# ielhelw/mcmc-ammsb-gpu

Hardware: AMD Instinct MI355X
Metric: mini-batch edges/s (SG-MCMC a-MMSB learner loop) (higher is better)
Workload: dtype f32

## Files before the change

### include/ammsb.h

```cpp
#ifndef AMMSB_H
#define AMMSB_H

#include <stddef.h>
#include <stdint.h>

#ifdef __cplusplus
extern "C" {
#endif

#define AMMSB_VERSION 200

enum {
  AMMSB_OK = 0,
  AMMSB_EINVAL = -1,
  AMMSB_EHIP = -2,
  AMMSB_ENOMEM = -3,
  AMMSB_ENODEV = -4,
  AMMSB_ERANGE = -5
};

#define AMMSB_MAX_GROUPS 65535u
#define AMMSB_RPM_MAX_BLOCKS 32

typedef struct { uint64_t x, y; } ammsb_seed;

typedef struct {
  uint64_t N, K, E;
  uint32_t num_node_sample;
  float alpha, a, b, c, epsilon, eta0, eta1;
} ammsb_params;

typedef struct {
  void* blocks[AMMSB_RPM_MAX_BLOCKS];
  uint64_t rows_in_block;
  uint64_t num_rows, num_cols;
  uint32_t num_blocks;
} ammsb_rpm;

typedef struct {
  const uint64_t* slots;
  uint64_t num_bins;
  uint32_t prime_idx;
} ammsb_set;

typedef struct {
  double link_ll, nonlink_ll;
  uint64_t link_cnt, nonlink_cnt;
} ammsb_ppx_sums;

typedef struct ammsb_ctx ammsb_ctx;

#define AMMSB_NOISE_OFF 1u
#define AMMSB_PHI_STREAMING 2u

int ammsb_version(void);
const char* ammsb_strerror(int code);
const char* ammsb_last_error(const ammsb_ctx* ctx);

int ammsb_params_quantize(ammsb_params* p);
float ammsb_eps_t(const ammsb_params* p, uint32_t step_count);

int ammsb_ctx_create(int device_id, const ammsb_params* params, ammsb_ctx** out);
int ammsb_ctx_destroy(ammsb_ctx* ctx);
int ammsb_ctx_params(const ammsb_ctx* ctx, ammsb_params* out);

int ammsb_rng_init(ammsb_ctx* ctx, ammsb_seed* seeds, uint64_t n, uint64_t sx, uint64_t sy, void* stream);
int ammsb_rng_init_mixed(ammsb_ctx* ctx, ammsb_seed* seeds, uint64_t n, uint64_t sx, uint64_t sy, void* stream);

int ammsb_set_has(ammsb_ctx* ctx, const ammsb_set* set, const uint64_t* keys, uint64_t n, uint8_t* out,
                  void* stream);

uint64_t ammsb_set_num_bins(uint64_t n);
int ammsb_set_build(ammsb_ctx* ctx, const uint64_t* keys, uint64_t n, uint64_t* slots, uint64_t num_bins,
                    uint32_t* prime_idx_out, uint32_t* scratch, void* stream);

int ammsb_pi_init_gamma(ammsb_ctx* ctx, const ammsb_rpm* pi, float* phi_sum, float eta0, float eta1,
                        ammsb_seed* seeds, void* stream);

int ammsb_sample_neighbors(ammsb_ctx* ctx, ammsb_seed* seeds, const uint32_t* nodes, uint32_t n_nodes,
                           uint32_t wg, uint32_t* table, uint32_t* packed, void* stream);

int ammsb_update_phi(ammsb_ctx* ctx, const float* beta, const ammsb_rpm* pi, const float* phi_sum,
                     const ammsb_set* training_set, const uint32_t* nodes, const uint32_t* neighbors,
                     uint32_t n_nodes, uint32_t step_count, ammsb_seed* seeds, uint32_t wg, uint32_t flags,
                     uint32_t group_begin, uint32_t group_end, float* phi_vec, void* stream);

int ammsb_update_phi_occupancy(ammsb_ctx* ctx, uint32_t wg, int* blocks_per_cu, int* waves_per_block);

int ammsb_update_pi(ammsb_ctx* ctx, const ammsb_rpm* pi, float* phi_sum, const float* phi_vec,
                    const uint32_t* nodes, uint32_t n_nodes, uint32_t wg, void* stream);

int ammsb_theta_sum(ammsb_ctx* ctx, float* out, void* stream);

int ammsb_beta_grads(ammsb_ctx* ctx, const float* theta, const float* beta, const ammsb_rpm* pi,
                     const ammsb_set* training_set, const uint64_t* edges, uint32_t n_edges,
                     uint32_t edge_begin, uint32_t edge_end, uint32_t wg, float* grads_out, void* stream);

int ammsb_can_fuse_pi_beta(ammsb_ctx* ctx, uint32_t phi_wg, uint32_t beta_wg);
int ammsb_update_pi_beta_grads(ammsb_ctx* ctx, const float* theta, const float* beta, const ammsb_rpm* pi,
                               float* phi_sum, const float* phi_vec, const uint32_t* nodes,
                               const ammsb_set* training_set, const uint64_t* edges, uint32_t n_edges, uint32_t wg,
                               float* grads_out, void* stream);

int ammsb_sum_rows_f32(ammsb_ctx* ctx, const float* in, uint32_t rows, uint32_t cols, float* out, void* stream);

int ammsb_update_theta(ammsb_ctx* ctx, float* theta, float* beta, const float* grads, uint32_t step_count,
                       float scale, ammsb_seed* seeds, uint32_t flags, void* stream);

int ammsb_beta_from_theta(ammsb_ctx* ctx, const float* theta, float* beta, void* stream);

int ammsb_perplexity(ammsb_ctx* ctx, const float* beta, const ammsb_rpm* pi, const ammsb_set* heldout_set,
                     const uint64_t* edges, uint32_t n_edges, uint32_t edge_begin, uint32_t edge_end,
                     uint32_t call_count, uint32_t wg, float* ppx_per_edge, ammsb_ppx_sums* out, void* stream);


int ammsb_minibatch_link(ammsb_ctx* ctx, const uint64_t* csr_offsets, const uint32_t* csr_targets, uint32_t u,
                         uint32_t n, uint64_t* edges_out, uint32_t* nodes_out, void* stream);

uint32_t ammsb_minibatch_candidates(uint64_t N, uint32_t m);
uint32_t ammsb_minibatch_candidates_for(uint64_t N, uint32_t m, uint64_t excluded);
uint64_t ammsb_minibatch_workspace_bytes(uint32_t capacity);

int ammsb_minibatch_nonlink(ammsb_ctx* ctx, ammsb_seed* seeds, uint32_t n_candidates, uint32_t capacity, uint32_t u,
                            uint32_t m, const ammsb_set* training_set, const ammsb_set* heldout_set, void* workspace,
                            uint64_t* edges_out, uint32_t* nodes_out, uint32_t* count_out, void* stream);

typedef struct ammsb_loop ammsb_loop;

#define AMMSB_LOOP_TIMESTAMPS 1u

typedef struct {
  float* theta;
  float* beta;
  const ammsb_rpm* pi;
  float* phi_sum;
  const ammsb_set* training_set;
  const ammsb_set* heldout_set;
  ammsb_seed* phi_seeds;
  float* phi_vec;
  uint32_t phi_wg, phi_flags;
  ammsb_seed* beta_seeds;
  float* grads;
  uint32_t beta_wg, beta_flags;
  uint64_t* edges[2];
  uint32_t* nodes[2];
  uint32_t* neighbors[2];
  uint32_t* nbr_table[2];
  ammsb_seed* nbr_seeds[2];
  uint32_t nbr_wg;
  const uint64_t* csr_offsets;
  const uint32_t* csr_targets;
  ammsb_seed* mb_seeds;
  uint32_t mb_candidates;
  void* mb_workspace;
  uint32_t* mb_count;
  uint32_t mini_batch;
  uint32_t max_fan_out;
  uint32_t max_nodes;
  uint32_t max_edges;
  uint32_t flags;
} ammsb_loop_config;

typedef struct {
  uint32_t link, u, n, n_candidates;
} ammsb_mb_choice;

int ammsb_loop_create(ammsb_ctx* ctx, const ammsb_loop_config* cfg, ammsb_loop** out);
int ammsb_loop_destroy(ammsb_loop* loop);
// ... 30 lines not shown
```

### mcmc-ammsb-gpu_amd/_capi.py

```python
import ctypes as C
import os

_HERE = os.path.dirname(os.path.abspath(__file__))
LIB_PATH = os.environ.get("AMMSB_HIP_LIB") or os.path.join(_HERE, "libammsb_hip.so")

RPM_MAX_BLOCKS = 32
MAX_GROUPS = 65535
NOISE_OFF = 1
PHI_STREAMING = 2


class AmmsbError(RuntimeError):
    pass


class Params(C.Structure):
    _fields_ = [("N", C.c_uint64), ("K", C.c_uint64), ("E", C.c_uint64),
                ("num_node_sample", C.c_uint32),
                ("alpha", C.c_float), ("a", C.c_float), ("b", C.c_float), ("c", C.c_float),
                ("epsilon", C.c_float), ("eta0", C.c_float), ("eta1", C.c_float)]


class Rpm(C.Structure):
    _fields_ = [("blocks", C.c_void_p * RPM_MAX_BLOCKS), ("rows_in_block", C.c_uint64),
                ("num_rows", C.c_uint64), ("num_cols", C.c_uint64), ("num_blocks", C.c_uint32)]


class SetDesc(C.Structure):
    _fields_ = [("slots", C.c_void_p), ("num_bins", C.c_uint64), ("prime_idx", C.c_uint32)]


class PpxSums(C.Structure):
    _fields_ = [("link_ll", C.c_double), ("nonlink_ll", C.c_double),
                ("link_cnt", C.c_uint64), ("nonlink_cnt", C.c_uint64)]


_vp, _u32, _u64, _f32 = C.c_void_p, C.c_uint32, C.c_uint64, C.c_float
_P = C.POINTER

LOOP_TIMESTAMPS = 1


class LoopConfig(C.Structure):
    _fields_ = [("theta", _vp), ("beta", _vp), ("pi", _P(Rpm)), ("phi_sum", _vp),
                ("training_set", _P(SetDesc)), ("heldout_set", _P(SetDesc)),
                ("phi_seeds", _vp), ("phi_vec", _vp), ("phi_wg", _u32), ("phi_flags", _u32),
                ("beta_seeds", _vp), ("grads", _vp), ("beta_wg", _u32), ("beta_flags", _u32),
                ("edges", _vp * 2), ("nodes", _vp * 2), ("neighbors", _vp * 2), ("nbr_table", _vp * 2),
                ("nbr_seeds", _vp * 2), ("nbr_wg", _u32),
                ("csr_offsets", _vp), ("csr_targets", _vp), ("mb_seeds", _vp), ("mb_candidates", _u32),
                ("mb_workspace", _vp), ("mb_count", _vp), ("mini_batch", _u32), ("max_fan_out", _u32),
                ("max_nodes", _u32), ("max_edges", _u32), ("flags", _u32)]


class MbChoice(C.Structure):
    _fields_ = [("link", _u32), ("u", _u32), ("n", _u32), ("n_candidates", _u32)]


SIGNATURES = {
    "ammsb_version": [],
    "ammsb_strerror": [C.c_int],
    "ammsb_last_error": [_vp],
    "ammsb_last_kernel_name": [_vp, C.c_int],
    "ammsb_params_quantize": [_P(Params)],
    "ammsb_eps_t": [_P(Params), _u32],
    "ammsb_ctx_create": [C.c_int, _P(Params), _P(_vp)],
    "ammsb_ctx_destroy": [_vp],
    "ammsb_theta_sum": [_vp, _vp, _vp],
    "ammsb_ctx_params": [_vp, _P(Params)],
    "ammsb_rng_init": [_vp, _vp, _u64, _u64, _u64, _vp],
    "ammsb_rng_init_mixed": [_vp, _vp, _u64, _u64, _u64, _vp],
    "ammsb_set_has": [_vp, _P(SetDesc), _vp, _u64, _vp, _vp],
    "ammsb_set_num_bins": [_u64],
    "ammsb_set_build": [_vp, _vp, _u64, _vp, _u64, _P(_u32), _vp, _vp],
    "ammsb_pi_init_gamma": [_vp, _P(Rpm), _vp, _f32, _f32, _vp, _vp],
    "ammsb_sample_neighbors": [_vp, _vp, _vp, _u32, _u32, _vp, _vp, _vp],
    "ammsb_update_phi": [_vp, _vp, _P(Rpm), _vp, _P(SetDesc), _vp, _vp, _u32, _u32, _vp, _u32, _u32,
                         _u32, _u32, _vp, _vp],
    "ammsb_update_phi_occupancy": [_vp, _u32, _P(C.c_int), _P(C.c_int)],
    "ammsb_update_pi": [_vp, _P(Rpm), _vp, _vp, _vp, _u32, _u32, _vp],
    "ammsb_beta_grads": [_vp, _vp, _vp, _P(Rpm), _P(SetDesc), _vp, _u32, _u32, _u32, _u32, _vp, _vp],
    "ammsb_can_fuse_pi_beta": [_vp, _u32, _u32],
    "ammsb_update_pi_beta_grads": [_vp, _vp, _vp, _P(Rpm), _vp, _vp, _vp, _P(SetDesc), _vp, _u32, _u32, _vp, _vp],
    "ammsb_sum_rows_f32": [_vp, _vp, _u32, _u32, _vp, _vp],
    "ammsb_update_theta": [_vp, _vp, _vp, _vp, _u32, _f32, _vp, _u32, _vp],
    "ammsb_beta_from_theta": [_vp, _vp, _vp, _vp],
    "ammsb_perplexity": [_vp, _vp, _P(Rpm), _P(SetDesc), _vp, _u32, _u32, _u32, _u32, _u32, _vp, _vp, _vp],
    "ammsb_minibatch_link": [_vp, _vp, _vp, _u32, _u32, _vp, _vp, _vp],
    "ammsb_minibatch_candidates": [_u64, _u32],
    "ammsb_minibatch_candidates_for": [_u64, _u32, _u64],
    "ammsb_minibatch_workspace_bytes": [_u32],
    "ammsb_minibatch_nonlink": [_vp, _vp, _u32, _u32, _u32, _u32, _P(SetDesc), _P(SetDesc), _vp, _vp, _vp, _vp, _vp],
    "ammsb_loop_create": [_vp, _P(LoopConfig), _P(_vp)],
    "ammsb_loop_destroy": [_vp],
    "ammsb_loop_run": [_vp, _P(MbChoice), _P(MbChoice), _u32, _u32, _u32, _vp],
    "ammsb_loop_check": [_vp, _P(_u32)],
    "ammsb_loop_status": [_vp, _P(_u32), _P(_u32)],
    "ammsb_loop_timestamps": [_vp, _u32, _u32, _P(C.c_double), _P(C.c_double)],
    "ammsb_loop_step_stamps": [_vp, _u32, _u32, _P(C.c_double)],
    "ammsb_wg_sum_f32": [_vp, _vp, _vp, _u32, _u32, _u32, _vp],
    "ammsb_wg_sum_u32": [_vp, _vp, _vp, _u32, _u32, _u32, _vp],
    "ammsb_wg_normalize_f32": [_vp, _vp, _vp, _u32, _u32, _u32, _vp],
    "ammsb_rpm_sum_f32": [_vp, _P(Rpm), _vp, _u32, _vp],
    "ammsb_rpm_normalize_f32": [_vp, _P(Rpm), _vp, _u32, _vp],
    "ammsb_wg_sort_u32": [_vp, _vp, _vp, _u32, _vp],
    "ammsb_wg_sort_f32": [_vp, _vp, _vp, _u32, _vp],
    "ammsb_randn_fill": [_vp, _vp, _u32, _u32, _vp, _vp],
    "ammsb_rpm_fetch": [_vp, _P(Rpm), _u64, _u64, _vp, _vp],
    "ammsb_clock_probe": [_vp, _vp, _u32, _u32, _vp],
}
_OTHER_RES = {"ammsb_strerror": C.c_char_p, "ammsb_last_error": C.c_char_p, "ammsb_last_kernel_name": C.c_char_p,
              "ammsb_eps_t": C.c_float,
              "ammsb_minibatch_candidates": C.c_uint32, "ammsb_minibatch_candidates_for": C.c_uint32,
              "ammsb_minibatch_workspace_bytes": C.c_uint64, "ammsb_set_num_bins": C.c_uint64}

_lib = None


def load(path=None):
    global _lib
    if _lib is not None and path is None:
        return _lib
    so = path or LIB_PATH
    if not os.path.exists(so):
        raise AmmsbError("%s not found: build it with `make -C mcmc-ammsb-gpu_amd/csrc` "
                         "(or __graft_entry__.build()); there is no CPU fallback" % so)
    import torch
    lib = C.CDLL(so)
    for name, args in SIGNATURES.items():
        fn = getattr(lib, name)
        fn.argtypes = args
        fn.restype = _OTHER_RES.get(name, C.c_int)
    if path is None:
        _lib = lib
    return lib


def check(rc, ctx=None):
    if rc != 0:
        lib = load()
        msg = lib.ammsb_strerror(rc).decode()
        if ctx:
            msg += " (" + lib.ammsb_last_error(ctx).decode() + ")"
        raise AmmsbError("ammsb call failed: %d %s" % (rc, msg))
```

### mcmc-ammsb-gpu_amd/csrc/ammsb_core.hip

```cpp
#include <math.h>
#include <stdlib.h>
#include <string.h>

#include "ammsb_ctx.h"
#include "ammsb_dev.h"
#include "ammsb_step.h"

using namespace ammsb;


extern "C" int ammsb_version(void) { return AMMSB_VERSION; }

extern "C" const char* ammsb_strerror(int code) {
  switch (code) {
    case AMMSB_OK: return "ok";
    case AMMSB_EINVAL: return "invalid argument";
    case AMMSB_EHIP: return "HIP runtime error";
    case AMMSB_ENOMEM: return "out of device memory";
    case AMMSB_ENODEV: return "no usable gfx950 device";
    case AMMSB_ERANGE: return "size out of range for the launch shape";
    default: return "unknown error";
  }
}

// ... 165 lines not shown
  AMMSB_CHECK_ARG(ctx, m, "null matrix");
  AMMSB_CHECK_ARG(ctx, m->num_blocks >= 1 && m->num_blocks <= AMMSB_RPM_MAX_BLOCKS, "bad block count");
  AMMSB_CHECK_ARG(ctx, m->rows_in_block > 0 && m->num_cols > 0, "bad block shape");
  AMMSB_CHECK_ARG(ctx, (uint64_t)m->num_blocks * m->rows_in_block >= m->num_rows, "blocks do not cover rows");
  for (uint32_t i = 0; i < m->num_blocks; ++i) AMMSB_CHECK_ARG(ctx, m->blocks[i], "null block");
  return AMMSB_OK;
}


__global__ __launch_bounds__(64) void pi_init_kernel(ammsb_rpm pi, float* phi_sum, float eta0, float eta1,
                                                      ammsb_seed* seeds, uint32_t G) {
  using Grp = Group<32>;
  __shared__ ZigTables zig;
  zig_load(&zig);
  __syncthreads();
  const uint32_t g = blockIdx.x * Grp::PER_BLOCK + Grp::slot();
  const uint32_t l = Grp::lane();
  const bool live = g < G;
  ammsb_seed s = {0, 0};
  if (live) s = seeds[(uint64_t)g * 32 + l];
  const uint64_t N = pi.num_rows, K = pi.num_cols;
  const uint64_t trips = (N + G - 1) / G;
  int phase = 0;
  for (uint64_t t = 0; t < trips; ++t) {
    const uint64_t row = g + t * G;
    const bool on = live && row < N;
    float* r = on ? rpm_row(pi, row) : nullptr;
    float lsum = 0;
    if (on)
      for (uint64_t j = l; j < K; j += 32) {
        const float v = rng_gamma(s, &zig, eta0, eta1);
        r[j] = v;
        lsum += v;
      }
    const float sum = Grp::sum(lsum, (float*)nullptr, phase);
    if (on) {
      for (uint64_t j = l; j < K; j += 32) r[j] = r[j] / sum;
      if (l == 0) phi_sum[row] = sum;
    }
  }
  if (live) seeds[(uint64_t)g * 32 + l] = s;
}

extern "C" int ammsb_pi_init_gamma(ammsb_ctx* ctx, const ammsb_rpm* pi, float* phi_sum, float eta0, float eta1,
                                   ammsb_seed* seeds, void* stream) {
  AMMSB_CHECK_ARG(ctx, ctx && phi_sum && seeds, "null argument");
  int rc = check_rpm(ctx, pi);
  if (rc) return rc;
  const uint32_t G = pi->num_rows < AMMSB_MAX_GROUPS ? (uint32_t)pi->num_rows : AMMSB_MAX_GROUPS;
  pi_init_kernel<<<div_up(G, 2), 64, 0, as_stream(stream)>>>(*pi, phi_sum, eta0, eta1, seeds, G);
  AMMSB_LAUNCH_CHECK(ctx);
  return AMMSB_OK;
}


__device__ __forceinline__ void ns_generate(ammsb_seed& seed, uint32_t* out, uint32_t capacity, uint32_t max_id,
                                            uint32_t node) {
  uint32_t r, val;
  do {
    do {
      r = (uint32_t)(rng_next(seed) % (uint64_t)(max_id + 1));
    } while (r == node);
    const uint32_t l1 = (r ^ 553105253u) % capacity;
    const uint32_t l2 = 1u + (capacity << 1);
    for (uint32_t i = 0;; ++i) {
      const uint32_t offset = (l1 + i * l2) % capacity;
      val = out[offset];
      if (val == r) break;
      if (val == max_id + 1) {
        out[offset] = r;
        break;
      }
    }
  } while (val == r);
}

__host__ __device__ __forceinline__ uint32_t ns_global_size(uint32_t n_nodes, uint32_t wg) {
  uint32_t groups = n_nodes / wg + (n_nodes % wg ? 1 : 0);
  const uint32_t maxg = AMMSB_MAX_GROUPS / wg;
  if (groups > maxg) groups = maxg;
  return groups * wg;
}

__global__ __launch_bounds__(64) void sample_neighbors_kernel(ammsb_seed* seeds, const uint32_t* nodes,
                                                               uint32_t n_nodes, uint32_t N, uint32_t n,
                                                               uint32_t gsize, uint32_t* table, uint32_t* packed,
                                                               const ammsb_step_desc* desc, uint32_t wg) {
  if (desc) {
    n_nodes = desc->n_nodes;
    gsize = ns_global_size(n_nodes, wg);
  }
  const uint32_t gid = blockIdx.x * blockDim.x + threadIdx.x;
  if (gid >= gsize || gid >= n_nodes) return;
  const uint32_t capacity = 2 * n;
  ammsb_seed seed = seeds[gid];
  for (uint32_t i = gid; i < n_nodes; i += gsize) {
    uint32_t* out = table + (uint64_t)i * capacity;
    uint32_t* pk = packed + (uint64_t)i * n;
    const uint32_t node = nodes[i];
    for (uint32_t j = 0; j < capacity; ++j) out[j] = N;
    for (uint32_t j = 0; j < n; ++j) ns_generate(seed, out, capacity, N - 1, node);
    uint32_t count = 0;
    for (uint32_t j = 0; j < capacity && count < n; ++j) {
      const uint32_t v = out[j];
      if (v != N) pk[count++] = v;
    }
  }
  seeds[gid] = seed;
}

__global__ __launch_bounds__(64) void sample_neighbors_lds_kernel(ammsb_seed* seeds, const uint32_t* nodes,
                                                                   uint32_t n_nodes, uint32_t N, uint32_t n,
                                                                   uint32_t gsize, uint32_t* table, uint32_t* packed,
                                                                   const ammsb_step_desc* desc, uint32_t wg) {
  if (desc) {
    n_nodes = desc->n_nodes;
    gsize = ns_global_size(n_nodes, wg);
    if (blockIdx.x * 64 >= gsize || blockIdx.x * 64 >= n_nodes) return;
  }
  extern __shared__ uint32_t lds[];
  constexpr uint32_t S = 65;
  const uint32_t lane = threadIdx.x;
  const uint32_t gid = blockIdx.x * 64 + lane;
  const uint32_t capacity = 2 * n;
  const bool owner = gid < gsize && gid < n_nodes;
  ammsb_seed seed = owner ? seeds[gid] : ammsb_seed{0, 0};
  const uint32_t max_id = N - 1;
  const FastMod mod_n = fast_mod_init((uint64_t)max_id + 1);
  const uint64_t cap_m = ~0ull / capacity + 1;
  auto advance = [](uint32_t& row, uint32_t& col, uint32_t width) {
    col += 64;
    while (col >= width) {
      col -= width;
      ++row;
    }
  };
  for (uint32_t base = blockIdx.x * 64; base < n_nodes; base += gsize) {
    const uint32_t i = base + lane;
    const bool on = owner && i < n_nodes;
    const uint32_t live = min(64u, min(n_nodes - base, gsize - blockIdx.x * 64));
    for (uint32_t j = 0; j < capacity; ++j) lds[j * S + lane] = N;
    if (on) {
      const uint32_t node = nodes[i];
      for (uint32_t j = 0; j < n; ++j) {
        uint32_t r, val;
        do {
          do {
            r = (uint32_t)fast_mod(rng_next(seed), mod_n);
          } while (r == node);
          uint32_t offset = (uint32_t)__umul64hi(cap_m * (uint64_t)(r ^ 553105253u), capacity);
          for (;;) {
            val = lds[offset * S + lane];
            if (val == r) break;
            if (val == max_id + 1) {
              lds[offset * S + lane] = r;
              break;
            }
            offset = offset + 1 == capacity ? 0 : offset + 1;
          }
        } while (val == r);
      }
    }
    __syncthreads();
    uint32_t* tout = table + (uint64_t)base * capacity;
    {
      uint32_t row = 0, col = lane;
      while (col >= capacity) {
        col -= capacity;
        ++row;
      }
      for (uint32_t x = lane; x < live * capacity; x += 64) {
        tout[x] = lds[col * S + row];
        advance(row, col, capacity);
      }
    }
    __syncthreads();
    if (on) {
      uint32_t count = 0;
      for (uint32_t j = 0; j < capacity && count < n; ++j) {
        const uint32_t v = lds[j * S + lane];
        if (v != N) lds[(count++) * S + lane] = v;
      }
    }
    __syncthreads();
    uint32_t* pout = packed + (uint64_t)base * n;
    {
      uint32_t row = 0, col = lane;
      while (col >= n) {
        col -= n;
        ++row;
      }
      for (uint32_t x = lane; x < live * n; x += 64) {
        pout[x] = lds[col * S + row];
        advance(row, col, n);
      }
    }
    __syncthreads();
  }
  if (owner) seeds[gid] = seed;
}

__global__ __launch_bounds__(256) void sample_neighbors_wave_kernel(ammsb_seed* seeds, const uint32_t* nodes,
                                                                     uint32_t n_nodes, uint32_t N, uint32_t gsize,
                                                                     uint32_t* table, uint32_t* packed,
                                                                     const ammsb_step_desc* desc, uint32_t wg) {
  constexpr uint32_t CAP = 64, NN = 32, B = 40;
  if (desc) {
    n_nodes = desc->n_nodes;
    gsize = ns_global_size(n_nodes, wg);
  }
  const uint32_t lane = threadIdx.x & 63;
  const uint32_t gid = __builtin_amdgcn_readfirstlane(blockIdx.x * 4 + (threadIdx.x >> 6));
  if (gid >= gsize || gid >= n_nodes) return;
  ammsb_seed st = seeds[gid];
  const FastMod mod_n = fast_mod_init((uint64_t)N);
  for (uint32_t i = gid; i < n_nodes; i += gsize) {
    const uint32_t node = nodes[i];
    uint32_t slot = N;
    uint32_t count = 0;
    while (count < NN) {
      ammsb_seed run = st, mine = st;
      uint64_t raw = 0;
#pragma unroll 8
      for (uint32_t j = 0; j < B; ++j) {
        const uint64_t x = rng_next(run);
        if (lane == j) {
          raw = x;
          mine = run;
        }
      }
      const uint32_t r = (uint32_t)fast_mod(raw, mod_n);
      const uint32_t h = (r ^ 553105253u) & (CAP - 1);
      uint32_t used = 0;
      for (uint32_t j = 0; j < B && count < NN; ++j) {
        used = j + 1;
        const uint32_t rj = (uint32_t)__builtin_amdgcn_readlane((int)r, (int)j);
        if (rj == node) continue;
        if (__ballot(slot == rj) != 0ull) continue;
        const uint32_t hj = (uint32_t)__builtin_amdgcn_readlane((int)h, (int)j);
        const unsigned long long freeb = ~__ballot(slot != N);
        const unsigned long long rot = hj ? ((freeb >> hj) | (freeb << (64 - hj))) : freeb;
        const uint32_t pos = (hj + (uint32_t)__builtin_ctzll(rot)) & (CAP - 1);
        if (lane == pos) slot = rj;
        ++count;
      }
      auto lane64 = [&](uint64_t v) -> uint64_t {
        const uint32_t hi = (uint32_t)__builtin_amdgcn_readlane((int)(uint32_t)(v >> 32), (int)(used - 1));
        const uint32_t lo = (uint32_t)__builtin_amdgcn_readlane((int)(uint32_t)v, (int)(used - 1));
        return ((uint64_t)hi << 32) | lo;
      };
      st.x = lane64(mine.x);
      st.y = lane64(mine.y);
    }
    table[(uint64_t)i * CAP + lane] = slot;
    const unsigned long long occ = __ballot(slot != N);
    if (slot != N) packed[(uint64_t)i * NN + __popcll(occ & ((1ull << lane) - 1ull))] = slot;
  }
  if (lane == 0) seeds[gid] = st;
}

static int sample_neighbors_common(ammsb_ctx* ctx, ammsb_seed* seeds, const uint32_t* nodes, uint32_t n_nodes,
                                   uint32_t wg, uint32_t* table, uint32_t* packed, const ammsb_step_desc* desc,
                                   void* stream) {
  AMMSB_CHECK_ARG(ctx, ctx && seeds && nodes && table && packed, "null argument");
  AMMSB_CHECK_ARG(ctx, wg >= 1 && wg <= 1024, "sampler wg out of range");
  if (n_nodes == 0) return AMMSB_OK;
  const uint32_t n = ctx->params.num_node_sample;
  AMMSB_CHECK_ARG(ctx, ctx->params.N > (uint64_t)n + 1, "N must exceed num_node_sample + 1");
  const uint32_t gsize = ns_global_size(n_nodes, wg);
  const size_t lds_bytes = (size_t)2 * n * 65 * sizeof(uint32_t);
  static const bool per_thread = [] {
    const char* f = getenv("AMMSB_NBR_FORM");
    return f && f[0] == 't';
  }();
  if (n == 32 && !per_thread && n_nodes <= 20000) {
    const uint32_t waves = gsize < n_nodes ? gsize : n_nodes;
    ctx->kernel_name[AMMSB_KN_NBR] = "sample_neighbors_wave_kernel";
    sample_neighbors_wave_kernel<<<div_up(waves, 4), 256, 0, as_stream(stream)>>>(
        seeds, nodes, n_nodes, (uint32_t)ctx->params.N, gsize, table, packed, desc, wg);
  } else if (lds_bytes <= 64 * 1024) {
    ctx->kernel_name[AMMSB_KN_NBR] = "sample_neighbors_lds_kernel";
    sample_neighbors_lds_kernel<<<div_up(gsize, 64), 64, lds_bytes, as_stream(stream)>>>(
        seeds, nodes, n_nodes, (uint32_t)ctx->params.N, n, gsize, table, packed, desc, wg);
  } else {
    ctx->kernel_name[AMMSB_KN_NBR] = "sample_neighbors_kernel";
    sample_neighbors_kernel<<<div_up(gsize, 64), 64, 0, as_stream(stream)>>>(
        seeds, nodes, n_nodes, (uint32_t)ctx->params.N, n, gsize, table, packed, desc, wg);
  }
  AMMSB_LAUNCH_CHECK(ctx);
  return AMMSB_OK;
}

extern "C" int ammsb_sample_neighbors(ammsb_ctx* ctx, ammsb_seed* seeds, const uint32_t* nodes, uint32_t n_nodes,
                                      uint32_t wg, uint32_t* table, uint32_t* packed, void* stream) {
  return sample_neighbors_common(ctx, seeds, nodes, n_nodes, wg, table, packed, nullptr, stream);
}

int ammsb_sample_neighbors_d(ammsb_ctx* ctx, ammsb_seed* seeds, const uint32_t* nodes, uint32_t n_nodes_cap, uint32_t wg,
                             uint32_t* table, uint32_t* packed, const ammsb_step_desc* desc, void* stream) {
  AMMSB_CHECK_ARG(ctx, ctx && desc, "null descriptor");
  return sample_neighbors_common(ctx, seeds, nodes, n_nodes_cap, wg, table, packed, desc, stream);
}


__device__ __forceinline__ uint32_t power_of_2(uint32_t v) {
  v |= v >> 1;
  v |= v >> 2;
  v |= v >> 4;
  v |= v >> 8;
  v |= v >> 16;
  return v + 1;
}

template <typename T>
__device__ __forceinline__ T wg_sum_lds(const T* in, T* aux, uint32_t len) {
  const uint32_t lid = threadIdx.x, lsize = blockDim.x;
  T lsum = 0;
  for (uint32_t i = lid; i < len; i += lsize) lsum += in[i];
  aux[lid] = lsum;
  __syncthreads();
  for (uint32_t p2 = power_of_2(lsize) >> 1; p2 > 0; p2 >>= 1) {
    if (lid < p2 && lid + p2 < lsize) aux[lid] += aux[lid + p2];
    __syncthreads();
  }
  const T r = aux[0];
  __syncthreads();
  return r;
}

template <typename T>
__global__ void wg_sum_kernel(const T* in, T* out, uint32_t rows, uint32_t len) {
  __shared__ T aux[1024];
  for (uint32_t gid = blockIdx.x; gid < rows; gid += gridDim.x) {
    const T s = wg_sum_lds(in + (uint64_t)gid * len, aux, len);
    if (threadIdx.x == 0) out[gid] = s;
  }
}

__global__ void wg_normalize_kernel(float* in, float* sums, uint32_t rows, uint32_t len) {
  __shared__ float aux[1024];
  for (uint32_t gid = blockIdx.x; gid < rows; gid += gridDim.x) {
    float* row = in + (uint64_t)gid * len;
    const float sum = wg_sum_lds(row, aux, len);
    for (uint32_t i = threadIdx.x; i < len; i += blockDim.x) row[i] = row[i] / sum;
    if (sums && threadIdx.x == 0) sums[gid] = sum;
    __syncthreads();
  }
}

__global__ void rpm_sum_kernel(ammsb_rpm m, float* out, int normalize) {
  __shared__ float aux[1024];
  for (uint64_t gid = blockIdx.x; gid < m.num_rows; gid += gridDim.x) {
    float* row = rpm_row(m, gid);
    const float sum = wg_sum_lds(row, aux, (uint32_t)m.num_cols);
    if (normalize)
      for (uint64_t i = threadIdx.x; i < m.num_cols; i += blockDim.x) row[i] = row[i] / sum;
    if (threadIdx.x == 0) out[gid] = sum;
    __syncthreads();
  }
}

template <typename T>
__global__ void wg_sort_kernel(const T* in, T* out) {
  __shared__ T aux[1024];
  const size_t i = threadIdx.x, wg = blockDim.x;
  aux[i] = in[i];
  __syncthreads();
  for (size_t length = 1; length < wg; length <<= 1) {
    const bool direction = ((i & (length << 1)) != 0);
    for (size_t inc = length; inc > 0; inc >>= 1) {
      const size_t j = i ^ inc;
      const T idata = aux[i], jdata = aux[j];
      const bool smaller = (jdata < idata) || (jdata == idata && j < i);
      const bool swap = smaller ^ (j < i) ^ direction;
      __syncthreads();
      aux[i] = swap ? jdata : idata;
      __syncthreads();
    }
  }
  out[i] = aux[i];
}

static inline uint32_t cap_groups(uint64_t rows) { return rows < AMMSB_MAX_GROUPS ? (uint32_t)rows : AMMSB_MAX_GROUPS; }

// ... 107 lines not shown
```

### mcmc-ammsb-gpu_amd/csrc/ammsb_loop.hip

```cpp
#include "ammsb_ctx.h"
#include "ammsb_step.h"

#include <stdlib.h>
#include <string.h>

#include <atomic>
#include <chrono>
#include <mutex>
#include <new>
#include <thread>
#include <vector>

namespace {

constexpr uint32_t CHUNK = 1024;
constexpr uint32_t STAMP_CAP = AMMSB_STAMP_CAP;
constexpr int NBUF = 3;

__global__ void loop_prime_kernel(const ammsb_step_desc* ring, uint32_t* cursor, ammsb_step_desc* cur,
                                  ammsb_step_desc* nxt, const uint32_t* timeouts) {
  *cur = ring[0];
  *nxt = ring[2];
  *cursor = 0;
  if (timeouts && *timeouts != 0u) {
    cur->n_nodes = 0;
    cur->n_edges = 0;
  }
}

constexpr int HS_MAIN = 0, HS_AVAIL = 1, HS_TIMEOUTS = 2;

__global__ void loop_wait_kernel(const uint32_t* a, const uint32_t* b, int min_diff, uint32_t* timeouts,
                                 unsigned long long max_ticks, const ammsb_step_desc* src, ammsb_step_desc* dst,
                                 uint32_t fail_at) {
  const uint32_t have = *b;
  const unsigned long long t0 = wall_clock64();
  bool ok = false;
  for (;;) {
    if (__hip_atomic_load(timeouts, __ATOMIC_ACQUIRE, __HIP_MEMORY_SCOPE_AGENT) != 0u) break;
    if (fail_at != 0u && have + 1u == fail_at) {
      atomicAdd(timeouts, 1u);
      break;
    }
    const uint32_t v = __hip_atomic_load(a, __ATOMIC_ACQUIRE, __HIP_MEMORY_SCOPE_AGENT);
    if ((int)(v - have) >= min_diff) {
      ok = true;
      break;
    }
    if (wall_clock64() - t0 > max_ticks) {
      atomicAdd(timeouts, 1u);
      break;
    }
    __builtin_amdgcn_s_sleep(8);
  }
  if (dst) {
    if (ok) {
      *dst = *src;
    } else {
      ammsb_step_desc skip = *src;
      skip.n_nodes = 0;
      skip.n_edges = 0;
      skip.n_cand = 0;
      *dst = skip;
    }
  }
}

__global__ void loop_bump_kernel(uint32_t* counter, const ammsb_step_desc* desc) {
  if (ammsb_desc_skip(desc)) return;
  __hip_atomic_store(counter, *counter + 1u, __ATOMIC_RELEASE, __HIP_MEMORY_SCOPE_AGENT);
}

__global__ void loop_copy_kernel(uint4* dst, const uint4* src, size_t bytes, const uint32_t* timeouts) {
  if (timeouts && *timeouts != 0u) return;
  const size_t n16 = bytes / 16;
  for (size_t i = (size_t)blockIdx.x * blockDim.x + threadIdx.x; i < n16; i += (size_t)gridDim.x * blockDim.x)
    dst[i] = src[i];
  if (blockIdx.x == 0 && threadIdx.x < (bytes % 16) / 4)
    reinterpret_cast<uint32_t*>(dst + n16)[threadIdx.x] = reinterpret_cast<const uint32_t*>(src + n16)[threadIdx.x];
}

__global__ void loop_probe_wait_kernel(const uint32_t* flag, uint32_t* saw, unsigned long long max_ticks) {
  const unsigned long long t0 = wall_clock64();
  while (wall_clock64() - t0 <= max_ticks) {
    if (__hip_atomic_load(flag, __ATOMIC_ACQUIRE, __HIP_MEMORY_SCOPE_AGENT) != 0u) {
      *saw = 1u;
      return;
    }
    __builtin_amdgcn_s_sleep(8);
  }
  *saw = 0u;
}
__global__ void loop_probe_set_kernel(uint32_t* flag) { __hip_atomic_store(flag, 1u, __ATOMIC_RELEASE, __HIP_MEMORY_SCOPE_AGENT); }

struct Stage {
  ammsb_step_desc* ring;
  hipEvent_t done;
  bool used;
};

struct SampleBuf {
  uint64_t* edges;
  uint32_t* nodes;
  uint32_t* neighbors;
  uint32_t* nbr_table;
};

}

struct ammsb_loop {
  ammsb_ctx* ctx;
  ammsb_loop_config c;
  ammsb_rpm pi;
  ammsb_set training, heldout;
  bool has_heldout;
  hipStream_t main, side;
  hipEvent_t ev_in, ev_out, ev_prime, ev_first;
  hipEvent_t ev_main[NBUF], ev_samp[NBUF];
  SampleBuf buf[NBUF];
  void* own_mem;
  ammsb_step_desc* d_ring;
  uint32_t* d_cursor;
  ammsb_step_desc* d_cur[2];
  ammsb_step_desc* d_nxt[NBUF];
  uint32_t* d_hs;
  ammsb_step_desc* d_samp[NBUF];
  bool use_events;
  bool direct_only;
  uint32_t fallbacks;
  uint32_t test_fail_at;
  struct Run {
    ammsb_mb_choice pending;
    std::vector<ammsb_mb_choice> next;
    uint32_t n_steps, first_step_count, parity;
    hipStream_t stream;
    uint64_t main_start;
  };
  std::vector<Run>* runs;
  uint64_t main_total;
  unsigned long long wait_ticks;
  unsigned long long* d_stamps;
  Stage stage[2];
  int next_stage;
  hipGraphExec_t exec_main[2][NBUF][2];
  hipGraphExec_t exec_samp[2][NBUF][2];
  uint32_t link_nodes_cap, link_edges_cap, n_nbr;
  float w_link, w_nonlink;
  int wall_khz;
  uint64_t graphs_launched;
  bool serial_launch;
  bool eager_launch;
  bool host_prof;
  double t_side_us, t_main_us, t_run_us, t_pro_us, t_epi_us;
  uint64_t runs_done;
};

namespace {

#define LOOP_HIP(lp, call)                                                                              \
  do {                                                                                                  \
    hipError_t e_ = (call);                                                                             \
    if (e_ != hipSuccess) {                                                                             \
      snprintf((lp)->ctx->err, sizeof((lp)->ctx->err), "%s: %s -> %s", __func__, #call, hipGetErrorString(e_)); \
      return AMMSB_EHIP;                                                                                \
    }                                                                                                   \
  } while (0)

#define LOOP_RC(call)         \
  do {                        \
    const int rc_ = (call);   \
    if (rc_ != AMMSB_OK) return rc_; \
  } while (0)

int record_sampler(ammsb_loop* lp, int nl, int b, int sp, const ammsb_step_desc* desc, hipStream_t st) {
  const ammsb_loop_config& c = lp->c;
  ammsb_ctx* ctx = lp->ctx;
  const SampleBuf& o = lp->buf[b];
  const uint32_t m = c.mini_batch;
  if (!lp->use_events) {
    loop_wait_kernel<<<1, 1, 0, st>>>(lp->d_hs + HS_MAIN, lp->d_hs + HS_AVAIL, -2, lp->d_hs + HS_TIMEOUTS, lp->wait_ticks,
                                      desc, lp->d_samp[b], lp->test_fail_at);
    LOOP_HIP(lp, hipGetLastError());
    desc = lp->d_samp[b];
  }
  if (nl)
    LOOP_RC(ammsb_minibatch_link_d(ctx, c.csr_offsets, c.csr_targets, lp->link_edges_cap, o.edges, o.nodes, desc, st));
  else
    LOOP_RC(ammsb_minibatch_nonlink_d(ctx, c.mb_seeds, c.mb_candidates, m, &lp->training,
                                      lp->has_heldout ? &lp->heldout : nullptr, c.mb_workspace, o.edges, o.nodes,
                                      c.mb_count, desc, st));
  LOOP_RC(ammsb_sample_neighbors_d(ctx, c.nbr_seeds[sp], o.nodes, nl ? lp->link_nodes_cap : m + 1, c.nbr_wg, o.nbr_table,
                                   o.neighbors, desc, st));
  if (!lp->use_events) {
    loop_bump_kernel<<<1, 1, 0, st>>>(lp->d_hs + HS_AVAIL, desc);
    LOOP_HIP(lp, hipGetLastError());
  }
  return AMMSB_OK;
}

int record_main(ammsb_loop* lp, int cl, int b, int dp, hipStream_t st) {
  const ammsb_loop_config& c = lp->c;
  ammsb_ctx* ctx = lp->ctx;
  const SampleBuf& in = lp->buf[b];
  const ammsb_step_desc* cur = lp->d_cur[dp];
  const uint32_t m = c.mini_batch;
  const uint32_t cap_nodes = cl ? lp->link_nodes_cap : m + 1;
  const uint32_t cap_edges = cl ? lp->link_edges_cap : m;
  LOOP_RC(ammsb_update_phi_d(ctx, c.beta, &lp->pi, c.phi_sum, &lp->training, in.nodes, in.neighbors, cap_nodes,
                             c.phi_seeds, c.phi_wg, c.phi_flags, c.phi_vec, cur, lp->d_stamps, st));
  const bool fuse_pi = ammsb_beta_can_fuse_pi(ctx, c.phi_wg, c.beta_wg) && lp->pi.num_cols % 4 == 0;
  const ammsb_pi_fusion fuse = {c.phi_vec, c.phi_sum, in.nodes, lp->d_stamps};
  if (!fuse_pi)
    LOOP_RC(ammsb_update_pi_d(ctx, &lp->pi, c.phi_sum, c.phi_vec, in.nodes, cap_nodes, c.phi_wg, cur, lp->d_stamps, st));
  const bool hs = !lp->use_events;
  const ammsb_step_advance adv = {lp->d_ring, lp->d_cursor, lp->d_cur[1 - dp], lp->d_nxt[b], 3u,
                                  hs ? lp->d_hs + HS_MAIN : nullptr, hs ? lp->d_hs + HS_AVAIL : nullptr,
                                  hs ? lp->d_hs + HS_TIMEOUTS : nullptr, lp->wait_ticks, lp->d_stamps};
  LOOP_RC(ammsb_beta_step_d(ctx, c.theta, c.beta, &lp->pi, &lp->training, in.edges, cap_edges, c.beta_wg, c.grads,
                            c.beta_seeds, c.beta_flags, cur, &adv, fuse_pi ? &fuse : nullptr, lp->d_stamps, st));
  return AMMSB_OK;
}

int capture(ammsb_loop* lp, int kind, int link, int b, int dp, hipGraphExec_t* out) {
  hipStream_t st = kind == 2 ? lp->side : lp->main;
  LOOP_HIP(lp, hipStreamBeginCapture(st, hipStreamCaptureModeThreadLocal));
  const int rc = kind == 2 ? record_sampler(lp, link, b, dp, lp->d_nxt[b], st) : record_main(lp, link, b, dp, st);
  hipGraph_t g = nullptr;
  const hipError_t e = hipStreamEndCapture(st, &g);
  if (rc != AMMSB_OK) {
    if (g) (void)hipGraphDestroy(g);
    return rc;
  }
  if (e != hipSuccess || !g) {
    snprintf(lp->ctx->err, sizeof lp->ctx->err, "ammsb_loop: hipStreamEndCapture -> %s", hipGetErrorString(e));
    return AMMSB_EHIP;
  }
  const hipError_t e2 = hipGraphInstantiate(out, g, nullptr, nullptr, 0);
  (void)hipGraphDestroy(g);
  if (e2 != hipSuccess) {
    snprintf(lp->ctx->err, sizeof lp->ctx->err, "ammsb_loop: hipGraphInstantiate -> %s", hipGetErrorString(e2));
    return AMMSB_EHIP;
  }
  return AMMSB_OK;
}

void destroy(ammsb_loop* lp) {
  if (!lp) return;
  if (lp->host_prof && lp->graphs_launched)
    fprintf(stderr,
            "ammsb_loop host profile: %llu steps, hipGraphLaunch sampler %.2f us, main %.2f us per step; %llu runs: %.1f us "
            "each (prologue %.1f, epilogue %.1f)\n",
            (unsigned long long)lp->graphs_launched, lp->t_side_us / lp->graphs_launched, lp->t_main_us / lp->graphs_launched,
            (unsigned long long)lp->runs_done, lp->t_run_us / lp->runs_done, lp->t_pro_us / lp->runs_done, lp->t_epi_us / lp->runs_done);
  if (lp->main) (void)hipStreamSynchronize(lp->main);
  if (lp->side) (void)hipStreamSynchronize(lp->side);
  for (int a = 0; a < 2; ++a)
    for (int b = 0; b < NBUF; ++b)
      for (int p = 0; p < 2; ++p) {
        if (lp->exec_main[a][b][p]) (void)hipGraphExecDestroy(lp->exec_main[a][b][p]);
        if (lp->exec_samp[a][b][p]) (void)hipGraphExecDestroy(lp->exec_samp[a][b][p]);
      }
  for (Stage& st : lp->stage) {
    if (st.ring) (void)hipHostFree(st.ring);
    if (st.done) (void)hipEventDestroy(st.done);
  }
  for (hipEvent_t ev : {lp->ev_in, lp->ev_out, lp->ev_prime, lp->ev_first, lp->ev_main[0], lp->ev_main[1], lp->ev_main[2],
                        lp->ev_samp[0], lp->ev_samp[1], lp->ev_samp[2]})
    if (ev) (void)hipEventDestroy(ev);
  if (lp->d_ring) (void)hipFree(lp->d_ring);
  if (lp->d_stamps) (void)hipFree(lp->d_stamps);
  if (lp->d_hs) (void)hipFree(lp->d_hs);
  if (lp->own_mem) (void)hipFree(lp->own_mem);
  if (lp->side) (void)hipStreamDestroy(lp->side);
  if (lp->main) (void)hipStreamDestroy(lp->main);
  delete lp->runs;
  delete lp;
}

ammsb_step_desc make_desc(const ammsb_loop* lp, const ammsb_mb_choice& ch, uint32_t step) {
  ammsb_step_desc d;
  memset(&d, 0, sizeof d);
  if (ch.link) {
    d.n_nodes = ch.n + 1;
    d.n_edges = ch.n;
    d.scale = lp->w_link;
  } else {
    d.n_nodes = lp->c.mini_batch + 1;
    d.n_edges = lp->c.mini_batch;
    d.scale = lp->w_nonlink;
  }
  d.eps_t = ammsb_eps_t(&lp->ctx->params, step);
  d.u = ch.u;
  d.link = ch.link ? 1u : 0u;
  d.n_cand = ch.n_candidates;
  d.step = step;
  return d;
}

int check_choice(ammsb_loop* lp, const ammsb_mb_choice& ch) {
  ammsb_ctx* ctx = lp->ctx;
  AMMSB_CHECK_ARG(ctx, ch.u < ctx->params.N, "mini-batch vertex out of range");
  if (ch.link) {
    AMMSB_CHECK_ARG(ctx, ch.n > 0 && ch.n <= lp->link_edges_cap, "link batch: degree 0 or above max_fan_out");
  } else {
    AMMSB_CHECK_ARG(ctx, ch.n_candidates >= lp->c.mini_batch && ch.n_candidates <= lp->c.mb_candidates &&
                             ch.n_candidates % 256 == 0,
                    "non-link batch: bad candidate count");
  }
  return AMMSB_OK;
}

size_t align256(size_t x) { return (x + 255) & ~(size_t)255; }

}

extern "C" int ammsb_loop_create(ammsb_ctx* ctx, const ammsb_loop_config* cfg, ammsb_loop** out) {
  AMMSB_CHECK_ARG(ctx, ctx && cfg && out, "null argument");
  const ammsb_loop_config& c = *cfg;
  AMMSB_CHECK_ARG(ctx, c.theta && c.beta && c.pi && c.phi_sum && c.training_set && c.phi_seeds && c.phi_vec &&
                           c.beta_seeds && c.grads,
                  "null model / operator buffer");
  for (int i = 0; i < 2; ++i)
    AMMSB_CHECK_ARG(ctx, c.edges[i] && c.nodes[i] && c.neighbors[i] && c.nbr_table[i] && c.nbr_seeds[i],
                    "null sample buffer");
  for (int i = 0; i < 2; ++i)
    AMMSB_CHECK_ARG(ctx, ((reinterpret_cast<uintptr_t>(c.edges[i]) | reinterpret_cast<uintptr_t>(c.nodes[i]) |
                           reinterpret_cast<uintptr_t>(c.neighbors[i]) | reinterpret_cast<uintptr_t>(c.nbr_table[i])) & 15u) == 0,
                    "edges / nodes / neighbors / nbr_table must be 16-byte aligned");
  AMMSB_CHECK_ARG(ctx, c.csr_offsets && c.csr_targets && c.mb_seeds && c.mb_workspace && c.mb_count,
                  "null mini-batch sampler buffer");
  AMMSB_CHECK_ARG(ctx, c.mini_batch > 0 && c.max_fan_out > 0, "mini_batch / max_fan_out must be positive");
  AMMSB_CHECK_ARG(ctx, c.mb_candidates >= c.mini_batch && c.mb_candidates % 256 == 0, "bad candidate capacity");
  AMMSB_CHECK_ARG(ctx, c.max_nodes >= c.mini_batch + 1 && c.max_nodes >= c.max_fan_out + 1 && c.max_edges >= c.mini_batch &&
                           c.max_edges >= c.max_fan_out,
                  "max_nodes / max_edges smaller than the largest mini-batch (sample.cc:129-131)");
  AMMSB_HIP(ctx, hipSetDevice(ctx->device));
  ammsb_loop* lp = new (std::nothrow) ammsb_loop();
  if (!lp) return AMMSB_ENOMEM;
  memset(static_cast<void*>(lp), 0, sizeof *lp);
  lp->ctx = ctx;
  lp->c = c;
  lp->pi = *c.pi;
  lp->training = *c.training_set;
  lp->has_heldout = c.heldout_set != nullptr;
  if (lp->has_heldout) lp->heldout = *c.heldout_set;
  lp->c.pi = &lp->pi;
  lp->c.training_set = &lp->training;
  lp->c.heldout_set = lp->has_heldout ? &lp->heldout : nullptr;
  lp->link_edges_cap = c.max_fan_out;
  lp->link_nodes_cap = c.max_fan_out + 1;
  lp->n_nbr = ctx->params.num_node_sample;
  lp->w_link = static_cast<float>(ctx->params.N);
  lp->w_nonlink = static_cast<float>(2 * ctx->params.E) / static_cast<float>(c.mini_batch);
#define CREATE_HIP(call)                                                                           \
  do {                                                                                             \
    hipError_t e_ = (call);                                                                        \
    if (e_ != hipSuccess) {                                                                        \
      snprintf(ctx->err, sizeof ctx->err, "ammsb_loop_create: %s -> %s", #call, hipGetErrorString(e_)); \
      destroy(lp);                                                                                 \
      return AMMSB_EHIP;                                                                           \
    }                                                                                              \
  } while (0)
  {
    static const int prio = [] {
      const char* f = getenv("AMMSB_LOOP_PRIO");
      return f ? atoi(f) : 0;
    }();
    int least = 0, greatest = 0;
    if (prio) CREATE_HIP(hipDeviceGetStreamPriorityRange(&least, &greatest));
    static const int side_cus = [] {
      const char* f = getenv("AMMSB_LOOP_SIDE_CUS");
      return f ? atoi(f) : 0;
    }();
    if (side_cus > 0 && side_cus < ctx->num_cus) {
      uint32_t mask[16] = {0};
      for (int i = 0; i < side_cus && i < 512; ++i) mask[i / 32] |= 1u << (i % 32);
      CREATE_HIP(hipStreamCreateWithFlags(&lp->main, hipStreamNonBlocking));
      CREATE_HIP(hipExtStreamCreateWithCUMask(&lp->side, (uint32_t)((ctx->num_cus + 31) / 32), mask));
    } else if (prio && least != greatest) {
      CREATE_HIP(hipStreamCreateWithPriority(&lp->main, hipStreamNonBlocking, greatest));
      CREATE_HIP(hipStreamCreateWithPriority(&lp->side, hipStreamNonBlocking, least));
    } else {
      CREATE_HIP(hipStreamCreateWithFlags(&lp->main, hipStreamNonBlocking));
      CREATE_HIP(hipStreamCreateWithFlags(&lp->side, hipStreamNonBlocking));
    }
  }
  for (hipEvent_t* ev : {&lp->ev_in, &lp->ev_out, &lp->ev_prime, &lp->ev_first, &lp->ev_main[0], &lp->ev_main[1],
                         &lp->ev_main[2], &lp->ev_samp[0], &lp->ev_samp[1], &lp->ev_samp[2]})
    CREATE_HIP(hipEventCreateWithFlags(ev, hipEventDisableTiming));
  for (int i = 0; i < 2; ++i) lp->buf[i] = SampleBuf{c.edges[i], c.nodes[i], c.neighbors[i], c.nbr_table[i]};
  {
    const size_t e_b = align256(sizeof(uint64_t) * c.max_edges), n_b = align256(sizeof(uint32_t) * c.max_nodes);
    const size_t p_b = align256(sizeof(uint32_t) * (size_t)c.max_nodes * lp->n_nbr);
    const size_t t_b = align256(sizeof(uint32_t) * (size_t)c.max_nodes * 2 * lp->n_nbr);
    CREATE_HIP(hipMalloc(&lp->own_mem, e_b + n_b + p_b + t_b));
    CREATE_HIP(hipMemset(lp->own_mem, 0, e_b + n_b + p_b + t_b));
    char* p = static_cast<char*>(lp->own_mem);
    lp->buf[2].edges = reinterpret_cast<uint64_t*>(p);
    lp->buf[2].nodes = reinterpret_cast<uint32_t*>(p + e_b);
    lp->buf[2].neighbors = reinterpret_cast<uint32_t*>(p + e_b + n_b);
    lp->buf[2].nbr_table = reinterpret_cast<uint32_t*>(p + e_b + n_b + p_b);
  }
  lp->runs = new (std::nothrow) std::vector<ammsb_loop::Run>();
  if (!lp->runs) {
    destroy(lp);
    return AMMSB_ENOMEM;
  }
  const size_t n_desc = CHUNK + 4 + 8;
  CREATE_HIP(hipMalloc(&lp->d_ring, sizeof(ammsb_step_desc) * n_desc + 64));
  CREATE_HIP(hipMemset(lp->d_ring, 0, sizeof(ammsb_step_desc) * n_desc + 64));
  lp->d_cur[0] = lp->d_ring + CHUNK + 4;
  lp->d_cur[1] = lp->d_ring + CHUNK + 5;
  lp->d_nxt[0] = lp->d_ring + CHUNK + 6;
  lp->d_nxt[1] = lp->d_ring + CHUNK + 7;
  lp->d_nxt[2] = lp->d_ring + CHUNK + 8;
  for (int b = 0; b < NBUF; ++b) lp->d_samp[b] = lp->d_ring + CHUNK + 9 + b;
  lp->d_cursor = reinterpret_cast<uint32_t*>(lp->d_ring + n_desc);
  {
    CREATE_HIP(hipMalloc(&lp->d_hs, 64));
    const uint32_t hs0[4] = {0u, 1u, 0u, 0u};
    CREATE_HIP(hipMemcpy(lp->d_hs, hs0, sizeof hs0, hipMemcpyHostToDevice));
    const char* mode = getenv("AMMSB_LOOP_HANDSHAKE");
    const char* pmc = getenv("ROCPROF_COUNTER_COLLECTION");
    auto truthy = [](const char* v) { return v && v[0] && strcmp(v, "0") != 0 && strcmp(v, "False") != 0 && strcmp(v, "false") != 0; };
    const bool serialising_tool = truthy(pmc) || truthy(getenv("AMD_SERIALIZE_KERNEL")) || truthy(getenv("HIP_LAUNCH_BLOCKING")) ||
                                  truthy(getenv("CUDA_LAUNCH_BLOCKING"));
    lp->use_events = mode ? strcmp(mode, "event") == 0 : serialising_tool;
    int khz0 = 100000;
    CREATE_HIP(hipDeviceGetAttribute(&khz0, hipDeviceAttributeWallClockRate, ctx->device));
    if (!lp->use_events && !(mode && strcmp(mode, "flag") == 0)) {
      uint32_t* probe = lp->d_hs + 8;
      CREATE_HIP(hipMemset(probe, 0, 2 * sizeof(uint32_t)));
      loop_probe_wait_kernel<<<1, 1, 0, lp->main>>>(probe, probe + 1, 20ull * (unsigned long long)(khz0 > 0 ? khz0 : 100000));
      CREATE_HIP(hipGetLastError());
      loop_probe_set_kernel<<<1, 1, 0, lp->side>>>(probe);
      CREATE_HIP(hipGetLastError());
      CREATE_HIP(hipStreamSynchronize(lp->main));
      CREATE_HIP(hipStreamSynchronize(lp->side));
      uint32_t saw = 0;
      CREATE_HIP(hipMemcpy(&saw, probe + 1, sizeof saw, hipMemcpyDeviceToHost));
      if (!saw) lp->use_events = true;
    }
    if (const char* f = getenv("AMMSB_LOOP_TEST_FAIL_AT")) {
      const long v = strtol(f, nullptr, 10);
      if (v > 0) {
        lp->test_fail_at = (uint32_t)v;
        fprintf(stderr, "ammsb_loop: AMMSB_LOOP_TEST_FAIL_AT=%ld -- the sampler chain of mini-batch %ld will be made to give up (fault injection)\n", v, v);
      }
    }
    lp->host_prof = getenv("AMMSB_LOOP_HOSTPROF") != nullptr;
    const char* lm = getenv("AMMSB_LOOP_LAUNCH");
    lp->serial_launch = lm && strcmp(lm, "serial") == 0;
    lp->eager_launch = !(lm && strcmp(lm, "graph") == 0) && !lp->serial_launch && !lp->use_events;
    int khz = 100000;
    CREATE_HIP(hipDeviceGetAttribute(&khz, hipDeviceAttributeWallClockRate, ctx->device));
    lp->wait_ticks = 5000ull * (unsigned long long)(khz > 0 ? khz : 100000);
    if (const char* w = getenv("AMMSB_LOOP_WAIT_MS")) {
      char* end = nullptr;
      const long ms = strtol(w, &end, 10);
      if (end == w || *end != '\0' || ms < 1 || ms > 600000) {
        fprintf(stderr, "ammsb_loop: AMMSB_LOOP_WAIT_MS='%s' ignored (want 1 .. 600000); waits give up after 5 s\n", w);
      } else {
        lp->wait_ticks = (unsigned long long)ms * (unsigned long long)(khz > 0 ? khz : 100000);
        fprintf(stderr, "ammsb_loop: AMMSB_LOOP_WAIT_MS=%ld -- device-side waits give up after %ld ms\n", ms, ms);
      }
    }
  }
  for (Stage& st : lp->stage) {
    CREATE_HIP(hipHostMalloc(&st.ring, sizeof(ammsb_step_desc) * (CHUNK + 4), hipHostMallocDefault));
    CREATE_HIP(hipEventCreateWithFlags(&st.done, hipEventDisableTiming));
    st.used = false;
  }
  if (c.flags & AMMSB_LOOP_TIMESTAMPS) {
    CREATE_HIP(hipMalloc(&lp->d_stamps, sizeof(unsigned long long) * AMMSB_STAMP_SLOTS * STAMP_CAP));
    CREATE_HIP(hipMemset(lp->d_stamps, 0, sizeof(unsigned long long) * AMMSB_STAMP_SLOTS * STAMP_CAP));
    CREATE_HIP(hipDeviceGetAttribute(&lp->wall_khz, hipDeviceAttributeWallClockRate, ctx->device));
  }
#undef CREATE_HIP
  for (int link = 0; link < 2; ++link)
    for (int b = 0; b < NBUF; ++b)
      for (int dp = 0; dp < 2; ++dp) {
        int rc = capture(lp, 1, link, b, dp, &lp->exec_main[link][b][dp]);
        if (rc == AMMSB_OK) rc = capture(lp, 2, link, b, dp, &lp->exec_samp[link][b][dp]);
        if (rc != AMMSB_OK) {
          destroy(lp);
          return rc;
        }
      }
  *out = lp;
  return AMMSB_OK;
}

extern "C" int ammsb_loop_destroy(ammsb_loop* lp) {
  destroy(lp);
  return AMMSB_OK;
}

static std::mutex g_submit_mutex;

namespace {

int submit(ammsb_loop* lp, const ammsb_mb_choice* pending, const ammsb_mb_choice* next, uint32_t n_steps,
           uint32_t first_step_count, uint32_t parity, hipStream_t s, uint32_t done0, uint32_t avail0) {
  ammsb_ctx* ctx = lp->ctx;
  const uint32_t p0 = parity;
  const bool ev = lp->use_events;
  using clk = std::chrono::steady_clock;
  auto us_since = [](clk::time_point t) { return std::chrono::duration<double, std::micro>(clk::now() - t).count(); };
  const clk::time_point t_run = clk::now();
  auto choice = [&](uint32_t j) -> const ammsb_mb_choice& { return j == 0 ? *pending : next[j - 1]; };
  LOOP_HIP(lp, hipEventRecord(lp->ev_in, s));
  LOOP_HIP(lp, hipStreamWaitEvent(lp->main, lp->ev_in, 0));
  uint32_t done = done0;
  if (done0 == n_steps && avail0 <= n_steps) {
    Stage& st = lp->stage[lp->next_stage];
    lp->next_stage ^= 1;
    if (st.used) LOOP_HIP(lp, hipEventSynchronize(st.done));
    st.ring[0] = make_desc(lp, choice(n_steps), first_step_count + n_steps);
    LOOP_HIP(lp, hipMemcpyAsync(lp->d_ring, st.ring, sizeof(ammsb_step_desc), hipMemcpyHostToDevice, lp->main));
    LOOP_HIP(lp, hipEventRecord(st.done, lp->main));
    st.used = true;
    LOOP_HIP(lp, hipEventRecord(lp->ev_prime, lp->main));
    LOOP_HIP(lp, hipStreamWaitEvent(lp->side, lp->ev_prime, 0));
    LOOP_RC(record_sampler(lp, choice(n_steps).link ? 1 : 0, (int)((p0 + n_steps) % NBUF), (int)((p0 + n_steps) & 1u),
                           lp->d_ring, lp->side));
    if (ev) LOOP_HIP(lp, hipEventRecord(n_steps == 1 ? lp->ev_first : lp->ev_samp[(n_steps - 2) % NBUF], lp->side));
  }
  while (done < n_steps) {
    const uint32_t cnt = n_steps - done < CHUNK ? n_steps - done : CHUNK;
    const clk::time_point t_pro = clk::now();
    Stage& st = lp->stage[lp->next_stage];
    lp->next_stage ^= 1;
    if (st.used) LOOP_HIP(lp, hipEventSynchronize(st.done));
    for (uint32_t i = 0; i < cnt + 4; ++i) {
      const uint32_t j = done + i <= n_steps ? done + i : n_steps;
      st.ring[i] = make_desc(lp, choice(j), first_step_count + done + i);
    }
    LOOP_HIP(lp, hipMemcpyAsync(lp->d_ring, st.ring, sizeof(ammsb_step_desc) * (cnt + 4), hipMemcpyHostToDevice, lp->main));
    LOOP_HIP(lp, hipEventRecord(st.done, lp->main));
    st.used = true;
    const int dp0 = (int)((p0 + done) & 1u);
    loop_prime_kernel<<<1, 1, 0, lp->main>>>(lp->d_ring, lp->d_cursor, lp->d_cur[dp0], lp->d_nxt[(p0 + done + 2) % NBUF],
                                             ev ? nullptr : lp->d_hs + HS_TIMEOUTS);
    LOOP_HIP(lp, hipGetLastError());
    LOOP_RC(ammsb_theta_coef_d(ctx, lp->c.theta, lp->c.beta, lp->main));
    LOOP_HIP(lp, hipEventRecord(lp->ev_prime, lp->main));
    if (done == done0) {
      const uint32_t hi = done0 + 2 < n_steps + 1 ? done0 + 2 : n_steps + 1;
      for (uint32_t j = avail0 > done0 ? avail0 : done0; j < hi; ++j) {
        if (j == 0) continue;
        LOOP_HIP(lp, hipStreamWaitEvent(lp->side, lp->ev_prime, 0));
        LOOP_RC(record_sampler(lp, choice(j).link ? 1 : 0, (int)((p0 + j) % NBUF), (int)((p0 + j) & 1u),
                               lp->d_ring + (j - done0), lp->side));
        if (ev) LOOP_HIP(lp, hipEventRecord(j == 1 ? lp->ev_first : lp->ev_samp[(j - 2) % NBUF], lp->side));
      }
    }
    lp->t_pro_us += us_since(t_pro);
    bool threaded = !ev && cnt >= 32 && !lp->serial_launch && avail0 <= 1;
    if (threaded) {
      hipError_t side_err = hipSuccess;
      int side_rc = AMMSB_OK, main_rc = AMMSB_OK;
      std::atomic<uint32_t> main_sub(0), side_sub(0);
      std::atomic<bool> stop(false);
      const clk::time_point ts = clk::now();
      auto side_body = [&]() {
        side_err = hipSetDevice(ctx->device);
        if (side_err == hipSuccess) side_err = hipStreamWaitEvent(lp->side, lp->ev_prime, 0);
        for (uint32_t i = 0; i < cnt && side_err == hipSuccess && side_rc == AMMSB_OK && !stop.load(); ++i) {
          const uint32_t gi = done + i;
          if (gi + 2 > n_steps) break;
          while (main_sub.load(std::memory_order_acquire) < i) std::this_thread::yield();
          const int b = (int)((p0 + gi + 2) % NBUF), dp = (int)((p0 + gi) & 1u), nl = choice(gi + 2).link ? 1 : 0;
          if (lp->eager_launch) side_rc = record_sampler(lp, nl, b, dp, lp->d_nxt[b], lp->side);
          else side_err = hipGraphLaunch(lp->exec_samp[nl][b][dp], lp->side);
          side_sub.store(i + 1, std::memory_order_release);
        }
        if (side_err != hipSuccess || side_rc != AMMSB_OK) stop.store(true);
        side_sub.store(cnt + 2, std::memory_order_release);
      };
      std::thread helper;
      try {
        helper = std::thread(side_body);
      } catch (...) {
        threaded = false;
      }
      if (threaded) {
        hipError_t main_err = hipSuccess;
        for (uint32_t i = 0; i < cnt && main_err == hipSuccess && main_rc == AMMSB_OK && !stop.load(); ++i) {
          const uint32_t gi = done + i;
          while (i >= 1 && side_sub.load(std::memory_order_acquire) < i) std::this_thread::yield();
          const int b = (int)((p0 + gi) % NBUF), dp = (int)((p0 + gi) & 1u), cl = choice(gi).link ? 1 : 0;
          if (lp->eager_launch) main_rc = record_main(lp, cl, b, dp, lp->main);
          else main_err = hipGraphLaunch(lp->exec_main[cl][b][dp], lp->main);
          main_sub.store(i + 1, std::memory_order_release);
        }
        if (main_err != hipSuccess || main_rc != AMMSB_OK) stop.store(true);
        main_sub.store(cnt + 2, std::memory_order_release);
        if (lp->host_prof) lp->t_main_us += us_since(ts);
        helper.join();
        if (lp->host_prof) lp->t_side_us += us_since(ts);
        LOOP_HIP(lp, side_err);
        LOOP_HIP(lp, main_err);
        LOOP_RC(side_rc);
        LOOP_RC(main_rc);
      }
    }
    if (!threaded)
    for (uint32_t i = 0; i < cnt; ++i) {
      const uint32_t gi = done + i;
      const int dp = (int)((p0 + gi) & 1u);
      const bool sample = gi + 2 <= n_steps && gi + 2 >= avail0;
      if (sample) {
        if (i == 0) LOOP_HIP(lp, hipStreamWaitEvent(lp->side, lp->ev_prime, 0));
        else if (ev) LOOP_HIP(lp, hipStreamWaitEvent(lp->side, lp->ev_main[(gi - 1) % NBUF], 0));
        const auto t0 = lp->host_prof ? std::chrono::steady_clock::now() : std::chrono::steady_clock::time_point();
        const int nl = choice(gi + 2).link ? 1 : 0, b = (int)((p0 + gi + 2) % NBUF);
        if (lp->direct_only) LOOP_RC(record_sampler(lp, nl, b, dp, lp->d_nxt[b], lp->side));
        else LOOP_HIP(lp, hipGraphLaunch(lp->exec_samp[nl][b][dp], lp->side));
        if (lp->host_prof) lp->t_side_us += std::chrono::duration<double, std::micro>(std::chrono::steady_clock::now() - t0).count();
        if (ev) LOOP_HIP(lp, hipEventRecord(lp->ev_samp[gi % NBUF], lp->side));
      }
      if (ev && gi >= avail0) {
        if (gi == 1) LOOP_HIP(lp, hipStreamWaitEvent(lp->main, lp->ev_first, 0));
        else LOOP_HIP(lp, hipStreamWaitEvent(lp->main, lp->ev_samp[(gi - 2) % NBUF], 0));
      }
      const auto t1 = lp->host_prof ? std::chrono::steady_clock::now() : std::chrono::steady_clock::time_point();
      const int cl = choice(gi).link ? 1 : 0, bm = (int)((p0 + gi) % NBUF);
      if (lp->direct_only) LOOP_RC(record_main(lp, cl, bm, dp, lp->main));
      else LOOP_HIP(lp, hipGraphLaunch(lp->exec_main[cl][bm][dp], lp->main));
      if (lp->host_prof) lp->t_main_us += std::chrono::duration<double, std::micro>(std::chrono::steady_clock::now() - t1).count();
      if (ev) LOOP_HIP(lp, hipEventRecord(lp->ev_main[gi % NBUF], lp->main));
    }
    lp->graphs_launched += cnt;
    done += cnt;
  }
  const clk::time_point t_epi = clk::now();
  if (ev && n_steps >= avail0) LOOP_HIP(lp, hipStreamWaitEvent(lp->main, n_steps == 1 ? lp->ev_first : lp->ev_samp[(n_steps - 2) % NBUF], 0));
  if (!ev) {
    loop_wait_kernel<<<1, 1, 0, lp->main>>>(lp->d_hs + HS_AVAIL, lp->d_hs + HS_MAIN, 1, lp->d_hs + HS_TIMEOUTS, lp->wait_ticks,
                                            nullptr, nullptr, 0u);
    LOOP_HIP(lp, hipGetLastError());
  }
  const uint32_t from = (p0 + n_steps) % NBUF, to = (p0 + n_steps) & 1u;
  if (from != to) {
    const ammsb_mb_choice& ch = choice(n_steps);
    const size_t ne = ch.link ? ch.n : lp->c.mini_batch, nv = ne + 1;
    const SampleBuf &a = lp->buf[from], &b = lp->buf[to];
    const uint32_t* poison = ev ? nullptr : lp->d_hs + HS_TIMEOUTS;
    auto copy = [&](void* dst, const void* src, size_t bytes) {
      const size_t n16 = bytes / 16;
      const unsigned blocks = (unsigned)(n16 / 256 + 1 < 1024 ? n16 / 256 + 1 : 1024);
      loop_copy_kernel<<<blocks, 256, 0, lp->main>>>(static_cast<uint4*>(dst), static_cast<const uint4*>(src), bytes, poison);
    };
    copy(b.edges, a.edges, sizeof(uint64_t) * ne);
    copy(b.nodes, a.nodes, sizeof(uint32_t) * nv);
    copy(b.neighbors, a.neighbors, sizeof(uint32_t) * nv * lp->n_nbr);
    copy(b.nbr_table, a.nbr_table, sizeof(uint32_t) * nv * 2 * lp->n_nbr);
    LOOP_HIP(lp, hipGetLastError());
  }
  LOOP_HIP(lp, hipEventRecord(lp->ev_out, lp->main));
  LOOP_HIP(lp, hipStreamWaitEvent(s, lp->ev_out, 0));
  lp->t_epi_us += us_since(t_epi);
  lp->t_run_us += us_since(t_run);
  lp->runs_done += 1;
  return AMMSB_OK;
}

}

extern "C" int ammsb_loop_run(ammsb_loop* lp, const ammsb_mb_choice* pending, const ammsb_mb_choice* next,
                              uint32_t n_steps, uint32_t first_step_count, uint32_t parity, void* stream) {
  if (!lp) return AMMSB_EINVAL;
  ammsb_ctx* ctx = lp->ctx;
  AMMSB_CHECK_ARG(ctx, pending && (next || n_steps == 0), "null argument");
  AMMSB_CHECK_ARG(ctx, parity < 2 && first_step_count >= 1, "bad parity / step count");
  if (n_steps == 0) return AMMSB_OK;
  LOOP_RC(check_choice(lp, *pending));
  for (uint32_t i = 0; i < n_steps; ++i) LOOP_RC(check_choice(lp, next[i]));
  std::lock_guard<std::mutex> guard(g_submit_mutex);
  if (!lp->use_events) {
    try {
      ammsb_loop::Run r;
      r.pending = *pending;
      r.next.assign(next, next + n_steps);
      r.n_steps = n_steps;
      r.first_step_count = first_step_count;
      r.parity = parity;
      r.stream = as_stream(stream);
      r.main_start = lp->main_total;
      lp->runs->push_back(std::move(r));
    } catch (...) {
      return AMMSB_ENOMEM;
    }
  }
  lp->main_total += n_steps;
  return submit(lp, pending, next, n_steps, first_step_count, parity, as_stream(stream), 0u, 1u);
}

extern "C" int ammsb_loop_check(ammsb_loop* lp, uint32_t* wait_timeouts) {
  if (!lp) return AMMSB_EINVAL;
  ammsb_ctx* ctx = lp->ctx;
  AMMSB_CHECK_ARG(ctx, wait_timeouts, "null argument");
  std::lock_guard<std::mutex> guard(g_submit_mutex);
  LOOP_HIP(lp, hipStreamSynchronize(lp->side));
  LOOP_HIP(lp, hipStreamSynchronize(lp->main));
  uint32_t hs[3] = {0, 0, 0};
  LOOP_HIP(lp, hipMemcpy(hs, lp->d_hs, sizeof hs, hipMemcpyDeviceToHost));
  *wait_timeouts = 0;
  if (!hs[HS_TIMEOUTS]) {
    lp->runs->clear();
    return AMMSB_OK;
  }
  const uint64_t done_total = lp->main_total - (uint64_t)(uint32_t)((uint32_t)lp->main_total - hs[HS_MAIN]);
  const uint32_t avail_ahead = hs[HS_AVAIL] - hs[HS_MAIN];
  lp->use_events = true;
  lp->direct_only = true;
  lp->eager_launch = false;
  lp->fallbacks += 1;
  const uint32_t clear = 0;
  LOOP_HIP(lp, hipMemcpy(lp->d_hs + HS_TIMEOUTS, &clear, sizeof clear, hipMemcpyHostToDevice));
  std::vector<ammsb_loop::Run> runs;
  runs.swap(*lp->runs);
  const uint64_t avail_total = done_total + (avail_ahead <= 3 ? avail_ahead : 0);
  bool resumed = false;
  for (const ammsb_loop::Run& r : runs) {
    if (!resumed && r.main_start + r.n_steps <= done_total && r.main_start + r.n_steps < avail_total) continue;
    uint32_t done0 = 0, avail0 = 1;
    if (!resumed) {
      done0 = (uint32_t)(done_total > r.main_start ? done_total - r.main_start : 0);
      if (done0 > r.n_steps) done0 = r.n_steps;
      avail0 = (uint32_t)(avail_total > r.main_start ? avail_total - r.main_start : 0);
      if (avail0 == 0) avail0 = 1;
      resumed = true;
    }
    const int rc = submit(lp, &r.pending, r.next.data(), r.n_steps, r.first_step_count, r.parity, r.stream, done0, avail0);
    if (rc != AMMSB_OK) {
      *wait_timeouts = hs[HS_TIMEOUTS];
      return rc;
    }
  }
  LOOP_HIP(lp, hipStreamSynchronize(lp->side));
// ... 54 lines not shown
```

### mcmc-ammsb-gpu_amd/csrc/ammsb_phi.hip

```cpp
#pragma clang fp contract(off)

#include <stdlib.h>

#include "ammsb_ctx.h"
#include "ammsb_dev.h"
#include "ammsb_step.h"

#include <type_traits>

using namespace ammsb;

#ifdef AMMSB_PHI_TRACE
__device__ unsigned long long g_phi_trace[256];
#define PHI_TRACE(slot) do { if (blockIdx.x == 0 && threadIdx.x == 0 && (slot) < 256) g_phi_trace[(slot)] = __builtin_readcyclecounter(); } while (0)
extern "C" int ammsb_debug_trace(unsigned long long* out, int n) {
  return hipMemcpyFromSymbol(out, HIP_SYMBOL(g_phi_trace), sizeof(unsigned long long) * (n < 256 ? n : 256)) == hipSuccess ? 0 : -2;
}
#define AMMSB_PHI_BLK_CAP 65536
__device__ unsigned long long g_phi_blk[AMMSB_PHI_BLK_CAP * 5];
#define PHI_BLK(end) do { if (threadIdx.x == 0 && blockIdx.x < AMMSB_PHI_BLK_CAP) { \
    g_phi_blk[blockIdx.x * 5 + (end)] = __builtin_readcyclecounter(); \
    g_phi_blk[blockIdx.x * 5 + 2 + (end)] = __builtin_amdgcn_s_memrealtime(); \
    if (!(end)) g_phi_blk[blockIdx.x * 5 + 4] = (unsigned long long)__builtin_amdgcn_s_getreg((31 << 11) | 4) | \
                                               ((unsigned long long)__builtin_amdgcn_s_getreg((31 << 11) | 20) << 32); } } while (0)
extern "C" int ammsb_debug_blocks(unsigned long long* out, int n_blocks) {
  return hipMemcpyFromSymbol(out, HIP_SYMBOL(g_phi_blk), sizeof(unsigned long long) * 5 * (n_blocks < AMMSB_PHI_BLK_CAP ? n_blocks : AMMSB_PHI_BLK_CAP)) == hipSuccess ? 0 : -2;
}
#else
#define PHI_TRACE(slot) do { } while (0)
#define PHI_BLK(end) do { } while (0)
#endif

#ifndef AMMSB_PHI_LDS3_DEFAULT
#define AMMSB_PHI_LDS3_DEFAULT false
#endif

namespace {

struct PhiArgs {
  const float* beta;
  ammsb_rpm pi;
  const float* phi_sum;
  DevSet set;
  const uint32_t* nodes;
  const uint32_t* neighbors;
  ammsb_seed* seeds;
  float* phi_vec;
  uint32_t n_nodes, G, group_begin, group_end;
  uint32_t K, n;
  float eps_t, alpha, epsilon, Nn;
  uint32_t noise_on;
  uint32_t rows_nt;
  const ammsb_step_desc* desc;
  unsigned long long* stamps;
};


struct PhiStep {
  uint32_t n_nodes, G, group_end;
  float eps_t;
};
__device__ __forceinline__ PhiStep phi_step(const PhiArgs& a) {
  PhiStep st = {a.n_nodes, a.G, a.group_end, a.eps_t};
  if (a.desc) {
    st.n_nodes = a.desc->n_nodes;
    st.G = st.n_nodes < AMMSB_MAX_GROUPS ? st.n_nodes : AMMSB_MAX_GROUPS;
    st.group_end = st.G;
    st.eps_t = a.desc->eps_t;
  }
  return st;
}

template <int L, int KPT, int DEPTH, bool FULL, bool ONE = false>
__global__ __launch_bounds__(Group<L>::BLOCK) void update_phi_kernel(const PhiArgs a) {
  if constexpr (ONE) __builtin_assume(a.pi.num_blocks == 1);
  using Grp = Group<L>;
  extern __shared__ uint32_t s_nb_all[];
  __shared__ ZigTables zig;
  __shared__ float aux[Grp::AUX];

  const int l = Grp::lane();
  const int slot = Grp::slot();
  uint32_t* s_nb = s_nb_all + slot * a.n;
  const PhiStep st = phi_step(a);
  if (st.n_nodes == 0) return;
  note_stamp(a.stamps, a.desc, AMMSB_STAMP_PHI);
  const uint32_t g = a.group_begin + blockIdx.x * Grp::PER_BLOCK + slot;
  const bool live = g < st.group_end;
  const uint32_t K = a.K, n = a.n;
  const float EPS = a.epsilon;

  if (a.noise_on) zig_load(&zig);

  auto col = [&](int j) -> uint32_t { return l + j * L; };
  auto ccol = [&](int j) -> uint32_t {
    const uint32_t k = l + j * L;
    return FULL ? k : (k < K ? k : K - 1);
  };
  auto has = [&](int j) -> bool { return FULL || (uint32_t)(l + j * L) < K; };

  float bf[KPT];
  bool beta_safe = true;
#pragma unroll
  for (int j = 0; j < KPT; ++j) {
    const float b = a.beta[2 * ccol(j) + 1];
    bf[j] = b - EPS;
    beta_safe = beta_safe && in_range(b, EPS, kBetaHi);
  }

  ammsb_seed rs = {0, 0};
  if (live && a.noise_on) rs = a.seeds[(uint64_t)g * L + l];

  const uint32_t trips = (st.n_nodes + st.G - 1) / st.G;
  int phase = 0;
  for (uint32_t t = 0; t < trips; ++t) {
    const uint64_t i_raw = (uint64_t)g + (uint64_t)t * st.G;
    const bool on = live && i_raw < st.n_nodes;
    if constexpr (Grp::PER_BLOCK == 1) {
      if (!on) continue;
    }
    const uint64_t i = on ? i_raw : 0;
    const uint32_t node = a.nodes[i];

    __syncthreads();
    for (uint32_t q = l; q < n; q += L) {
      const uint32_t nb = a.neighbors[i * n + q];
      const bool y = set_has(a.set, make_edge(node, nb));
      s_nb[q] = nb | (y ? 0x80000000u : 0u);
    }
    __syncthreads();

    const float phi_sum = a.phi_sum[node];
    const float inv_phi_sum = 1.0f / phi_sum;
    const float* row_a = rpm_row(a.pi, node);
    float pi_a[KPT], grads[KPT], rden[KPT];
    bool node_safe = beta_safe && in_range(phi_sum, kPhiSumLo, kPhiSumHi);
#pragma unroll
    for (int j = 0; j < KPT; ++j) {
      const float x = row_a[ccol(j)];
      pi_a[j] = has(j) ? x : 0.0f;
      grads[j] = 0.0f;
      const float den = pi_a[j] * phi_sum;
      rden[j] = refined_rcp(den);
      node_safe = node_safe && (in_range(den, kDenLo, kDenHi) || !has(j));
    }

    float buf[DEPTH][KPT];
    auto load_row = [&](float (&dst)[KPT], uint32_t q) {
      uint32_t w = s_nb[q] & 0x7fffffffu;
      if constexpr (L >= 64) w = __builtin_amdgcn_readfirstlane(w);
      const float* row = rpm_row(a.pi, w);
#pragma unroll
      for (int j = 0; j < KPT; ++j) dst[j] = row[ccol(j)];
    };
    auto consume = [&](float (&pin)[KPT], uint32_t q) {
      bool y = (s_nb[q] >> 31) != 0;
      if constexpr (L >= 64) y = __builtin_amdgcn_readfirstlane((int)y) != 0;
      const float e = y ? EPS : 1.0f - EPS;
      float partial = 0.0f;
      float lo = 1.0f;
      if (y) {
#pragma unroll
        for (int j = 0; j < KPT; ++j) {
          float tt = pin[j] * bf[j];
          tt = tt + e;
          pin[j] = pi_a[j] * tt;
        }
      } else {
#pragma unroll
        for (int j = 0; j < KPT; ++j) {
          const float tt0 = pin[j] * bf[j];
          const float tt = e - tt0;
          pin[j] = pi_a[j] * tt;
        }
      }
#pragma unroll
      for (int j = 0; j < KPT; ++j) {
        partial += pin[j];
        lo = fminf(lo, has(j) ? fabsf(pin[j]) : 1.0f);
      }
      const float probs_sum = Grp::sum(partial, aux, phase);
      if (node_safe && lo >= kProbsLo && in_range(probs_sum, kPsumLo, kPsumHi)) {
        const float rps = refined_rcp(probs_sum);
#pragma unroll
        for (int j = 0; j < KPT; ++j) {
          float qv = div_with_rcp(pin[j], probs_sum, rps);
          qv = div_with_rcp(qv, pi_a[j] * phi_sum, rden[j]);
          grads[j] += qv - inv_phi_sum;
        }
      } else {
#pragma unroll
        for (int j = 0; j < KPT; ++j) {
          float qv = pin[j] / probs_sum;
          qv = qv / (pi_a[j] * phi_sum);
          grads[j] += qv - inv_phi_sum;
        }
      }
    };

    bool batched = false;
    if constexpr (KPT <= 2 && DEPTH == 4) {
      if (n % 4 == 0) {
        batched = true;
        float nxt[4][KPT];
        auto consume4 = [&](float (&pin)[4][KPT], uint32_t q0) {
          float ee[4], sg[4], part[4], lo[4], psum[4];
          bool fast[4], all_fast = true;
#pragma unroll
          for (int r = 0; r < 4; ++r) {
            const bool y = (s_nb[q0 + r] >> 31) != 0;
// ... 169 lines not shown
  auto group_sync = [&]() {
    if constexpr (NB == 1) {
      __syncthreads();
    } else {
      asm volatile("s_waitcnt lgkmcnt(0)" ::: "memory");
      __builtin_amdgcn_wave_barrier();
    }
  };

  const PhiStep st = phi_step(a);
  note_stamp(a.stamps, a.desc, AMMSB_STAMP_PHI);
  if constexpr (NB > 1) {
    if (a.noise_on) zig_load(&zig);
    __syncthreads();
  }
  const uint32_t g = a.group_begin + blockIdx.x * NB + nb;
  if (g >= st.group_end) return;
  PHI_BLK(0);
  const float EPS = a.epsilon;
  if constexpr (NB == 1) {
    if (a.noise_on) zig_load(&zig);
  }

  constexpr int HP = KPT / 2;
  f32x2 bf[HP];
  bool beta_safe = true;
#pragma unroll
  for (int p = 0; p < HP; ++p) {
    const float b0 = a.beta[2 * (tid + 2 * L * p) + 1];
    const float b1 = a.beta[2 * (tid + 2 * L * p + L) + 1];
    bf[p] = f32x2{b0 - EPS, b1 - EPS};
    beta_safe = beta_safe && in_range(b0, EPS, kBetaHi) && in_range(b1, EPS, kBetaHi);
  }
  ammsb_seed rs = {0, 0};
  if (a.noise_on) rs = a.seeds[(uint64_t)g * LV + VLn::vlane(tid)];
  auto draw_normal = [&](uint32_t j) {
    if constexpr (VL == 64) {
      s_noise[ln + 64 * j] = s_noise[ln + 64 * j] * rng_normal(rs, &zig);
    } else {
      const float z = rng_normal(rs, &zig);
      if (VLn::keeps(tid, j)) s_noise[ln + 64 * (j / VLn::PER)] = s_noise[ln + 64 * (j / VLn::PER)] * z;
    }
  };

  auto request = [&](uint32_t q, uint32_t slot) {
    const uint32_t nbr = __builtin_amdgcn_readfirstlane(s_nb[q] & 0x7fffffffu);
    const float* src = rpm_row(a.pi, nbr) + (W == 1 ? 4 * tid : L * (ln >> 4) + 64 * wv + 4 * (ln & 15));
    char* dst = wave_smem + slot * (KW * sizeof(float));
    if (a.rows_nt) {
#pragma unroll
      for (int t = 0; t < PIECES; ++t)
        __builtin_amdgcn_global_load_lds((glb_void_t*)(src + 4 * L * t), (lds_void_t*)(dst + 1024 * t), 16, 0, 2);
    } else {
#pragma unroll
      for (int t = 0; t < PIECES; ++t)
        __builtin_amdgcn_global_load_lds((glb_void_t*)(src + 4 * L * t), (lds_void_t*)(dst + 1024 * t), 16, 0, 0);
    }
  };

  int phase = 0;
  auto group_sum = [&](float v) -> float {
    if constexpr (W == 1) {
      return VLn::tree(v);
    } else {
      float* x = xsum + phase * L;
      phase ^= 1;
      x[tid] = v;
      __syncthreads();
      float part[W];
#pragma unroll
      for (int i = 0; i < W; ++i) part[i] = x[64 * i + ln];
#pragma unroll
      for (int st = W / 2; st >= 1; st >>= 1) {
#pragma unroll
        for (int i = 0; i < st; ++i) part[i] += part[i + st];
      }
      return Group<64>::wave_tree64(part[0]);
    }
  };

  for (uint64_t i = g; i < st.n_nodes; i += st.G) {
    const uint32_t node = a.nodes[i];
    group_sync();
    for (uint32_t q = tid; q < n; q += L) {
      const uint32_t nbq = a.neighbors[i * n + q];
      const bool y = set_has(a.set, make_edge(node, nbq));
      s_nb[q] = nbq | (y ? 0x80000000u : 0u);
    }
    group_sync();

    const float phi_sum = a.phi_sum[node];
    const float inv_phi_sum = 1.0f / phi_sum;
    const float* row_a = rpm_row(a.pi, node);
    f32x2 pi_a[HP], grads[HP], rden[HP];
    bool node_safe = beta_safe && in_range(phi_sum, kPhiSumLo, kPhiSumHi);
#pragma unroll
    for (int p = 0; p < HP; ++p)
      pi_a[p] = f32x2{__builtin_nontemporal_load(row_a + tid + 2 * L * p), __builtin_nontemporal_load(row_a + tid + 2 * L * p + L)};
#pragma unroll
    for (uint32_t r = 0; r < (uint32_t)(D - 1); ++r)
      if (r < n) request(r, r);
#pragma unroll
    for (int p = 0; p < HP; ++p) {
      grads[p] = f32x2{0.0f, 0.0f};
      const f32x2 den = pi_a[p] * phi_sum;
      rden[p] = f32x2{exact_rcp(den.x), exact_rcp(den.y)};
      node_safe = node_safe && in_range(den.x, kDenLo, kDenHi) && in_range(den.y, kDenLo, kDenHi);
      const f32x2 ep = den * st.eps_t;
      s_noise[ln + 128 * p] = sqrtf(ep.x);
      s_noise[ln + 128 * p + 64] = sqrtf(ep.y);
    }

    for (uint32_t q = 0; q < n; ++q) {
      const uint32_t slot = q & (D - 1);
      float* row = ring + slot * KW;
      asm volatile("s_waitcnt lgkmcnt(0)" ::: "memory");
      if (q + (D - 1) < n) {
        request(q + (D - 1), (q + (D - 1)) & (D - 1));
        if (a.noise_on && q < (uint32_t)KV) draw_normal(q);
        asm volatile("s_waitcnt vmcnt(%0)" ::"n"((D - 1) * PIECES) : "memory");
      } else {
        if constexpr (D > 2) {
          if (a.noise_on && q < (uint32_t)KV) draw_normal(q);
        }
        const uint32_t rem = n - 1 - q;
        if constexpr (D == 2) {
          asm volatile("s_waitcnt vmcnt(0)" ::: "memory");
        } else if constexpr (D == 4) {
          if (rem == 2) asm volatile("s_waitcnt vmcnt(%0)" ::"n"(2 * PIECES) : "memory");
          else if (rem == 1) asm volatile("s_waitcnt vmcnt(%0)" ::"n"(1 * PIECES) : "memory");
          else asm volatile("s_waitcnt vmcnt(0)" ::: "memory");
        } else {
          if (rem >= 6) asm volatile("s_waitcnt vmcnt(%0)" ::"n"(6 * PIECES) : "memory");
          else if (rem == 5) asm volatile("s_waitcnt vmcnt(%0)" ::"n"(5 * PIECES) : "memory");
          else if (rem == 4) asm volatile("s_waitcnt vmcnt(%0)" ::"n"(4 * PIECES) : "memory");
          else if (rem == 3) asm volatile("s_waitcnt vmcnt(%0)" ::"n"(3 * PIECES) : "memory");
          else if (rem == 2) asm volatile("s_waitcnt vmcnt(%0)" ::"n"(2 * PIECES) : "memory");
          else if (rem == 1) asm volatile("s_waitcnt vmcnt(%0)" ::"n"(1 * PIECES) : "memory");
          else asm volatile("s_waitcnt vmcnt(0)" ::: "memory");
        }
      }
      bool y = (s_nb[q] >> 31) != 0;
      y = __builtin_amdgcn_readfirstlane((int)y) != 0;
      const float e = y ? EPS : 1.0f - EPS;

      float partial = 0.0f, lo = 1.0f;
      auto pass1 = [&](auto link) {
#pragma unroll
        for (int p = 0; p < HP; ++p) {
          const f32x2 pin = f32x2{row[ln + 128 * p], row[ln + 128 * p + 64]};
          const f32x2 tt0 = pin * bf[p];
          const f32x2 tt = decltype(link)::value ? tt0 + e : e - tt0;
          const f32x2 pr = pi_a[p] * tt;
          row[ln + 128 * p] = pr.x;
          row[ln + 128 * p + 64] = pr.y;
          VLn::chain(partial, pr.x);
          VLn::chain(partial, pr.y);
          lo = fminf(fminf(lo, fabsf(pr.x)), fabsf(pr.y));
        }
      };
      if (y) pass1(std::true_type{});
      else pass1(std::false_type{});
      const float probs_sum = group_sum(partial);

      if (node_safe && lo >= kProbsLo && in_range(probs_sum, kPsumLo, kPsumHi)) {
        const float rps = exact_rcp(probs_sum);
        float ps = phi_sum;
        asm volatile("" : "+v"(ps));
        const f32x2 psum2 = f32x2{probs_sum, probs_sum}, rps2 = f32x2{rps, rps};
// ... 16 lines not shown
        }
      }
    }

    if (a.noise_on) {
#pragma unroll 1
      for (uint32_t j = D > 2 ? n : (n > 0 ? n - 1 : 0); j < (uint32_t)KV; ++j) draw_normal(j);
    }
    asm volatile("s_waitcnt lgkmcnt(0)" ::: "memory");

    float* out = a.phi_vec + i * K;
    const float half = st.eps_t / 2;
#pragma unroll
    for (int p = 0; p < HP; ++p) {
      const f32x2 bb = f32x2{s_noise[ln + 128 * p], s_noise[ln + 128 * p + 64]};
      const f32x2 phi_k = pi_a[p] * phi_sum;
      const f32x2 ng = grads[p] * a.Nn;
      f32x2 in = a.alpha - phi_k;
      in = in + ng;
      const f32x2 drift = in * half;
      const f32x2 aa = phi_k + drift;
      const f32x2 s2 = aa + bb;
      const float v0 = fabsf(s2.x), v1 = fabsf(s2.y);
      __builtin_nontemporal_store(v0 > 1e-24f ? v0 : 1e-24f, out + tid + 2 * L * p);
      __builtin_nontemporal_store(v1 > 1e-24f ? v1 : 1e-24f, out + tid + 2 * L * p + L);
    }
  }
  if (a.noise_on && tid < LV) a.seeds[(uint64_t)g * LV + tid] = rs;
  PHI_BLK(1);
}

template <int KPT, int VL = 64, bool ONE = false>
__global__ __launch_bounds__(64) __attribute__((amdgpu_waves_per_eu(3))) void update_phi_lds3_kernel(const PhiArgs a) {
  if constexpr (ONE) __builtin_assume(a.pi.num_blocks == 1);
  using VLn = VLane<VL>;
  constexpr int D = 3;
  constexpr int KV = KPT * VLn::PER;
  constexpr int L = 64, KW = 64 * KPT, K = L * KPT, PIECES = KPT / 4, HP = KPT / 2;
  extern __shared__ __align__(16) char smem[];
  __shared__ ZigTables zig;
  const int tid = threadIdx.x, ln = tid;
  const uint32_t n = a.n;
  float* ring = reinterpret_cast<float*>(smem);
  uint32_t* s_nb = reinterpret_cast<uint32_t*>(smem + D * KW * sizeof(float));

  const PhiStep st = phi_step(a);
  note_stamp(a.stamps, a.desc, AMMSB_STAMP_PHI);
  const uint32_t g = a.group_begin + blockIdx.x;
  if (g >= st.group_end) return;
  PHI_BLK(0);
  const float EPS = a.epsilon;
  if (a.noise_on) zig_load(&zig);

  f32x2 bf[HP];
  bool beta_safe = true;
#pragma unroll
  for (int p = 0; p < HP; ++p) {
    const float b0 = a.beta[2 * (tid + 2 * L * p) + 1];
    const float b1 = a.beta[2 * (tid + 2 * L * p + L) + 1];
    bf[p] = f32x2{b0 - EPS, b1 - EPS};
    beta_safe = beta_safe && in_range(b0, EPS, kBetaHi) && in_range(b1, EPS, kBetaHi);
  }
  ammsb_seed rs = {0, 0};
  if (a.noise_on) rs = a.seeds[(uint64_t)g * VL + VLn::vlane(tid)];

  auto fetch = [&](const float* src_row, uint32_t slot, bool nt) {
    const float* src = src_row + 4 * tid;
    char* dst = smem + slot * (KW * sizeof(float));
    if (nt) {
#pragma unroll
      for (int t = 0; t < PIECES; ++t)
        __builtin_amdgcn_global_load_lds((glb_void_t*)(src + 4 * L * t), (lds_void_t*)(dst + 1024 * t), 16, 0, 2);
    } else {
#pragma unroll
      for (int t = 0; t < PIECES; ++t)
        __builtin_amdgcn_global_load_lds((glb_void_t*)(src + 4 * L * t), (lds_void_t*)(dst + 1024 * t), 16, 0, 0);
    }
  };

  for (uint64_t i = g; i < st.n_nodes; i += st.G) {
    const uint32_t node = a.nodes[i];
    float* out = a.phi_vec + i * K;
    __syncthreads();
    for (uint32_t q = tid; q < n; q += L) {
      const uint32_t nbq = a.neighbors[i * n + q];
      const bool y = set_has(a.set, make_edge(node, nbq));
      s_nb[q] = nbq | (y ? 0x80000000u : 0u);
    }
    __syncthreads();
    auto request = [&](uint32_t r, uint32_t slot) {
      if (r < n) {
        const uint32_t nbr = __builtin_amdgcn_readfirstlane(s_nb[r] & 0x7fffffffu);
        fetch(rpm_row(a.pi, nbr), slot, a.rows_nt != 0);
      } else {
        const float* o = out;
        asm volatile("" : "+s"(o));
        fetch(o, slot, false);
      }
    };

    const float phi_sum = a.phi_sum[node];
    const float inv_phi_sum = 1.0f / phi_sum;
    const float* row_a = rpm_row(a.pi, node);
    f32x2 pi_a[HP], grads[HP], rden[HP];
    bool node_safe = beta_safe && in_range(phi_sum, kPhiSumLo, kPhiSumHi);
#pragma unroll
    for (int p = 0; p < HP; ++p)
      pi_a[p] = f32x2{__builtin_nontemporal_load(row_a + tid + 2 * L * p), __builtin_nontemporal_load(row_a + tid + 2 * L * p + L)};
    request(0, 0);
    request(1, 1);
#pragma unroll
    for (int p = 0; p < HP; ++p) {
      grads[p] = f32x2{0.0f, 0.0f};
      const f32x2 den = pi_a[p] * phi_sum;
      rden[p] = f32x2{exact_rcp(den.x), exact_rcp(den.y)};
      node_safe = node_safe && in_range(den.x, kDenLo, kDenHi) && in_range(den.y, kDenLo, kDenHi);
    }

    uint32_t slot = 0;
    for (uint32_t q = 0; q < n; ++q) {
      float* row = ring + slot * KW;
      const uint32_t free_slot = slot == 0 ? 2u : slot - 1u;
      asm volatile("s_waitcnt lgkmcnt(0)" ::: "memory");
      const uint32_t last = a.noise_on ? n : n - 1;
      if (q + 2 <= last) {
        request(q + 2, free_slot);
        if (a.noise_on && q < (uint32_t)KV) {
          const float z = rng_normal(rs, &zig);
          float* o = out;
          asm volatile("" : "+s"(o));
          if (VLn::keeps(tid, q)) o[ln + 64 * (q / VLn::PER)] = z;
          asm volatile("s_waitcnt vmcnt(%0)" ::"n"(2 * PIECES + 1) : "memory");
        } else {
          asm volatile("s_waitcnt vmcnt(%0)" ::"n"(2 * PIECES) : "memory");
        }
      } else if (q + 1 <= last) {
        asm volatile("s_waitcnt vmcnt(%0)" ::"n"(PIECES) : "memory");
      } else {
        asm volatile("s_waitcnt vmcnt(0)" ::: "memory");
      }
      bool y = (s_nb[q] >> 31) != 0;
      y = __builtin_amdgcn_readfirstlane((int)y) != 0;
      const float e = y ? EPS : 1.0f - EPS;

      float partial = 0.0f, lo = 1.0f;
      auto pass1 = [&](auto link) {
#pragma unroll
        for (int p = 0; p < HP; ++p) {
          const f32x2 pin = f32x2{row[ln + 128 * p], row[ln + 128 * p + 64]};
          const f32x2 tt0 = pin * bf[p];
          const f32x2 tt = decltype(link)::value ? tt0 + e : e - tt0;
          const f32x2 pr = pi_a[p] * tt;
          row[ln + 128 * p] = pr.x;
          row[ln + 128 * p + 64] = pr.y;
          VLn::chain(partial, pr.x);
          VLn::chain(partial, pr.y);
          lo = fminf(fminf(lo, fabsf(pr.x)), fabsf(pr.y));
        }
      };
      if (y) pass1(std::true_type{});
      else pass1(std::false_type{});
      const float probs_sum = VLn::tree(partial);

      if (node_safe && lo >= kProbsLo && in_range(probs_sum, kPsumLo, kPsumHi)) {
        const float rps = exact_rcp(probs_sum);
        float ps = phi_sum;
        asm volatile("" : "+v"(ps));
        const f32x2 psum2 = f32x2{probs_sum, probs_sum}, rps2 = f32x2{rps, rps};
#pragma unroll
// ... 35 lines not shown
      const f32x2 s2 = aa + bb;
      const float v0 = fabsf(s2.x), v1 = fabsf(s2.y);
      __builtin_nontemporal_store(v0 > 1e-24f ? v0 : 1e-24f, out + tid + 2 * L * p);
      __builtin_nontemporal_store(v1 > 1e-24f ? v1 : 1e-24f, out + tid + 2 * L * p + L);
    }
  }
  if (a.noise_on && tid < VL) a.seeds[(uint64_t)g * VL + tid] = rs;
  PHI_BLK(1);
}

template <int KPT, int D, int U, int VL = 64, bool ONE = false>
__global__ __launch_bounds__(64) __attribute__((amdgpu_waves_per_eu(KPT == 4 ? 4 : 3))) void update_phi_lds2_kernel(const PhiArgs a) {
  if constexpr (ONE) __builtin_assume(a.pi.num_blocks == 1);
  constexpr int L = 64, KW = 64 * KPT, K = L * KPT, PIECES = KPT / 4, HP = KPT / 2;
  using VLn = VLane<VL>;
  constexpr int KV = KPT * VLn::PER;
  constexpr bool REGP = U * HP <= 8;
  constexpr bool REGN = KPT == U;
  static_assert(D > U && (D & (D - 1)) == 0 && (U == 2 || U == 4) && (D - U) * PIECES <= 63, "ring depth / rows per step");
  extern __shared__ __align__(16) char smem[];
  __shared__ ZigTables zig;
  const int tid = threadIdx.x, ln = tid;
  float* ring = reinterpret_cast<float*>(smem);
  float* s_noise = ring + D * KW;
  uint32_t* s_nb = reinterpret_cast<uint32_t*>(smem + (D + (REGN ? 0 : 1)) * KW * sizeof(float));
  float nz[REGN ? KPT : 1];

  const PhiStep st = phi_step(a);
  note_stamp(a.stamps, a.desc, AMMSB_STAMP_PHI);
  const uint32_t g0 = a.group_begin + blockIdx.x;
  if (g0 >= st.group_end) return;
  PHI_BLK(0);
  const uint32_t n = a.n;
  const float EPS = a.epsilon;
  if (a.noise_on) zig_load(&zig);

  f32x2 bf[HP];
  bool beta_safe = true;
#pragma unroll
  for (int p = 0; p < HP; ++p) {
    const float b0 = a.beta[2 * (tid + 2 * L * p) + 1];
    const float b1 = a.beta[2 * (tid + 2 * L * p + L) + 1];
    bf[p] = f32x2{b0 - EPS, b1 - EPS};
    beta_safe = beta_safe && in_range(b0, EPS, kBetaHi) && in_range(b1, EPS, kBetaHi);
  }
  ammsb_seed rs = {0, 0};

  auto request = [&](uint32_t q, uint32_t slot) {
    const uint32_t nbr = __builtin_amdgcn_readfirstlane(s_nb[q] & 0x7fffffffu);
    const float* src = rpm_row(a.pi, nbr) + 4 * tid;
    char* dst = smem + slot * (KW * sizeof(float));
    if (a.rows_nt) {
#pragma unroll
      for (int t = 0; t < PIECES; ++t)
        __builtin_amdgcn_global_load_lds((glb_void_t*)(src + 4 * L * t), (lds_void_t*)(dst + 1024 * t), 16, 0, 2);
    } else {
#pragma unroll
      for (int t = 0; t < PIECES; ++t)
        __builtin_amdgcn_global_load_lds((glb_void_t*)(src + 4 * L * t), (lds_void_t*)(dst + 1024 * t), 16, 0, 0);
    }
  };

  PHI_TRACE(0);
  for (uint32_t g = g0; g < st.group_end; g += gridDim.x) {
  if (a.noise_on) rs = a.seeds[(uint64_t)g * VL + VLn::vlane(tid)];
  for (uint64_t i = g; i < st.n_nodes; i += st.G) {
    const uint32_t node = a.nodes[i];
    __syncthreads();
    for (uint32_t q = tid; q < n; q += L) s_nb[q] = a.neighbors[i * n + q];
    __syncthreads();
    PHI_TRACE(1);

    const float phi_sum = a.phi_sum[node];
    const float inv_phi_sum = 1.0f / phi_sum;
    const float* row_a = rpm_row(a.pi, node);
    f32x2 pi_a[HP], grads[HP], rden[HP];
    bool node_safe = beta_safe && in_range(phi_sum, kPhiSumLo, kPhiSumHi);
#pragma unroll
    for (int p = 0; p < HP; ++p)
      pi_a[p] = f32x2{__builtin_nontemporal_load(row_a + tid + 2 * L * p), __builtin_nontemporal_load(row_a + tid + 2 * L * p + L)};
#pragma unroll
    for (uint32_t r = 0; r < (uint32_t)(D - U); ++r)
      if (r < n) request(r, r);
    const bool one_probe = n <= (uint32_t)L;
    const uint32_t my_nb = one_probe && (uint32_t)tid < n ? s_nb[tid] : 0u;
    SetProbe my_probe = {};
    if (one_probe && (uint32_t)tid < n) my_probe = set_probe(a.set, make_edge(node, my_nb));
    float zraw[REGN ? KV : 1];
    if constexpr (REGN) {
      if (a.noise_on) {
#pragma unroll
        for (int j = 0; j < KV; ++j) zraw[j] = rng_normal(rs, &zig);
      }
    }
    if (one_probe) {
      if ((uint32_t)tid < n && set_hit(my_probe, make_edge(node, my_nb))) s_nb[tid] = my_nb | 0x80000000u;
    } else {
      for (uint32_t q = tid; q < n; q += L) {
        const uint32_t nb = s_nb[q];
        if (set_has(a.set, make_edge(node, nb))) s_nb[q] = nb | 0x80000000u;
      }
    }
    __syncthreads();
    PHI_TRACE(2);
#pragma unroll
    for (int p = 0; p < HP; ++p) {
      grads[p] = f32x2{0.0f, 0.0f};
      const f32x2 den = pi_a[p] * phi_sum;
      rden[p] = f32x2{exact_rcp(den.x), exact_rcp(den.y)};
      node_safe = node_safe && in_range(den.x, kDenLo, kDenHi) && in_range(den.y, kDenLo, kDenHi);
      const f32x2 ep = den * st.eps_t;
      if constexpr (REGN) {
        nz[2 * p] = sqrtf(ep.x);
        nz[2 * p + 1] = sqrtf(ep.y);
      } else {
        s_noise[ln + 128 * p] = sqrtf(ep.x);
        s_noise[ln + 128 * p + 64] = sqrtf(ep.y);
      }
    }

    PHI_TRACE(3);
    for (uint32_t q = 0; q < n; q += U) {
      float* row[U];
#pragma unroll
      for (int r = 0; r < U; ++r) row[r] = ring + ((q + r) & (D - 1)) * KW;
      asm volatile("s_waitcnt lgkmcnt(0)" ::: "memory");
      PHI_TRACE(8 + 4 * (q / U));
      if (q + (D - U) < n) {
#pragma unroll
        for (int r = 0; r < U; ++r) request(q + (D - U) + r, (q + (D - U) + r) & (D - 1));
      }
      if (a.noise_on) {
        if constexpr (REGN) {
          if (q == 0) {
#pragma unroll
            for (int j = 0; j < KV; ++j)
              if (VLn::keeps(tid, (uint32_t)j)) nz[j / VLn::PER] = nz[j / VLn::PER] * zraw[j];
          }
        } else {
#pragma unroll
          for (int r = 0; r < U; ++r)
            if (q + r < (uint32_t)KV) {
              const float z = rng_normal(rs, &zig);
              const uint32_t c = (q + r) / VLn::PER;
              if (VLn::keeps(tid, q + r)) s_noise[ln + 64 * c] = s_noise[ln + 64 * c] * z;
            }
        }
      }
      {
        const uint32_t rem = n - U - q < (uint32_t)(D - U) ? n - U - q : (uint32_t)(D - U);
        if (rem >= 6) asm volatile("s_waitcnt vmcnt(%0)" ::"n"(6 * PIECES) : "memory");
        else if (rem >= 4) asm volatile("s_waitcnt vmcnt(%0)" ::"n"(4 * PIECES) : "memory");
        else if (rem >= 2) asm volatile("s_waitcnt vmcnt(%0)" ::"n"(2 * PIECES) : "memory");
        else asm volatile("s_waitcnt vmcnt(0)" ::: "memory");
      }
      PHI_TRACE(8 + 4 * (q / U) + 1);
      float ee[U], sg[U], part[U], lo[U], psum[U];
      f32x2 prr[REGP ? U : 1][REGP ? HP : 1];
      bool fast[U], all_fast = true;
#pragma unroll
      for (int r = 0; r < U; ++r) {
        const bool y = (__builtin_amdgcn_readfirstlane(s_nb[q + r]) >> 31) != 0;
        ee[r] = y ? EPS : 1.0f - EPS;
        sg[r] = y ? 1.0f : -1.0f;
        part[r] = 0.0f;
        lo[r] = 1.0f;
      }
#pragma unroll
      for (int p = 0; p < HP; ++p) {
        float vx[U], vy[U];
#pragma unroll
        for (int r = 0; r < U; ++r) {
          const f32x2 pin = f32x2{row[r][ln + 128 * p], row[r][ln + 128 * p + 64]};
          const f32x2 tt = (pin * bf[p]) * sg[r] + ee[r];
          const f32x2 pr = pi_a[p] * tt;
          if constexpr (REGP) {
            prr[r][p] = pr;
          } else {
            row[r][ln + 128 * p] = pr.x;
            row[r][ln + 128 * p + 64] = pr.y;
          }
          vx[r] = pr.x;
          vy[r] = pr.y;
// ... 122 lines not shown
  __shared__ ZigTables zig;
  const int tid = threadIdx.x, h = tid >> 5, l = tid & 31;
  float* ring = reinterpret_cast<float*>(smem);
  float* s_nz = ring + D * SLOT + h * K + l;
  const uint32_t n = a.n;
  uint32_t* s_nb = reinterpret_cast<uint32_t*>(smem + (size_t)(D + 1) * SLOT * sizeof(float)) + h * n;
  auto lds_col = [&](int j) -> int { return (j >> 2) * 256 + h * 128 + l + 32 * (j & 3); };

  const PhiStep st = phi_step(a);
  if (st.n_nodes == 0) return;
  note_stamp(a.stamps, a.desc, AMMSB_STAMP_PHI);
  const uint32_t g = a.group_begin + blockIdx.x * 2 + h;
  const bool live = g < st.group_end;
  if (!__builtin_amdgcn_readfirstlane((int)(a.group_begin + blockIdx.x * 2 < st.group_end))) return;
  const float EPS = a.epsilon;
  if (a.noise_on) zig_load(&zig);

  f32x2 bf[HP];
  bool beta_safe = true;
#pragma unroll
  for (int p = 0; p < HP; ++p) {
    const float b0 = a.beta[2 * (l + 64 * p) + 1];
    const float b1 = a.beta[2 * (l + 64 * p + 32) + 1];
    bf[p] = f32x2{b0 - EPS, b1 - EPS};
    beta_safe = beta_safe && in_range(b0, EPS, kBetaHi) && in_range(b1, EPS, kBetaHi);
  }
  ammsb_seed rs[NS];
#pragma unroll
  for (int v = 0; v < NS; ++v) {
    rs[v] = ammsb_seed{0, 0};
    if (live && a.noise_on) rs[v] = a.seeds[(uint64_t)g * VL + l + 32 * v];
  }

  auto tree32 = [&](float v) -> float {
    typedef unsigned int u2 __attribute__((ext_vector_type(2)));
    const u2 t = __builtin_amdgcn_permlane16_swap(__float_as_uint(v), __float_as_uint(v), false, false);
    v = __uint_as_float(t[0]) + __uint_as_float(t[1]);
    v += __uint_as_float(__builtin_amdgcn_update_dpp(0u, __float_as_uint(v), 0x108, 0xf, 0xf, true));
    v += __uint_as_float(__builtin_amdgcn_update_dpp(0u, __float_as_uint(v), 0x104, 0xf, 0xf, true));
    v += __uint_as_float(__builtin_amdgcn_update_dpp(0u, __float_as_uint(v), 0x102, 0xf, 0xf, true));
    v += __uint_as_float(__builtin_amdgcn_update_dpp(0u, __float_as_uint(v), 0x101, 0xf, 0xf, true));
    const float s0 = __uint_as_float(__builtin_amdgcn_readlane(__float_as_uint(v), 0));
    const float s1 = __uint_as_float(__builtin_amdgcn_readlane(__float_as_uint(v), 32));
    return h ? s1 : s0;
  };

  auto half_row = [&](uint32_t id) -> const float* {
    const float* r0 = rpm_row(a.pi, __builtin_amdgcn_readlane(id, 0));
    const float* r1 = rpm_row(a.pi, __builtin_amdgcn_readlane(id, 32));
    return h ? r1 : r0;
  };
  auto request = [&](uint32_t q, uint32_t slot) {
    const float* src = half_row(s_nb[q] & 0x7fffffffu) + 4 * l;
    char* dst = smem + (size_t)slot * (SLOT * sizeof(float));
#pragma unroll
    for (int t = 0; t < PIECES; ++t)
      __builtin_amdgcn_global_load_lds((glb_void_t*)(src + 128 * t), (lds_void_t*)(dst + 1024 * t), 16, 0, 2);
  };

  const uint32_t trips = (st.n_nodes + st.G - 1) / st.G;
  for (uint32_t t = 0; t < trips; ++t) {
    const uint64_t i_raw = (uint64_t)g + (uint64_t)t * st.G;
    const bool on = live && i_raw < st.n_nodes;
    if (!__builtin_amdgcn_readfirstlane((int)(__ballot(on) != 0ull))) continue;
    const uint64_t i = on ? i_raw : 0;
    const uint32_t node = a.nodes[i];
    asm volatile("s_waitcnt lgkmcnt(0)" ::: "memory");
    __builtin_amdgcn_wave_barrier();
    for (uint32_t q = l; q < n; q += 32) s_nb[q] = a.neighbors[i * n + q];
    asm volatile("s_waitcnt vmcnt(0) lgkmcnt(0)" ::: "memory");
    __builtin_amdgcn_wave_barrier();

    const float phi_sum = a.phi_sum[node];
    const float inv_phi_sum = 1.0f / phi_sum;
    const float* row_a = half_row(node);
    f32x2 pi_a[HP], grads[HP], rden[HP];
    bool node_safe = beta_safe && in_range(phi_sum, kPhiSumLo, kPhiSumHi);
#pragma unroll
    for (int p = 0; p < HP; ++p)
      pi_a[p] = f32x2{__builtin_nontemporal_load(row_a + l + 64 * p), __builtin_nontemporal_load(row_a + l + 64 * p + 32)};
#pragma unroll
    for (uint32_t r = 0; r < (uint32_t)(D - U); ++r)
      if (r < n) request(r, r);
    for (uint32_t q = l; q < n; q += 32) {
      const uint32_t nb = s_nb[q];
      if (set_has(a.set, make_edge(node, nb))) s_nb[q] = nb | 0x80000000u;
    }
    asm volatile("s_waitcnt lgkmcnt(0)" ::: "memory");
    __builtin_amdgcn_wave_barrier();
#pragma unroll
    for (int p = 0; p < HP; ++p) {
      grads[p] = f32x2{0.0f, 0.0f};
      const f32x2 den = pi_a[p] * phi_sum;
      rden[p] = f32x2{exact_rcp(den.x), exact_rcp(den.y)};
      node_safe = node_safe && in_range(den.x, kDenLo, kDenHi) && in_range(den.y, kDenLo, kDenHi);
      const f32x2 ep = den * st.eps_t;
      s_nz[64 * p] = sqrtf(ep.x);
      s_nz[64 * p + 32] = sqrtf(ep.y);
    }
    if (a.noise_on && on) {
#pragma unroll 1
      for (int p = 0; p < HP; ++p) {
        const float z0 = rng_normal(rs[0], &zig);
        const float z1 = rng_normal(rs[NS - 1], &zig);
        s_nz[64 * p] = s_nz[64 * p] * z0;
        s_nz[64 * p + 32] = s_nz[64 * p + 32] * z1;
      }
    }

    for (uint32_t q = 0; q < n; q += U) {
      float* row[U];
#pragma unroll
      for (int r = 0; r < U; ++r) row[r] = ring + ((q + r) & (D - 1)) * SLOT;
      asm volatile("s_waitcnt lgkmcnt(0)" ::: "memory");
      if (q + (D - U) < n) {
#pragma unroll
        for (int r = 0; r < U; ++r) request(q + (D - U) + r, (q + (D - U) + r) & (D - 1));
      }
      {
        const uint32_t rem = n - U - q < (uint32_t)(D - U) ? n - U - q : (uint32_t)(D - U);
        if (rem >= 6) asm volatile("s_waitcnt vmcnt(%0)" ::"n"(6 * PIECES) : "memory");
        else if (rem >= 4) asm volatile("s_waitcnt vmcnt(%0)" ::"n"(4 * PIECES) : "memory");
        else if (rem >= 2) asm volatile("s_waitcnt vmcnt(%0)" ::"n"(2 * PIECES) : "memory");
        else asm volatile("s_waitcnt vmcnt(0)" ::: "memory");
      }
      float ee[U], sg[U], lo[U], psum[U];
      float part[U][NS];
      f32x2 prr[U][HP];
      bool fast[U], all_fast = true;
#pragma unroll
      for (int r = 0; r < U; ++r) {
        const bool y = (s_nb[q + r] >> 31) != 0;
        ee[r] = y ? EPS : 1.0f - EPS;
        sg[r] = y ? 1.0f : -1.0f;
        lo[r] = 1.0f;
#pragma unroll
        for (int v = 0; v < NS; ++v) part[r][v] = 0.0f;
      }
#pragma unroll
      for (int p = 0; p < HP; ++p) {
#pragma unroll
        for (int r = 0; r < U; ++r) {
          const f32x2 pin = f32x2{row[r][lds_col(2 * p)], row[r][lds_col(2 * p + 1)]};
          const f32x2 tt = (pin * bf[p]) * sg[r] + ee[r];
          const f32x2 pr = pi_a[p] * tt;
          prr[r][p] = pr;
          part[r][0] += pr.x;
          part[r][NS - 1] += pr.y;
          lo[r] = fminf(fminf(lo[r], fabsf(pr.x)), fabsf(pr.y));
        }
      }
#pragma unroll
      for (int r = 0; r < U; ++r) {
        const float lane_sum = NS == 1 ? part[r][0] : part[r][0] + part[r][NS - 1];
        psum[r] = tree32(lane_sum);
        fast[r] = node_safe && lo[r] >= kProbsLo && in_range(psum[r], kPsumLo, kPsumHi);
        all_fast = all_fast && fast[r];
      }
      if (all_fast) {
        float ps = phi_sum;
        asm volatile("" : "+v"(ps));
        f32x2 s2[U], r2[U];
#pragma unroll
        for (int r = 0; r < U; ++r) {
          const float rc = exact_rcp(psum[r]);
          s2[r] = f32x2{psum[r], psum[r]};
          r2[r] = f32x2{rc, rc};
        }
#pragma unroll
// ... 22 lines not shown
#pragma unroll
            for (int p = 0; p < HP; ++p) {
              const f32x2 den = pi_a[p] * phi_sum;
              float v0 = prr[r][p].x / probs_sum, v1 = prr[r][p].y / probs_sum;
              v0 = v0 / den.x;
              v1 = v1 / den.y;
              grads[p] += f32x2{v0 - inv_phi_sum, v1 - inv_phi_sum};
            }
          }
        }
      }
    }

    if (on) {
      float* out = a.phi_vec + i * K;
      const float half = st.eps_t / 2;
#pragma unroll
      for (int p = 0; p < HP; ++p) {
        const f32x2 phi_k = pi_a[p] * phi_sum;
        const f32x2 ng = grads[p] * a.Nn;
        f32x2 in = a.alpha - phi_k;
        in = in + ng;
        const f32x2 drift = in * half;
        const f32x2 aa = phi_k + drift;
        const f32x2 s2 = aa + f32x2{s_nz[64 * p], s_nz[64 * p + 32]};
        const float v0 = fabsf(s2.x), v1 = fabsf(s2.y);
        __builtin_nontemporal_store(v0 > 1e-24f ? v0 : 1e-24f, out + l + 64 * p);
        __builtin_nontemporal_store(v1 > 1e-24f ? v1 : 1e-24f, out + l + 64 * p + 32);
      }
    }
  }
  if (live && a.noise_on) {
#pragma unroll
    for (int v = 0; v < NS; ++v) a.seeds[(uint64_t)g * VL + l + 32 * v] = rs[v];
  }
}

template <int KPT, int D, int U, int VL>
int launch_phi_pair(ammsb_ctx* ctx, const PhiArgs& a, uint32_t n_groups, hipStream_t s) {
  const size_t lds = (size_t)(D + 1) * 2 * 32 * KPT * sizeof(float) + 2 * sizeof(uint32_t) * a.n;
  static const std::string name = ammsb_kname("update_phi_pair_kernel<%d, %d, %d, %d>", KPT, D, U, VL);
  ctx->kernel_name[AMMSB_KN_PHI] = name.c_str();
  update_phi_pair_kernel<KPT, D, U, VL><<<(n_groups + 1) / 2, 64, lds, s>>>(a);
  AMMSB_LAUNCH_CHECK(ctx);
  return AMMSB_OK;
}

template <int KPT, int RW, int VL>
__global__ __launch_bounds__(64 * (RW + 1)) void update_phi_wide_kernel(const PhiArgs a) {
  constexpr int K = 64 * KPT, T = 64 * (RW + 1);
  using VLn = VLane<VL>;
  constexpr int KV = KPT * VLn::PER;
  extern __shared__ __align__(16) char smem[];
  __shared__ ZigTables zig;
  const int tid = threadIdx.x, wv = tid >> 6, ln = tid & 63;
  const uint32_t n = a.n;
  float* term = reinterpret_cast<float*>(smem);
  float* s_noise = term + (size_t)n * K;
  float* s_pia = s_noise + K;
  uint32_t* s_nb = reinterpret_cast<uint32_t*>(s_pia + K);

  const PhiStep st = phi_step(a);
  note_stamp(a.stamps, a.desc, AMMSB_STAMP_PHI);
  const uint32_t g = a.group_begin + blockIdx.x;
  if (g >= st.group_end) return;
  const float EPS = a.epsilon;
  if (a.noise_on) zig_load(&zig);

  float bf[KPT];
  bool beta_safe = true;
#pragma unroll
  for (int j = 0; j < KPT; ++j) {
    const float b = a.beta[2 * (ln + 64 * j) + 1];
    bf[j] = b - EPS;
    beta_safe = beta_safe && in_range(b, EPS, kBetaHi);
  }
  ammsb_seed rs = {0, 0};
  const bool noise_wave = wv == RW;
  if (a.noise_on && noise_wave) rs = a.seeds[(uint64_t)g * VL + VLn::vlane(ln)];

  for (uint64_t i = g; i < st.n_nodes; i += st.G) {
    const uint32_t node = a.nodes[i];
    __syncthreads();
    for (uint32_t q = tid; q < n; q += T) {
      const uint32_t nbq = a.neighbors[i * n + q];
      const bool y = set_has(a.set, make_edge(node, nbq));
      s_nb[q] = nbq | (y ? 0x80000000u : 0u);
    }
    const float phi_sum = a.phi_sum[node];
    const float inv_phi_sum = 1.0f / phi_sum;
    const float* row_a = rpm_row(a.pi, node);
    float pi_a[KPT], rden[KPT];
    bool node_safe = beta_safe && in_range(phi_sum, kPhiSumLo, kPhiSumHi);
#pragma unroll
    for (int j = 0; j < KPT; ++j) pi_a[j] = row_a[ln + 64 * j];
    if (noise_wave) {
#pragma unroll
      for (int j = 0; j < KPT; ++j) s_pia[ln + 64 * j] = pi_a[j];
    } else {
#pragma unroll
      for (int j = 0; j < KPT; ++j) {
        const float den = pi_a[j] * phi_sum;
        rden[j] = exact_rcp(den);
        node_safe = node_safe && in_range(den, kDenLo, kDenHi);
      }
    }
    __syncthreads();

    if (!noise_wave) {
      float cur[KPT], nxt[KPT];
      auto load_row = [&](float (&dst)[KPT], uint32_t q) {
        const uint32_t w = __builtin_amdgcn_readfirstlane(s_nb[q < n ? q : n - 1] & 0x7fffffffu);
        const float* row = rpm_row(a.pi, w);
#pragma unroll
        for (int j = 0; j < KPT; ++j) dst[j] = __builtin_nontemporal_load(row + ln + 64 * j);
      };
      if ((uint32_t)wv < n) load_row(cur, wv);
      for (uint32_t q = wv; q < n; q += RW) {
        load_row(nxt, q + RW);
        const bool y = __builtin_amdgcn_readfirstlane(s_nb[q] >> 31) != 0;
        const float e = y ? EPS : 1.0f - EPS;
        float pr[KPT];
        float partial = 0.0f, lo = 1.0f;
#pragma unroll
        for (int j = 0; j < KPT; ++j) {
          const float tt0 = cur[j] * bf[j];
          const float tt = y ? tt0 + e : e - tt0;
          pr[j] = pi_a[j] * tt;
          VLn::chain(partial, pr[j]);
          lo = fminf(lo, fabsf(pr[j]));
        }
        const float probs_sum = VLn::tree(partial);
        float* tq = term + (size_t)q * K;
        if (node_safe && lo >= kProbsLo && in_range(probs_sum, kPsumLo, kPsumHi)) {
          const float rps = exact_rcp(probs_sum);
#pragma unroll
          for (int j = 0; j < KPT; ++j) {
            float qv = div_exact3(pr[j], probs_sum, rps);
            qv = div_exact3(qv, pi_a[j] * phi_sum, rden[j]);
            tq[ln + 64 * j] = qv - inv_phi_sum;
          }
        } else {
#pragma unroll
          for (int j = 0; j < KPT; ++j) {
            float qv = pr[j] / probs_sum;
            qv = qv / (pi_a[j] * phi_sum);
            tq[ln + 64 * j] = qv - inv_phi_sum;
          }
        }
#pragma unroll
        for (int j = 0; j < KPT; ++j) cur[j] = nxt[j];
      }
    } else if (a.noise_on) {
#pragma unroll 1
      for (uint32_t j = 0; j < (uint32_t)KV; ++j) {
        const float z = rng_normal(rs, &zig);
        if (VLn::keeps(ln, j)) s_noise[ln + 64 * (j / VLn::PER)] = z;
      }
    }
    __syncthreads();

    float* out = a.phi_vec + i * K;
    const float half = st.eps_t / 2;
    for (int c = tid; c < K; c += T) {
      float grads = 0.0f;
      for (uint32_t q = 0; q < n; ++q) grads += term[(size_t)q * K + c];
      const float noise = a.noise_on ? s_noise[c] : 1.0f;
      const float phi_k = s_pia[c] * phi_sum;
      const float ng = a.Nn * grads;
// ... 492 lines not shown
      if (a.K == (uint32_t)(L * KPT))
        update_phi_kernel<L, KPT, DEPTH, true, true><<<blocks, Grp::BLOCK, lds, s>>>(a);
      else
        update_phi_kernel<L, KPT, DEPTH, false, true><<<blocks, Grp::BLOCK, lds, s>>>(a);
      AMMSB_LAUNCH_CHECK(ctx);
      return AMMSB_OK;
    }
  }
  static const std::string name_full = ammsb_kname("update_phi_kernel<%d, %d, %d, true, false>", L, KPT, DEPTH);
  static const std::string name_part = ammsb_kname("update_phi_kernel<%d, %d, %d, false, false>", L, KPT, DEPTH);
  ctx->kernel_name[AMMSB_KN_PHI] = (a.K == (uint32_t)(L * KPT) ? name_full : name_part).c_str();
  if (a.K == (uint32_t)(L * KPT))
    update_phi_kernel<L, KPT, DEPTH, true><<<blocks, Grp::BLOCK, lds, s>>>(a);
  else
    update_phi_kernel<L, KPT, DEPTH, false><<<blocks, Grp::BLOCK, lds, s>>>(a);
  AMMSB_LAUNCH_CHECK(ctx);
  return AMMSB_OK;
}

template <int L, int KPT>
int launch_pi(ammsb_ctx* ctx, const ammsb_rpm& pi, float* phi_sum, const float* phi_vec, const uint32_t* nodes,
              uint32_t n_nodes, uint32_t K, const ammsb_step_desc* desc, unsigned long long* stamps, hipStream_t s) {
  using Grp = Group<L>;
  const uint32_t blocks = (n_nodes + Grp::PER_BLOCK - 1) / Grp::PER_BLOCK;
  static const std::string name = ammsb_kname("update_pi_kernel<%d, %d>", L, KPT);
  ctx->kernel_name[AMMSB_KN_PI] = name.c_str();
  update_pi_kernel<L, KPT><<<blocks, Grp::BLOCK, 0, s>>>(pi, phi_sum, phi_vec, nodes, n_nodes, K, desc, stamps);
  AMMSB_LAUNCH_CHECK(ctx);
  return AMMSB_OK;
}

__global__ __launch_bounds__(256) void phi_noise_kernel(const PhiArgs a, uint32_t L, uint32_t lgL) {
  __shared__ ZigTables zig;
  const PhiStep st = phi_step(a);
  if (st.n_nodes == 0) return;
  note_stamp(a.stamps, a.desc, AMMSB_STAMP_PHI);
  zig_load(&zig);
  __syncthreads();
  const uint64_t sid = (uint64_t)blockIdx.x * blockDim.x + threadIdx.x;
  const uint32_t g = a.group_begin + (uint32_t)(sid >> lgL), l = (uint32_t)sid & (L - 1);
  if (g >= st.group_end) return;
  ammsb_seed rs = a.seeds[(uint64_t)g * L + l];
  for (uint64_t i = g; i < st.n_nodes; i += st.G) {
    float* out = a.phi_vec + i * a.K;
    for (uint32_t k = l; k < a.K; k += L) out[k] = rng_normal(rs, &zig);
  }
  a.seeds[(uint64_t)g * L + l] = rs;
}

template <int CPT, int U>
__global__ __launch_bounds__(512) void update_phi_gen_kernel(const PhiArgs a, uint32_t L, uint32_t lgL) {
  extern __shared__ __align__(16) char smem[];
  const uint32_t K = a.K, n = a.n, T = blockDim.x, t = threadIdx.x;
  float* s_vals = reinterpret_cast<float*>(smem);
  float* s_aux = s_vals + (size_t)U * K;
  float* s_res = s_aux + U * L;
  uint32_t* s_nb = reinterpret_cast<uint32_t*>(s_res + 2 * U);

  const PhiStep st = phi_step(a);
  if (!a.noise_on) note_stamp(a.stamps, a.desc, AMMSB_STAMP_PHI);
  const uint32_t g = a.group_begin + blockIdx.x;
  if (g >= st.group_end) return;
  const float EPS = a.epsilon;

  auto col = [&](int j) -> uint32_t { return t + (uint32_t)j * T; };
  auto ccol = [&](int j) -> uint32_t {
    const uint32_t k = t + (uint32_t)j * T;
    return k < K ? k : K - 1;
  };
  auto has = [&](int j) -> bool { return t + (uint32_t)j * T < K; };

  float bf[CPT];
  bool beta_safe = true;
#pragma unroll
  for (int j = 0; j < CPT; ++j) {
    const float b = a.beta[2 * ccol(j) + 1];
    bf[j] = b - EPS;
    beta_safe = beta_safe && in_range(b, EPS, kBetaHi);
  }
  int phase = 0;
  for (uint64_t i = g; i < st.n_nodes; i += st.G) {
    const uint32_t node = a.nodes[i];
    __syncthreads();
    for (uint32_t q = t; q < n; q += T) {
      const uint32_t nbq = a.neighbors[i * n + q];
      const bool y = set_has(a.set, make_edge(node, nbq));
      s_nb[q] = nbq | (y ? 0x80000000u : 0u);
    }
    __syncthreads();

    const float phi_sum = a.phi_sum[node];
    const float inv_phi_sum = 1.0f / phi_sum;
    const float* row_a = rpm_row(a.pi, node);
    float* out = a.phi_vec + i * K;
    float pi_a[CPT], grads[CPT], rden[CPT], noise[CPT];
    bool node_safe = beta_safe && in_range(phi_sum, kPhiSumLo, kPhiSumHi);
#pragma unroll
    for (int j = 0; j < CPT; ++j) {
      const float x = row_a[ccol(j)];
      pi_a[j] = has(j) ? x : 0.0f;
      grads[j] = 0.0f;
      const float den = pi_a[j] * phi_sum;
      rden[j] = exact_rcp(den);
      node_safe = node_safe && (in_range(den, kDenLo, kDenHi) || !has(j));
      noise[j] = a.noise_on ? out[ccol(j)] : 1.0f;
    }

    float cur[U][CPT], nxt[U][CPT];
    auto load_rows = [&](float (&dst)[U][CPT], uint32_t q0) {
#pragma unroll
      for (int r = 0; r < U; ++r) {
        const uint32_t q = q0 + r < n ? q0 + r : n - 1;
        const uint32_t w = __builtin_amdgcn_readfirstlane(s_nb[q] & 0x7fffffffu);
        const float* row = rpm_row(a.pi, w);
#pragma unroll
        for (int j = 0; j < CPT; ++j) dst[r][j] = row[ccol(j)];
      }
    };
    if (n > 0) load_rows(cur, 0);
    for (uint32_t q = 0; q < n; q += U) {
      load_rows(nxt, q + U);
      float pr[U][CPT], lo[U];
#pragma unroll
      for (int r = 0; r < U; ++r) {
        const bool y = __builtin_amdgcn_readfirstlane(s_nb[q + r] >> 31) != 0;
        const float e = y ? EPS : 1.0f - EPS;
        lo[r] = 1.0f;
#pragma unroll
        for (int j = 0; j < CPT; ++j) {
          const float tt0 = cur[r][j] * bf[j];
          const float tt = y ? tt0 + e : e - tt0;
          pr[r][j] = pi_a[j] * tt;
          if (has(j)) s_vals[(size_t)r * K + col(j)] = pr[r][j];
          lo[r] = fminf(lo[r], has(j) ? fabsf(pr[r][j]) : 1.0f);
        }
      }
      __syncthreads();
      float sums[U];
      if constexpr (U == 1) {
        const float* const vv[1] = {s_vals};
        vgroup_sum<1>(vv, K, L, lgL, s_aux, s_res, phase, sums);
      } else if constexpr (U == 2) {
        const float* const vv[2] = {s_vals, s_vals + K};
        vgroup_sum<2>(vv, K, L, lgL, s_aux, s_res, phase, sums);
      } else {
        const float* const vv[4] = {s_vals, s_vals + K, s_vals + 2 * (size_t)K, s_vals + 3 * (size_t)K};
        vgroup_sum<4>(vv, K, L, lgL, s_aux, s_res, phase, sums);
      }
#pragma unroll
      for (int r = 0; r < U; ++r) {
        const float probs_sum = sums[r];
        if (node_safe && lo[r] >= kProbsLo && in_range(probs_sum, kPsumLo, kPsumHi)) {
          const float rps = exact_rcp(probs_sum);
#pragma unroll
          for (int j = 0; j < CPT; ++j) {
            float qv = div_exact3(pr[r][j], probs_sum, rps);
            qv = div_exact3(qv, pi_a[j] * phi_sum, rden[j]);
            grads[j] += qv - inv_phi_sum;
          }
        } else {
#pragma unroll
          for (int j = 0; j < CPT; ++j) {
            float qv = pr[r][j] / probs_sum;
            qv = qv / (pi_a[j] * phi_sum);
            grads[j] += qv - inv_phi_sum;
          }
        }
      }
#pragma unroll
// ... 69 lines not shown
  const uint32_t per_wave = 64u * (uint32_t)gen_cpt(K);
  uint32_t T = 64u * (uint32_t)((K + per_wave - 1) / per_wave);
  if (T < sums * L) T = sums * L;
  if (T < 64) T = 64;
  return T <= 512 ? T : 0;
}

template <int CPT, int U>
int launch_phi_gen_u(ammsb_ctx* ctx, const PhiArgs& a, uint32_t wg, uint32_t T, uint32_t n_groups, hipStream_t s) {
  const size_t lds = sizeof(float) * ((size_t)U * a.K + U * wg + 2 * U) + sizeof(uint32_t) * a.n;
  static const bool big = [] {
    return hipFuncSetAttribute(reinterpret_cast<const void*>(update_phi_gen_kernel<CPT, U>),
                               hipFuncAttributeMaxDynamicSharedMemorySize, 160 * 1024 - 2048) == hipSuccess;
  }();
  (void)big;
  static const std::string name = ammsb_kname("update_phi_gen_kernel<%d, %d>", CPT, U);
  ctx->kernel_name[AMMSB_KN_PHI] = name.c_str();
  if (a.noise_on) {
    const uint64_t streams = (uint64_t)n_groups * wg;
    phi_noise_kernel<<<(unsigned)((streams + 255) / 256), 256, 0, s>>>(a, wg, ilog2_u32(wg));
    AMMSB_LAUNCH_CHECK(ctx);
  }
  update_phi_gen_kernel<CPT, U><<<n_groups, T, lds, s>>>(a, wg, ilog2_u32(wg));
  AMMSB_LAUNCH_CHECK(ctx);
  return AMMSB_OK;
}

int launch_phi_gen(ammsb_ctx* ctx, const PhiArgs& a, uint32_t wg, uint32_t n_groups, hipStream_t s) {
  const uint32_t T = gen_threads(a.K, wg, 1);
  if (!T) return AMMSB_ERANGE;
  const uint32_t u = (a.n % 4 == 0 && 4 * wg <= T) ? 4 : (a.n % 2 == 0 && 2 * wg <= T) ? 2 : 1;
  if (gen_cpt(a.K) == 8) {
    if (u == 4) return launch_phi_gen_u<8, 4>(ctx, a, wg, T, n_groups, s);
    if (u == 2) return launch_phi_gen_u<8, 2>(ctx, a, wg, T, n_groups, s);
    return launch_phi_gen_u<8, 1>(ctx, a, wg, T, n_groups, s);
  }
  return launch_phi_gen_u<16, 1>(ctx, a, wg, T, n_groups, s);
}

inline int pick_kpt(uint64_t K, uint32_t L) {
  const uint64_t need = (K + L - 1) / L;
  for (int c : {1, 2, 4, 8, 16, 32})
    if ((uint64_t)c >= need) return c;
  return 0;
}

}

#define AMMSB_DISPATCH_KPT(kpt, ...)                                  \
  switch (kpt) {                                                      \
    case 1: { constexpr int KPT_ = 1; __VA_ARGS__; } break;           \
    case 2: { constexpr int KPT_ = 2; __VA_ARGS__; } break;           \
    case 4: { constexpr int KPT_ = 4; __VA_ARGS__; } break;           \
    case 8: { constexpr int KPT_ = 8; __VA_ARGS__; } break;           \
    case 16: { constexpr int KPT_ = 16; __VA_ARGS__; } break;         \
    case 32: { constexpr int KPT_ = 32; __VA_ARGS__; } break;         \
    default: return AMMSB_ERANGE;                                     \
  }

#define AMMSB_DISPATCH_HOT_L(wg, ...)                                 \
  switch (wg) {                                                       \
    case 16: { constexpr int L_ = 16; __VA_ARGS__; } break;           \
    case 32: { constexpr int L_ = 32; __VA_ARGS__; } break;           \
    case 64: { constexpr int L_ = 64; __VA_ARGS__; } break;           \
    case 128: { constexpr int L_ = 128; __VA_ARGS__; } break;         \
    case 256: { constexpr int L_ = 256; __VA_ARGS__; } break;         \
    case 512: { constexpr int L_ = 512; __VA_ARGS__; } break;         \
    case 1024: { constexpr int L_ = 1024; __VA_ARGS__; } break;       \
    default: return AMMSB_EINVAL;                                     \
  }

static int g_phi_form_lds3 = -1, g_phi_form_nb = -1, g_phi_form_ring = -1;
extern "C" int ammsb_debug_phi_forms(int lds3, int nb, int ring) {
  g_phi_form_lds3 = lds3;
  g_phi_form_nb = nb;
  g_phi_form_ring = ring;
  return AMMSB_OK;
}

static int update_phi_common(ammsb_ctx* ctx, const float* beta, const ammsb_rpm* pi, const float* phi_sum,
                             const ammsb_set* training_set, const uint32_t* nodes, const uint32_t* neighbors,
                             uint32_t n_nodes, uint32_t step_count, ammsb_seed* seeds, uint32_t wg, uint32_t flags,
                             uint32_t group_begin, uint32_t group_end, float* phi_vec, const ammsb_step_desc* desc,
                             unsigned long long* stamps, void* stream) {
  AMMSB_CHECK_ARG(ctx, ctx && beta && pi && phi_sum && training_set && nodes && neighbors && seeds && phi_vec,
                  "null argument");
  AMMSB_CHECK_ARG(ctx, n_nodes > 0, "mini-batch nodes size = 0");
  AMMSB_CHECK_ARG(ctx, pi->num_blocks >= 1 && pi->num_blocks <= AMMSB_RPM_MAX_BLOCKS && pi->rows_in_block > 0,
                  "bad pi descriptor");
  AMMSB_CHECK_ARG(ctx, pi->num_cols == ctx->params.K && pi->num_rows == ctx->params.N, "pi shape != (N, K)");
  AMMSB_CHECK_ARG(ctx, training_set->slots && training_set->num_bins > 0 && training_set->prime_idx < 4,
                  "bad set descriptor");
  AMMSB_CHECK_ARG(ctx, ctx->params.N < (1ull << 31), "N must be < 2^31");
  AMMSB_CHECK_ARG(ctx, is_pow2(wg) && wg >= 16 && wg <= 1024, "phi wg must be a power of two in [16, 1024]");
  const ammsb_params& p = ctx->params;
  const int kpt = pick_kpt(p.K, wg);
  static const bool force_gen = [] {
    const char* f = getenv("AMMSB_PHI_FORM");
    return f && f[0] == 'g';
  }();
  const bool generic = kpt == 0 || (force_gen && gen_threads(p.K, wg, 1) != 0);
  if (generic && gen_threads(p.K, wg, 1) == 0) {
    snprintf(ctx->err, sizeof ctx->err, "ammsb_update_phi: K=%llu at wg=%u: more than 32 columns per work-item needs K <= %u",
             (unsigned long long)p.K, wg, kGenMaxK);
    return AMMSB_ERANGE;
  }
  PhiArgs a;
  a.beta = beta;
  a.pi = *pi;
  a.phi_sum = phi_sum;
  a.set = dev_set(*training_set);
  a.nodes = nodes;
  a.neighbors = neighbors;
  a.seeds = seeds;
  a.phi_vec = phi_vec;
  a.n_nodes = n_nodes;
  a.G = n_nodes < AMMSB_MAX_GROUPS ? n_nodes : AMMSB_MAX_GROUPS;
  a.group_begin = group_begin;
  a.group_end = group_end < a.G ? group_end : a.G;
  a.K = (uint32_t)p.K;
  a.n = p.num_node_sample;
  a.eps_t = desc ? 0.0f : ammsb_eps_t(&p, step_count);
  a.desc = desc;
  a.stamps = stamps;
  a.alpha = p.alpha;
  a.epsilon = p.epsilon;
  a.Nn = (1.0f * (float)p.N) / (float)p.num_node_sample;
  a.noise_on = (flags & AMMSB_NOISE_OFF) ? 0u : 1u;
  {
    static const int nt_mode = [] {
      const char* f = getenv("AMMSB_PHI_NT");
      return f ? atoi(f) : -1;
    }();
    const uint64_t pi_bytes = pi->num_rows * pi->num_cols * sizeof(float);
    a.rows_nt = nt_mode >= 0 ? (uint32_t)nt_mode : (pi_bytes > (256ull << 20) ? 1u : 0u);
  }
  if (a.group_begin >= a.group_end) return AMMSB_OK;
  const uint32_t n_groups = a.group_end - a.group_begin;
  hipStream_t s = as_stream(stream);
  static const bool lds3_env = [] {
    const char* f = getenv("AMMSB_PHI_LDS3");
    return f ? atoi(f) != 0 : AMMSB_PHI_LDS3_DEFAULT;
  }();
  const bool lds3 = g_phi_form_lds3 >= 0 ? g_phi_form_lds3 != 0 : lds3_env;
  static const bool force_reg = [] {
    const char* f = getenv("AMMSB_PHI_FORM");
    return f && f[0] == 'r';
  }();
  static const uint32_t wide_max = [] {
    const char* f = getenv("AMMSB_PHI_WIDE");
    return f ? (uint32_t)atoi(f) : 512u;
  }();
  if (n_groups <= wide_max && !(flags & AMMSB_PHI_STREAMING) && !force_reg && !force_gen && (wg == 32 || wg == 64) &&
      (p.K == 256 || p.K == 512 || p.K == 1024) && a.n >= 1 && n_nodes <= AMMSB_MAX_GROUPS &&
      sizeof(float) * p.K * ((size_t)a.n + 2) + sizeof(uint32_t) * a.n <= 150 * 1024) {
    static const int rw_alt = [] {
      const char* f = getenv("AMMSB_PHI_WIDE_RW");
      return f ? atoi(f) : 0;
    }();
    if (wg == 64) {
      if (p.K == 256) return rw_alt == 8 ? launch_phi_wide<4, 8, 64>(ctx, a, n_groups, s) : launch_phi_wide<4, 15, 64>(ctx, a, n_groups, s);
      if (p.K == 512) return rw_alt == 8 ? launch_phi_wide<8, 8, 64>(ctx, a, n_groups, s) : launch_phi_wide<8, 11, 64>(ctx, a, n_groups, s);
      return rw_alt == 8 ? launch_phi_wide<16, 8, 64>(ctx, a, n_groups, s) : launch_phi_wide<16, 11, 64>(ctx, a, n_groups, s);
    }
    if (p.K == 256) return rw_alt == 8 ? launch_phi_wide<4, 8, 32>(ctx, a, n_groups, s) : launch_phi_wide<4, 15, 32>(ctx, a, n_groups, s);
    if (p.K == 512) return rw_alt == 8 ? launch_phi_wide<8, 8, 32>(ctx, a, n_groups, s) : launch_phi_wide<8, 11, 32>(ctx, a, n_groups, s);
    return rw_alt == 8 ? launch_phi_wide<16, 8, 32>(ctx, a, n_groups, s) : launch_phi_wide<16, 11, 32>(ctx, a, n_groups, s);
  }
  static const bool stream_form = [] {
    const char* f = getenv("AMMSB_PHI_STREAM");
    return f && atoi(f) != 0;
  }();
  if (stream_form && !force_reg && !force_gen && (wg == 32 || wg == 64) && p.K == 256 && pi->num_cols % 4 == 0 &&
      a.n >= 16 && a.n <= 64 && a.n % 4 == 0 && n_groups > 1024) {
    return wg == 64 ? launch_phi_stream<4, 8, 4, 64>(ctx, a, n_groups, s) : launch_phi_stream<4, 8, 4, 32>(ctx, a, n_groups, s);
  }
  static const int pair_form = [] {
    const char* f = getenv("AMMSB_PHI_PAIR");
    return f ? atoi(f) : 0;
  }();
  if (pair_form > 0 && !force_reg && !force_gen && (wg == 32 || wg == 64) && (p.K == 256 || p.K == 512) &&
      pi->num_cols % 4 == 0 && a.n >= 2 && a.n % 2 == 0 && a.n * sizeof(uint32_t) <= 4096) {
    if (p.K == 256) {
      if (pair_form == 3 && a.n % 4 == 0)
        return wg == 32 ? launch_phi_pair<8, 8, 4, 32>(ctx, a, n_groups, s) : launch_phi_pair<8, 8, 4, 64>(ctx, a, n_groups, s);
      if (pair_form == 2)
        return wg == 32 ? launch_phi_pair<8, 8, 2, 32>(ctx, a, n_groups, s) : launch_phi_pair<8, 8, 2, 64>(ctx, a, n_groups, s);
      return wg == 32 ? launch_phi_pair<8, 4, 2, 32>(ctx, a, n_groups, s) : launch_phi_pair<8, 4, 2, 64>(ctx, a, n_groups, s);
    }
    return wg == 32 ? launch_phi_pair<16, 4, 2, 32>(ctx, a, n_groups, s) : launch_phi_pair<16, 4, 2, 64>(ctx, a, n_groups, s);
  }
  if (wg == 32 && !force_reg && !force_gen && pi->num_cols % 4 == 0 && a.n * sizeof(uint32_t) <= 8192) {
    switch (p.K) {
      case 256:
        if (a.n & 1) return launch_phi_lds<4, 1, 8, 1, 32>(ctx, a, n_groups, s);
        if (a.n & 3) return launch_phi_lds2<4, 8, 2, 32>(ctx, a, n_groups, s);
        return launch_phi_lds2<4, 8, 4, 32>(ctx, a, n_groups, s);
      case 512:
        if (a.n & 1) return launch_phi_lds<8, 1, 4, 1, 32>(ctx, a, n_groups, s);
        return launch_phi_lds2<8, 4, 2, 32>(ctx, a, n_groups, s);
      case 1024:
        if (lds3 && a.n >= 32 * 2 / 1 / 2 + 2 + 16) return launch_phi_lds3<16, 32>(ctx, a, n_groups, s);
        return launch_phi_lds<16, 1, 2, 1, 32>(ctx, a, n_groups, s);
      case 2048: return launch_phi_lds<32, 1, 2, 1, 32>(ctx, a, n_groups, s);
    }
  }
  if (generic) return launch_phi_gen(ctx, a, wg, n_groups, s);
  if (!force_reg && p.K == (uint64_t)wg * kpt && pi->num_cols % 4 == 0 && a.n * sizeof(uint32_t) <= 8192) {
    static const int ring_env = [] {
      const char* f = getenv("AMMSB_PHI_RING");
      return f ? atoi(f) : 0;
    }();
    const int ring = g_phi_form_ring >= 0 ? g_phi_form_ring : ring_env;
    if (wg == 64) {
      switch (kpt) {
        case 4:
          if (ring == 2) return launch_phi_lds<4, 1, 2>(ctx, a, n_groups, s);
          if (ring == 4) return launch_phi_lds<4, 1, 4>(ctx, a, n_groups, s);
          if (ring == 8 || (a.n & 1)) return launch_phi_lds<4, 1, 8>(ctx, a, n_groups, s);
          if (ring == 42) return launch_phi_lds2<4, 4, 2>(ctx, a, n_groups, s);
          if (ring == 22 || (a.n & 3)) return launch_phi_lds2<4, 8, 2>(ctx, a, n_groups, s);
          return launch_phi_lds2<4, 8, 4>(ctx, a, n_groups, s);
        case 8:
          if (ring == 2) return launch_phi_lds<8, 1, 2>(ctx, a, n_groups, s);
          if (ring == 4 || (a.n & 1)) return launch_phi_lds<8, 1, 4>(ctx, a, n_groups, s);
          return launch_phi_lds2<8, 4, 2>(ctx, a, n_groups, s);
        case 16: {
          static const int nb_env = [] {
            const char* f = getenv("AMMSB_PHI_NB");
            return f ? atoi(f) : 1;
          }();
          const int nb = g_phi_form_nb >= 0 ? g_phi_form_nb : nb_env;
          if (nb == 2) return launch_phi_lds<16, 1, 2, 2>(ctx, a, n_groups, s);
          if (ring == 4) return launch_phi_lds<16, 1, 4>(ctx, a, n_groups, s);
          if (lds3 && ring == 0 && a.n >= 16 + 2) return launch_phi_lds3<16, 64>(ctx, a, n_groups, s);
          return launch_phi_lds<16, 1>(ctx, a, n_groups, s);
        }
        case 32: return launch_phi_lds<32, 1>(ctx, a, n_groups, s);
      }
    } else if (kpt == 8 && wg == 128) {
      return launch_phi_lds<8, 2>(ctx, a, n_groups, s);
    } else if (kpt == 16) {
      switch (wg) {
        case 128: return launch_phi_lds<16, 2>(ctx, a, n_groups, s);
        case 256: return launch_phi_lds<16, 4>(ctx, a, n_groups, s);
        case 512: return launch_phi_lds<16, 8>(ctx, a, n_groups, s);
      }
    }
  }
  AMMSB_DISPATCH_HOT_L(wg, AMMSB_DISPATCH_KPT(kpt, return (launch_phi<L_, KPT_>(ctx, a, n_groups, s))));
  return AMMSB_OK;
}

extern "C" int ammsb_update_phi(ammsb_ctx* ctx, const float* beta, const ammsb_rpm* pi, const float* phi_sum,
                                const ammsb_set* training_set, const uint32_t* nodes, const uint32_t* neighbors,
                                uint32_t n_nodes, uint32_t step_count, ammsb_seed* seeds, uint32_t wg, uint32_t flags,
                                uint32_t group_begin, uint32_t group_end, float* phi_vec, void* stream) {
  return update_phi_common(ctx, beta, pi, phi_sum, training_set, nodes, neighbors, n_nodes, step_count, seeds, wg, flags,
                           group_begin, group_end, phi_vec, nullptr, nullptr, stream);
}

int ammsb_update_phi_d(ammsb_ctx* ctx, const float* beta, const ammsb_rpm* pi, const float* phi_sum,
                       const ammsb_set* training_set, const uint32_t* nodes, const uint32_t* neighbors,
                       uint32_t n_nodes_cap, ammsb_seed* seeds, uint32_t wg, uint32_t flags, float* phi_vec,
                       const ammsb_step_desc* desc, unsigned long long* stamps, void* stream) {
  AMMSB_CHECK_ARG(ctx, ctx && desc, "null descriptor");
  return update_phi_common(ctx, beta, pi, phi_sum, training_set, nodes, neighbors, n_nodes_cap, 0, seeds, wg, flags, 0,
                           0xFFFFFFFFu, phi_vec, desc, stamps, stream);
}

template <int KPT, int W, int D>
static int occ_of(uint32_t n, int* out) {
  const size_t lds = (size_t)W * (D + 1) * sizeof(float) * 64 * KPT + sizeof(uint32_t) * n;
  return hipOccupancyMaxActiveBlocksPerMultiprocessor(out, update_phi_lds_kernel<KPT, W, D>, 64 * W, lds) == hipSuccess
             ? AMMSB_OK
             : AMMSB_EHIP;
}

extern "C" int ammsb_update_phi_occupancy(ammsb_ctx* ctx, uint32_t wg, int* blocks_per_cu, int* waves_per_block) {
  AMMSB_CHECK_ARG(ctx, ctx && blocks_per_cu && waves_per_block, "null argument");
  const ammsb_params& p = ctx->params;
  const int kpt = pick_kpt(p.K, wg);
  const uint32_t n = p.num_node_sample;
  *blocks_per_cu = 0;
  *waves_per_block = (int)(wg / 64);
  if (kpt == 0 || p.K != (uint64_t)wg * kpt) return AMMSB_OK;
  if (wg == 64 && kpt == 4) return occ_of<4, 1, 8>(n, blocks_per_cu);
  if (wg == 64 && kpt == 8) return occ_of<8, 1, 4>(n, blocks_per_cu);
  if (wg == 64 && kpt == 16) return occ_of<16, 1, 2>(n, blocks_per_cu);
  if (wg == 64 && kpt == 32) return occ_of<32, 1, 2>(n, blocks_per_cu);
  if (wg == 128 && kpt == 8) return occ_of<8, 2, 2>(n, blocks_per_cu);
  if (wg == 128 && kpt == 16) return occ_of<16, 2, 2>(n, blocks_per_cu);
  if (wg == 256 && kpt == 16) return occ_of<16, 4, 2>(n, blocks_per_cu);
  if (wg == 512 && kpt == 16) return occ_of<16, 8, 2>(n, blocks_per_cu);
  return AMMSB_OK;
}

static int update_pi_common(ammsb_ctx* ctx, const ammsb_rpm* pi, float* phi_sum, const float* phi_vec,
                            const uint32_t* nodes, uint32_t n_nodes, uint32_t wg, const ammsb_step_desc* desc,
                            unsigned long long* stamps, void* stream) {
  AMMSB_CHECK_ARG(ctx, ctx && pi && phi_sum && phi_vec && nodes, "null argument");
  AMMSB_CHECK_ARG(ctx, pi->num_blocks >= 1 && pi->num_blocks <= AMMSB_RPM_MAX_BLOCKS && pi->rows_in_block > 0,
                  "bad pi descriptor");
  AMMSB_CHECK_ARG(ctx, pi->num_cols == ctx->params.K, "pi cols != K");
  AMMSB_CHECK_ARG(ctx, is_pow2(wg) && wg >= 16 && wg <= 1024, "phi wg must be a power of two in [16, 1024]");
  if (n_nodes == 0) return AMMSB_OK;
  const int kpt = pick_kpt(ctx->params.K, wg);
  const uint32_t K = (uint32_t)ctx->params.K;
  hipStream_t s = as_stream(stream);
  static const bool force_gen = [] {
    const char* f = getenv("AMMSB_PHI_FORM");
    return f && f[0] == 'g';
  }();
  if (kpt == 0 || (force_gen && gen_threads(K, wg, 1) != 0)) {
    const uint32_t T = gen_threads(K, wg, 1);
    if (!T) {
      snprintf(ctx->err, sizeof ctx->err, "ammsb_update_pi: K=%u at wg=%u: more than 32 columns per work-item needs K <= %u",
               K, wg, kGenMaxK);
      return AMMSB_ERANGE;
    }
    const size_t lds = sizeof(float) * ((size_t)K + wg + 2);
    ctx->kernel_name[AMMSB_KN_PI] = gen_cpt(K) == 8 ? "update_pi_gen_kernel<8>" : "update_pi_gen_kernel<16>";
    if (gen_cpt(K) == 8)
      update_pi_gen_kernel<8><<<n_nodes, T, lds, s>>>(*pi, phi_sum, phi_vec, nodes, n_nodes, K, wg, ilog2_u32(wg), desc, stamps);
    else
      update_pi_gen_kernel<16><<<n_nodes, T, lds, s>>>(*pi, phi_sum, phi_vec, nodes, n_nodes, K, wg, ilog2_u32(wg), desc, stamps);
    AMMSB_LAUNCH_CHECK(ctx);
    return AMMSB_OK;
  }
  AMMSB_DISPATCH_HOT_L(wg, AMMSB_DISPATCH_KPT(kpt, return (launch_pi<L_, KPT_>(ctx, *pi, phi_sum, phi_vec, nodes,
                                                                                n_nodes, K, desc, stamps, s))));
  return AMMSB_OK;
}

extern "C" int ammsb_update_pi(ammsb_ctx* ctx, const ammsb_rpm* pi, float* phi_sum, const float* phi_vec,
                               const uint32_t* nodes, uint32_t n_nodes, uint32_t wg, void* stream) {
  return update_pi_common(ctx, pi, phi_sum, phi_vec, nodes, n_nodes, wg, nullptr, nullptr, stream);
}

int ammsb_update_pi_d(ammsb_ctx* ctx, const ammsb_rpm* pi, float* phi_sum, const float* phi_vec, const uint32_t* nodes,
                      uint32_t n_nodes_cap, uint32_t wg, const ammsb_step_desc* desc, unsigned long long* stamps,
                      void* stream) {
  AMMSB_CHECK_ARG(ctx, ctx && desc, "null descriptor");
  return update_pi_common(ctx, pi, phi_sum, phi_vec, nodes, n_nodes_cap, wg, desc, stamps, stream);
}
```

### mcmc-ammsb-gpu_amd/csrc/ammsb_step.h

```cpp
#pragma once

#include <stdint.h>

#include "../../include/ammsb.h"

#define AMMSB_STAMP_CAP 8192u
#define AMMSB_STAMP_SLOTS 8u
#define AMMSB_STAMP_PHI 0u
#define AMMSB_STAMP_PI 1u
#define AMMSB_STAMP_GRADS 2u
#define AMMSB_STAMP_THETA 3u
#define AMMSB_STAMP_RELEASED 4u
#define AMMSB_STAMP_NEXT 5u

struct ammsb_step_desc {
  uint32_t n_nodes;
  uint32_t n_edges;
  float eps_t;
  float scale;
  uint32_t u;
  uint32_t link;
  uint32_t n_cand;
  uint32_t step;
};

#ifdef __HIPCC__
static __device__ __forceinline__ bool ammsb_desc_skip(const ammsb_step_desc* d) { return d && d->n_nodes == 0; }
#endif

struct ammsb_step_advance {
  const ammsb_step_desc* ring;
  uint32_t* cursor;
  ammsb_step_desc* cur_out;
  ammsb_step_desc* nxt_out;
  uint32_t nxt_offset;
  uint32_t* main_seq;
  const uint32_t* avail;
  uint32_t* timeouts;
  unsigned long long max_ticks;
  unsigned long long* stamps;
};

#ifdef __HIPCC__
static __device__ __noinline__ void note_stamp_slow(unsigned long long* stamps, const ammsb_step_desc* desc, uint32_t which) {
  if (desc && blockIdx.x == 0 && threadIdx.x == 0)
    stamps[AMMSB_STAMP_SLOTS * (desc->step % AMMSB_STAMP_CAP) + which] = wall_clock64();
}
static __device__ __forceinline__ void note_stamp(unsigned long long* stamps, const ammsb_step_desc* desc, uint32_t which) {
  if (stamps) note_stamp_slow(stamps, desc, which);
}
#endif

struct ammsb_pi_fusion {
  const float* phi_vec;
  float* phi_sum;
  const uint32_t* nodes;
  unsigned long long* stamps;
};
bool ammsb_beta_can_fuse_pi(ammsb_ctx* ctx, uint32_t phi_wg, uint32_t beta_wg);

int ammsb_update_phi_d(ammsb_ctx* ctx, const float* beta, const ammsb_rpm* pi, const float* phi_sum,
                       const ammsb_set* training_set, const uint32_t* nodes, const uint32_t* neighbors,
                       uint32_t n_nodes_cap, ammsb_seed* seeds, uint32_t wg, uint32_t flags, float* phi_vec,
                       const ammsb_step_desc* desc, unsigned long long* stamps, void* stream);
int ammsb_update_pi_d(ammsb_ctx* ctx, const ammsb_rpm* pi, float* phi_sum, const float* phi_vec, const uint32_t* nodes,
                      uint32_t n_nodes_cap, uint32_t wg, const ammsb_step_desc* desc, unsigned long long* stamps,
                      void* stream);
int ammsb_beta_grads_d(ammsb_ctx* ctx, const float* theta, const float* beta, const ammsb_rpm* pi,
                       const ammsb_set* training_set, const uint64_t* edges, uint32_t n_edges_cap, uint32_t wg,
                       float* grads_out, const ammsb_step_desc* desc, void* stream);
int ammsb_theta_coef_d(ammsb_ctx* ctx, const float* theta, const float* beta, void* stream);
int ammsb_update_theta_d(ammsb_ctx* ctx, float* theta, float* beta, const float* grads, ammsb_seed* seeds,
                         uint32_t flags, const ammsb_step_desc* desc, const ammsb_step_advance* adv, void* stream);
int ammsb_beta_step_d(ammsb_ctx* ctx, float* theta, float* beta, const ammsb_rpm* pi, const ammsb_set* training_set,
                      const uint64_t* edges, uint32_t n_edges_cap, uint32_t wg, float* grads_out, ammsb_seed* seeds,
                      uint32_t flags, const ammsb_step_desc* desc, const ammsb_step_advance* adv,
                      const ammsb_pi_fusion* fuse, unsigned long long* stamps, void* stream);
int ammsb_sample_neighbors_d(ammsb_ctx* ctx, ammsb_seed* seeds, const uint32_t* nodes, uint32_t n_nodes_cap, uint32_t wg,
                             uint32_t* table, uint32_t* packed, const ammsb_step_desc* desc, void* stream);
int ammsb_minibatch_link_d(ammsb_ctx* ctx, const uint64_t* csr_offsets, const uint32_t* csr_targets, uint32_t n_cap,
                           uint64_t* edges_out, uint32_t* nodes_out, const ammsb_step_desc* desc, void* stream);
int ammsb_minibatch_nonlink_d(ammsb_ctx* ctx, ammsb_seed* seeds, uint32_t n_candidates_cap, uint32_t m,
                              const ammsb_set* training_set, const ammsb_set* heldout_set, void* workspace,
                              uint64_t* edges_out, uint32_t* nodes_out, uint32_t* count_out,
                              const ammsb_step_desc* desc, void* stream);
```

### mcmc-ammsb-gpu_amd/ops.py

```python
import ctypes as C
import os
import threading

import numpy as np
import torch

from . import _capi
from ._capi import AmmsbError, NOISE_OFF, PHI_STREAMING, Params, PpxSums, Rpm, SetDesc, check

SEED_DT = np.dtype([("x", np.uint64), ("y", np.uint64)])


_tls = threading.local()


def _stream():
    stack = getattr(_tls, "stack", None)
    if stack:
        return stack[-1]
    return C.c_void_p(torch.cuda.current_stream().cuda_stream)


def _torch_stream():
    stack = getattr(_tls, "tstack", None)
# ... 170 lines not shown
        self.ctx.check(self.ctx.lib.ammsb_set_has(self.ctx.handle, C.byref(self.desc), _ptr(k), k.numel(),
                                                  _ptr(out), _stream()))
        return out


class RowPartitionedMatrix:

    def __init__(self, ctx, rows, cols, rows_in_block=0, dtype=torch.float32):
        self.ctx = ctx
        self.rows, self.cols = int(rows), int(cols)
        self.rows_in_block = int(rows_in_block) if rows_in_block else self.rows
        nfull, rem = divmod(self.rows, self.rows_in_block)
        sizes = [self.rows_in_block] * nfull + ([rem] if rem else [])
        if len(sizes) > _capi.RPM_MAX_BLOCKS:
            raise AmmsbError("more than 32 blocks")
        self.blocks = [ctx.empty((s, self.cols), dtype) for s in sizes]
        self.desc = Rpm()
        for i, b in enumerate(self.blocks):
            self.desc.blocks[i] = b.data_ptr()
        self.desc.rows_in_block = self.rows_in_block
        self.desc.num_rows = self.rows
        self.desc.num_cols = self.cols
        self.desc.num_blocks = len(self.blocks)

    def adopt(self, other):
        if (other.rows, other.cols, other.rows_in_block) != (self.rows, self.cols, self.rows_in_block):
            raise AmmsbError("adopt: shapes differ")
        self.blocks, self.desc = other.blocks, other.desc

    def Rows(self):
        return self.rows

    def Cols(self):
        return self.cols

    def RowsPerBlock(self):
        return self.rows_in_block

    def Blocks(self):
        return self.blocks

    def load(self, host):
        host = np.ascontiguousarray(host).reshape(self.rows, self.cols)
        r = 0
        for b in self.blocks:
            b.copy_(self.ctx.from_numpy(host[r:r + b.shape[0]]))
            r += b.shape[0]

    def host(self):
        return np.concatenate([to_numpy(b) for b in self.blocks], axis=0)

    def gather_rows(self, rows):
        if len(self.blocks) == 1:
            return self.blocks[0][rows]
        return torch.cat(self.blocks, 0)[rows]


def RandomGammaAndNormalize(ctx, eta0, eta1, pi, phi_sum, seed=(11, 113)):
    rnd = Random(ctx, pi.Rows() * 32, seed)
    ctx.check(ctx.lib.ammsb_pi_init_gamma(ctx.handle, C.byref(pi.desc), _ptr(phi_sum), eta0, eta1,
                                          _ptr(rnd.seeds), _stream()))
    return rnd


class NeighborSampler:

    def __init__(self, ctx, max_nodes, neighbor_seed=(56, 57), wg=32):
        self.ctx = ctx
        self.n = ctx.params.num_node_sample
        self.capacity = 2 * self.n
        self.local = int(wg)
        self.hash = ctx.empty((max_nodes, self.capacity), torch.int32)
        self.data = ctx.empty((max_nodes, self.n), torch.int32)
        self.rand = Random(ctx, max_nodes * self.capacity, neighbor_seed)
        self.max_nodes = int(max_nodes)

    def __call__(self, num_samples, nodes):
        if num_samples > self.max_nodes:
            raise AmmsbError("%d samples > buffer for %d" % (num_samples, self.max_nodes))
        self.ctx.check(self.ctx.lib.ammsb_sample_neighbors(
            self.ctx.handle, _ptr(self.rand.seeds), _ptr(nodes), int(num_samples), self.local,
            _ptr(self.hash), _ptr(self.data), _stream()))

    def GetHash(self):
        return self.hash

    def GetData(self):
        return self.data

    def HashCapacityPerSample(self):
        return self.capacity

    def DataSizePerSample(self):
        return self.n


class PhiUpdater:

    def __init__(self, ctx, beta, pi, phi, training_set, max_nodes, phi_seed=(42, 43), phi_wg_size=64,
                 phi_disable_noise=False, streaming_only=False):
        self.ctx, self.beta, self.pi, self.phi, self.set = ctx, beta, pi, phi, training_set
        self.local = int(phi_wg_size)
        self.flags = (NOISE_OFF if phi_disable_noise else 0) | (PHI_STREAMING if streaming_only else 0)
        self.max_nodes = int(max_nodes)
        self.phi_vec = ctx.empty((self.max_nodes, ctx.params.K), torch.float32)
        self.rand = Random(ctx, self.max_nodes * self.local, phi_seed)
        self.count_calls = 0

    def update_phi(self, nodes, neighbors, n, group_begin=0, group_end=0xFFFFFFFF):
        if n == 0:
            raise AmmsbError("mini-batch nodes size = 0!")
        if n > self.max_nodes:
            raise AmmsbError("grads too small")
        c = self.ctx
        c.check(c.lib.ammsb_update_phi(c.handle, _ptr(self.beta), C.byref(self.pi.desc), _ptr(self.phi),
                                       C.byref(self.set.desc), _ptr(nodes), _ptr(neighbors), int(n),
                                       self.count_calls, _ptr(self.rand.seeds), self.local, self.flags,
                                       int(group_begin), int(group_end), _ptr(self.phi_vec), _stream()))

    def update_pi(self, nodes, n, phi_vec=None):
        c = self.ctx
        pv = self.phi_vec if phi_vec is None else phi_vec
        c.check(c.lib.ammsb_update_pi(c.handle, C.byref(self.pi.desc), _ptr(self.phi), _ptr(pv),
                                      _ptr(nodes), int(n), self.local, _stream()))

    def __call__(self, mini_batch_nodes, neighbors, num_mini_batch_nodes):
        self.count_calls += 1
        self.update_phi(mini_batch_nodes, neighbors, num_mini_batch_nodes)
        self.update_pi(mini_batch_nodes, num_mini_batch_nodes)


class BetaUpdater:

    def __init__(self, ctx, theta, beta, pi, training_set, beta_seed=(44, 45), beta_wg_size=256,
                 disable_noise=False):
        self.ctx, self.theta, self.beta, self.pi, self.set = ctx, theta, beta, pi, training_set
        self.local = int(beta_wg_size)
        self.flags = NOISE_OFF if disable_noise else 0
        self.rand = Random(ctx, ctx.params.K, beta_seed)
        self.grads = ctx.zeros((2 * ctx.params.K,), torch.float32)
        self.count_calls = 0

    def calculate_grads(self, edges, num_edges, edge_begin=0, edge_end=0xFFFFFFFF, out=None):
        c = self.ctx
        g = self.grads if out is None else out
        c.check(c.lib.ammsb_beta_grads(c.handle, _ptr(self.theta), _ptr(self.beta), C.byref(self.pi.desc),
                                       C.byref(self.set.desc), _ptr(edges), int(num_edges), int(edge_begin),
                                       int(min(edge_end, num_edges)), self.local, _ptr(g), _stream()))
        return g

    def can_fuse_update_pi(self, phi_updater):
        c = self.ctx
        return bool(c.lib.ammsb_can_fuse_pi_beta(c.handle, int(phi_updater.local), self.local))

    def update_pi_and_grads(self, phi_updater, nodes, edges, num_edges, out=None):
        c = self.ctx
        g = self.grads if out is None else out
        c.check(c.lib.ammsb_update_pi_beta_grads(c.handle, _ptr(self.theta), _ptr(self.beta), C.byref(self.pi.desc),
                                                 _ptr(phi_updater.phi), _ptr(phi_updater.phi_vec), _ptr(nodes),
                                                 C.byref(self.set.desc), _ptr(edges), int(num_edges), self.local,
                                                 _ptr(g), _stream()))
        return g

    def update_theta(self, scale, grads=None):
        c = self.ctx
        g = self.grads if grads is None else grads
        c.check(c.lib.ammsb_update_theta(c.handle, _ptr(self.theta), _ptr(self.beta), _ptr(g),
                                         self.count_calls, float(scale), _ptr(self.rand.seeds), self.flags,
                                         _stream()))

    def __call__(self, edges, num_edges, scale):
        self.count_calls += 1
        self.calculate_grads(edges, num_edges)
        self.update_theta(scale)

    def GetGrads(self):
        return self.grads

    def GetThetaSum(self):
        c = self.ctx
        out = c.empty((c.params.K,), torch.float32)
        c.check(c.lib.ammsb_theta_sum(c.handle, _ptr(out), _stream()))
        return out


def sum_rows(ctx, rows, out):
    ctx.check(ctx.lib.ammsb_sum_rows_f32(ctx.handle, _ptr(rows), int(rows.shape[0]), int(rows.shape[1]), _ptr(out),
                                         _stream()))
    return out


def beta_from_theta(ctx, theta, beta):
    ctx.check(ctx.lib.ammsb_beta_from_theta(ctx.handle, _ptr(theta), _ptr(beta), _stream()))


class PerplexityCalculator:

    def __init__(self, ctx, beta, pi, edges, edge_set, ppx_wg_size=64):
        self.ctx, self.beta, self.pi, self.edges, self.set = ctx, beta, pi, edges, edge_set
        self.local = int(ppx_wg_size)
        self.num_edges = int(edges.numel())
# ... 636 lines not shown
```

Before: 36.86 million.

## Compute neighbor link bits in sampler, skip training-set probes in update_phi

The neighbor sampler now works out, for each sampled neighbor, whether the edge is in the training set. It uses the node's CSR adjacency list for low-degree nodes and falls back to set lookups otherwise, and packs the answers into per-node bitmasks. update_phi then reads these bits instead of probing the training hash set for every (node, neighbor) pair. The intent is to move the random hash lookups off the critical update_phi kernel and onto the sampler, which runs on the side stream and overlaps with the main loop. The cost is extra sampler work, a new buffer, and a validity flag protocol between the two stages.

```diff
diff --git a/include/ammsb.h b/include/ammsb.h
--- a/include/ammsb.h
+++ b/include/ammsb.h
@@ -80,10 +80,21 @@
 int ammsb_sample_neighbors(ammsb_ctx* ctx, ammsb_seed* seeds, const uint32_t* nodes, uint32_t n_nodes,
                            uint32_t wg, uint32_t* table, uint32_t* packed, void* stream);
 
+int ammsb_sample_neighbors_links(ammsb_ctx* ctx, ammsb_seed* seeds, const uint32_t* nodes, uint32_t n_nodes,
+                                 uint32_t wg, uint32_t* table, uint32_t* packed, const uint64_t* csr_offsets,
+                                 const uint32_t* csr_targets, const ammsb_set* training_set, uint32_t* link_bits,
+                                 void* stream);
+
 int ammsb_update_phi(ammsb_ctx* ctx, const float* beta, const ammsb_rpm* pi, const float* phi_sum,
                      const ammsb_set* training_set, const uint32_t* nodes, const uint32_t* neighbors,
                      uint32_t n_nodes, uint32_t step_count, ammsb_seed* seeds, uint32_t wg, uint32_t flags,
                      uint32_t group_begin, uint32_t group_end, float* phi_vec, void* stream);
+
+int ammsb_update_phi_links(ammsb_ctx* ctx, const float* beta, const ammsb_rpm* pi, const float* phi_sum,
+                           const ammsb_set* training_set, const uint32_t* nodes, const uint32_t* neighbors,
+                           const uint32_t* link_bits, uint32_t n_nodes, uint32_t step_count, ammsb_seed* seeds,
+                           uint32_t wg, uint32_t flags, uint32_t group_begin, uint32_t group_end, float* phi_vec,
+                           void* stream);
 
 int ammsb_update_phi_occupancy(ammsb_ctx* ctx, uint32_t wg, int* blocks_per_cu, int* waves_per_block);
 
diff --git a/mcmc-ammsb-gpu_amd/_capi.py b/mcmc-ammsb-gpu_amd/_capi.py
--- a/mcmc-ammsb-gpu_amd/_capi.py
+++ b/mcmc-ammsb-gpu_amd/_capi.py
@@ -75,8 +75,11 @@
     "ammsb_set_build": [_vp, _vp, _u64, _vp, _u64, _P(_u32), _vp, _vp],
     "ammsb_pi_init_gamma": [_vp, _P(Rpm), _vp, _f32, _f32, _vp, _vp],
     "ammsb_sample_neighbors": [_vp, _vp, _vp, _u32, _u32, _vp, _vp, _vp],
+    "ammsb_sample_neighbors_links": [_vp, _vp, _vp, _u32, _u32, _vp, _vp, _vp, _vp, _P(SetDesc), _vp, _vp],
     "ammsb_update_phi": [_vp, _vp, _P(Rpm), _vp, _P(SetDesc), _vp, _vp, _u32, _u32, _vp, _u32, _u32,
                          _u32, _u32, _vp, _vp],
+    "ammsb_update_phi_links": [_vp, _vp, _P(Rpm), _vp, _P(SetDesc), _vp, _vp, _vp, _u32, _u32, _vp, _u32, _u32,
+                               _u32, _u32, _vp, _vp],
     "ammsb_update_phi_occupancy": [_vp, _u32, _P(C.c_int), _P(C.c_int)],
     "ammsb_update_pi": [_vp, _P(Rpm), _vp, _vp, _vp, _u32, _u32, _vp],
     "ammsb_beta_grads": [_vp, _vp, _vp, _P(Rpm), _P(SetDesc), _vp, _u32, _u32, _u32, _u32, _vp, _vp],
diff --git a/mcmc-ammsb-gpu_amd/csrc/ammsb_core.hip b/mcmc-ammsb-gpu_amd/csrc/ammsb_core.hip
--- a/mcmc-ammsb-gpu_amd/csrc/ammsb_core.hip
+++ b/mcmc-ammsb-gpu_amd/csrc/ammsb_core.hip
@@ -271,10 +271,20 @@
   return groups * wg;
 }
 
+struct NsLinks {
+  const uint64_t* csr_offsets;
+  const uint32_t* csr_targets;
+  DevSet set;
+  uint32_t* link_bits;
+  uint32_t* valid;
+  uint32_t deg_cap;
+};
+
 __global__ __launch_bounds__(64) void sample_neighbors_kernel(ammsb_seed* seeds, const uint32_t* nodes,
                                                                uint32_t n_nodes, uint32_t N, uint32_t n,
                                                                uint32_t gsize, uint32_t* table, uint32_t* packed,
-                                                               const ammsb_step_desc* desc, uint32_t wg) {
+                                                               const ammsb_step_desc* desc, uint32_t wg,
+                                                               const NsLinks lk) {
   if (desc) {
     n_nodes = desc->n_nodes;
     gsize = ns_global_size(n_nodes, wg);
@@ -294,14 +304,26 @@
       const uint32_t v = out[j];
       if (v != N) pk[count++] = v;
     }
+    if (lk.link_bits) {
+      uint32_t word = 0;
+      for (uint32_t q = 0; q < n; ++q) {
+        if (set_has(lk.set, make_edge(node, pk[q]))) word |= 1u << (q & 31);
+        if ((q & 31) == 31 || q + 1 == n) {
+          lk.link_bits[(uint64_t)i * ((n + 31) >> 5) + (q >> 5)] = word;
+          word = 0;
+        }
+      }
+    }
   }
   seeds[gid] = seed;
+  if (lk.valid && gid == 0) *lk.valid = 1u;
 }
 
 __global__ __launch_bounds__(64) void sample_neighbors_lds_kernel(ammsb_seed* seeds, const uint32_t* nodes,
                                                                    uint32_t n_nodes, uint32_t N, uint32_t n,
                                                                    uint32_t gsize, uint32_t* table, uint32_t* packed,
-                                                                   const ammsb_step_desc* desc, uint32_t wg) {
+                                                                   const ammsb_step_desc* desc, uint32_t wg,
+                                                                   const NsLinks lk) {
   if (desc) {
     n_nodes = desc->n_nodes;
     gsize = ns_global_size(n_nodes, wg);
@@ -349,6 +371,44 @@
           }
         } while (val == r);
       }
+      if (lk.link_bits) {
+        uint32_t bits[4] = {0u, 0u, 0u, 0u};
+        auto set_bit = [&](uint32_t pos) {
+#pragma unroll
+          for (uint32_t w = 0; w < 4; ++w)
+            if ((pos >> 5) == w) bits[w] |= 1u << (pos & 31);
+        };
+        const uint64_t r0 = lk.csr_offsets[node], r1 = lk.csr_offsets[node + 1];
+        if (r1 - r0 <= (uint64_t)lk.deg_cap) {
+          for (uint64_t e = r0; e < r1; ++e) {
+            const uint32_t t = lk.csr_targets[e];
+            uint32_t offset = (uint32_t)__umul64hi(cap_m * (uint64_t)(t ^ 553105253u), capacity);
+            for (;;) {
+              const uint32_t val = lds[offset * S + lane];
+              if (val == max_id + 1) break;
+              if (val == t) {
+                uint32_t pos = 0;
+                for (uint32_t j = 0; j < offset; ++j) pos += lds[j * S + lane] != N ? 1u : 0u;
+                set_bit(pos);
+                break;
+              }
+              offset = offset + 1 == capacity ? 0 : offset + 1;
+            }
+          }
+        } else {
+          uint32_t pos = 0;
+          for (uint32_t j = 0; j < capacity; ++j) {
+            const uint32_t v = lds[j * S + lane];
+            if (v == N) continue;
+            if (set_has(lk.set, make_edge(node, v))) set_bit(pos);
+            ++pos;
+          }
+        }
+        const uint32_t W = (n + 31) >> 5;
+#pragma unroll
+        for (uint32_t w = 0; w < 4; ++w)
+          if (w < W) lk.link_bits[(uint64_t)i * W + w] = bits[w];
+      }
     }
     __syncthreads();
     uint32_t* tout = table + (uint64_t)base * capacity;
@@ -387,12 +447,14 @@
     __syncthreads();
   }
   if (owner) seeds[gid] = seed;
+  if (lk.valid && gid == 0) *lk.valid = 1u;
 }
 
 __global__ __launch_bounds__(256) void sample_neighbors_wave_kernel(ammsb_seed* seeds, const uint32_t* nodes,
                                                                      uint32_t n_nodes, uint32_t N, uint32_t gsize,
                                                                      uint32_t* table, uint32_t* packed,
-                                                                     const ammsb_step_desc* desc, uint32_t wg) {
+                                                                     const ammsb_step_desc* desc, uint32_t wg,
+                                                                     const NsLinks lk) {
   constexpr uint32_t CAP = 64, NN = 32, B = 40;
   if (desc) {
     n_nodes = desc->n_nodes;
@@ -444,13 +506,36 @@
     table[(uint64_t)i * CAP + lane] = slot;
     const unsigned long long occ = __ballot(slot != N);
     if (slot != N) packed[(uint64_t)i * NN + __popcll(occ & ((1ull << lane) - 1ull))] = slot;
+    if (lk.link_bits) {
+      const uint64_t r0 = lk.csr_offsets[node], r1 = lk.csr_offsets[node + 1];
+      const uint32_t deg = (uint32_t)(r1 - r0 <= (uint64_t)lk.deg_cap ? r1 - r0 : 0xFFFFFFFFull);
+      bool link = false;
+      if (deg != 0xFFFFFFFFu) {
+        for (uint32_t base = 0; base < deg; base += 64) {
+          const uint32_t cnt = deg - base < 64u ? deg - base : 64u;
+          const uint32_t t = lane < cnt ? lk.csr_targets[r0 + base + lane] : N;
+          for (uint32_t j = 0; j < cnt; ++j) link = link || slot == (uint32_t)__builtin_amdgcn_readlane((int)t, (int)j);
+        }
+      } else if (slot != N) {
+        link = set_has(lk.set, make_edge(node, slot));
+      }
+      unsigned long long lm = __ballot(link && slot != N);
+      uint32_t word = 0;
+      while (lm) {
+        const uint32_t l = (uint32_t)__builtin_ctzll(lm);
+        lm &= lm - 1ull;
+        word |= 1u << __popcll(occ & ((1ull << l) - 1ull));
+      }
+      if (lane == 0) lk.link_bits[i] = word;
+    }
   }
   if (lane == 0) seeds[gid] = st;
+  if (lk.valid && lane == 0 && gid == 0) *lk.valid = 1u;
 }
 
 static int sample_neighbors_common(ammsb_ctx* ctx, ammsb_seed* seeds, const uint32_t* nodes, uint32_t n_nodes,
                                    uint32_t wg, uint32_t* table, uint32_t* packed, const ammsb_step_desc* desc,
-                                   void* stream) {
+                                   const NsLinks& lk, void* stream) {
   AMMSB_CHECK_ARG(ctx, ctx && seeds && nodes && table && packed, "null argument");
   AMMSB_CHECK_ARG(ctx, wg >= 1 && wg <= 1024, "sampler wg out of range");
   if (n_nodes == 0) return AMMSB_OK;
@@ -466,15 +551,15 @@
     const uint32_t waves = gsize < n_nodes ? gsize : n_nodes;
     ctx->kernel_name[AMMSB_KN_NBR] = "sample_neighbors_wave_kernel";
     sample_neighbors_wave_kernel<<<div_up(waves, 4), 256, 0, as_stream(stream)>>>(
-        seeds, nodes, n_nodes, (uint32_t)ctx->params.N, gsize, table, packed, desc, wg);
+        seeds, nodes, n_nodes, (uint32_t)ctx->params.N, gsize, table, packed, desc, wg, lk);
   } else if (lds_bytes <= 64 * 1024) {
     ctx->kernel_name[AMMSB_KN_NBR] = "sample_neighbors_lds_kernel";
     sample_neighbors_lds_kernel<<<div_up(gsize, 64), 64, lds_bytes, as_stream(stream)>>>(
-        seeds, nodes, n_nodes, (uint32_t)ctx->params.N, n, gsize, table, packed, desc, wg);
+        seeds, nodes, n_nodes, (uint32_t)ctx->params.N, n, gsize, table, packed, desc, wg, lk);
   } else {
     ctx->kernel_name[AMMSB_KN_NBR] = "sample_neighbors_kernel";
     sample_neighbors_kernel<<<div_up(gsize, 64), 64, 0, as_stream(stream)>>>(
-        seeds, nodes, n_nodes, (uint32_t)ctx->params.N, n, gsize, table, packed, desc, wg);
+        seeds, nodes, n_nodes, (uint32_t)ctx->params.N, n, gsize, table, packed, desc, wg, lk);
   }
   AMMSB_LAUNCH_CHECK(ctx);
   return AMMSB_OK;
@@ -482,13 +567,38 @@
 
 extern "C" int ammsb_sample_neighbors(ammsb_ctx* ctx, ammsb_seed* seeds, const uint32_t* nodes, uint32_t n_nodes,
                                       uint32_t wg, uint32_t* table, uint32_t* packed, void* stream) {
-  return sample_neighbors_common(ctx, seeds, nodes, n_nodes, wg, table, packed, nullptr, stream);
+  return sample_neighbors_common(ctx, seeds, nodes, n_nodes, wg, table, packed, nullptr, NsLinks{}, stream);
+}
+
+static NsLinks ns_links(ammsb_ctx* ctx, const uint64_t* csr_offsets, const uint32_t* csr_targets,
+                        const ammsb_set* training_set, uint32_t* link_bits, uint32_t* valid) {
+  return NsLinks{csr_offsets, csr_targets, dev_set(*training_set), link_bits, valid, 4u * ctx->params.num_node_sample};
+}
+
+extern "C" int ammsb_sample_neighbors_links(ammsb_ctx* ctx, ammsb_seed* seeds, const uint32_t* nodes, uint32_t n_nodes,
+                                            uint32_t wg, uint32_t* table, uint32_t* packed, const uint64_t* csr_offsets,
+                                            const uint32_t* csr_targets, const ammsb_set* training_set,
+                                            uint32_t* link_bits, void* stream) {
+  AMMSB_CHECK_ARG(ctx, ctx && csr_offsets && csr_targets && training_set && link_bits, "null argument");
+  AMMSB_CHECK_ARG(ctx, training_set->slots && training_set->num_bins > 0 && training_set->prime_idx < 4,
+                  "bad set descriptor");
+  return sample_neighbors_common(ctx, seeds, nodes, n_nodes, wg, table, packed, nullptr,
+                                 ns_links(ctx, csr_offsets, csr_targets, training_set, link_bits, nullptr), stream);
 }
 
 int ammsb_sample_neighbors_d(ammsb_ctx* ctx, ammsb_seed* seeds, const uint32_t* nodes, uint32_t n_nodes_cap, uint32_t wg,
                              uint32_t* table, uint32_t* packed, const ammsb_step_desc* desc, void* stream) {
   AMMSB_CHECK_ARG(ctx, ctx && desc, "null descriptor");
-  return sample_neighbors_common(ctx, seeds, nodes, n_nodes_cap, wg, table, packed, desc, stream);
+  return sample_neighbors_common(ctx, seeds, nodes, n_nodes_cap, wg, table, packed, desc, NsLinks{}, stream);
+}
+
+int ammsb_sample_neighbors_links_d(ammsb_ctx* ctx, ammsb_seed* seeds, const uint32_t* nodes, uint32_t n_nodes_cap,
+                                   uint32_t wg, uint32_t* table, uint32_t* packed, const uint64_t* csr_offsets,
+                                   const uint32_t* csr_targets, const ammsb_set* training_set, uint32_t* link_bits,
+                                   uint32_t* valid, const ammsb_step_desc* desc, void* stream) {
+  AMMSB_CHECK_ARG(ctx, ctx && desc && csr_offsets && csr_targets && training_set && link_bits, "null argument");
+  return sample_neighbors_common(ctx, seeds, nodes, n_nodes_cap, wg, table, packed, desc,
+                                 ns_links(ctx, csr_offsets, csr_targets, training_set, link_bits, valid), stream);
 }
 
 
diff --git a/mcmc-ammsb-gpu_amd/csrc/ammsb_loop.hip b/mcmc-ammsb-gpu_amd/csrc/ammsb_loop.hip
--- a/mcmc-ammsb-gpu_amd/csrc/ammsb_loop.hip
+++ b/mcmc-ammsb-gpu_amd/csrc/ammsb_loop.hip
@@ -104,6 +104,8 @@
   uint32_t* nodes;
   uint32_t* neighbors;
   uint32_t* nbr_table;
+  uint32_t* link_bits;
+  uint32_t* link_valid;
 };
 
 }
@@ -119,6 +121,7 @@
   hipEvent_t ev_main[NBUF], ev_samp[NBUF];
   SampleBuf buf[NBUF];
   void* own_mem;
+  uint32_t* link_mem;
   ammsb_step_desc* d_ring;
   uint32_t* d_cursor;
   ammsb_step_desc* d_cur[2];
@@ -189,8 +192,13 @@
     LOOP_RC(ammsb_minibatch_nonlink_d(ctx, c.mb_seeds, c.mb_candidates, m, &lp->training,
                                       lp->has_heldout ? &lp->heldout : nullptr, c.mb_workspace, o.edges, o.nodes,
                                       c.mb_count, desc, st));
-  LOOP_RC(ammsb_sample_neighbors_d(ctx, c.nbr_seeds[sp], o.nodes, nl ? lp->link_nodes_cap : m + 1, c.nbr_wg, o.nbr_table,
-                                   o.neighbors, desc, st));
+  if (o.link_bits)
+    LOOP_RC(ammsb_sample_neighbors_links_d(ctx, c.nbr_seeds[sp], o.nodes, nl ? lp->link_nodes_cap : m + 1, c.nbr_wg,
+                                           o.nbr_table, o.neighbors, c.csr_offsets, c.csr_targets, &lp->training,
+                                           o.link_bits, o.link_valid, desc, st));
+  else
+    LOOP_RC(ammsb_sample_neighbors_d(ctx, c.nbr_seeds[sp], o.nodes, nl ? lp->link_nodes_cap : m + 1, c.nbr_wg, o.nbr_table,
+                                     o.neighbors, desc, st));
   if (!lp->use_events) {
     loop_bump_kernel<<<1, 1, 0, st>>>(lp->d_hs + HS_AVAIL, desc);
     LOOP_HIP(lp, hipGetLastError());
@@ -207,7 +215,8 @@
   const uint32_t cap_nodes = cl ? lp->link_nodes_cap : m + 1;
   const uint32_t cap_edges = cl ? lp->link_edges_cap : m;
   LOOP_RC(ammsb_update_phi_d(ctx, c.beta, &lp->pi, c.phi_sum, &lp->training, in.nodes, in.neighbors, cap_nodes,
-                             c.phi_seeds, c.phi_wg, c.phi_flags, c.phi_vec, cur, lp->d_stamps, st));
+                             c.phi_seeds, c.phi_wg, c.phi_flags, c.phi_vec, cur, lp->d_stamps, in.link_bits, in.link_valid,
+                             st));
   const bool fuse_pi = ammsb_beta_can_fuse_pi(ctx, c.phi_wg, c.beta_wg) && lp->pi.num_cols % 4 == 0;
   const ammsb_pi_fusion fuse = {c.phi_vec, c.phi_sum, in.nodes, lp->d_stamps};
   if (!fuse_pi)
@@ -271,6 +280,7 @@
   if (lp->d_stamps) (void)hipFree(lp->d_stamps);
   if (lp->d_hs) (void)hipFree(lp->d_hs);
   if (lp->own_mem) (void)hipFree(lp->own_mem);
+  if (lp->link_mem) (void)hipFree(lp->link_mem);
   if (lp->side) (void)hipStreamDestroy(lp->side);
   if (lp->main) (void)hipStreamDestroy(lp->main);
   delete lp->runs;
@@ -388,7 +398,23 @@
   for (hipEvent_t* ev : {&lp->ev_in, &lp->ev_out, &lp->ev_prime, &lp->ev_first, &lp->ev_main[0], &lp->ev_main[1],
                          &lp->ev_main[2], &lp->ev_samp[0], &lp->ev_samp[1], &lp->ev_samp[2]})
     CREATE_HIP(hipEventCreateWithFlags(ev, hipEventDisableTiming));
-  for (int i = 0; i < 2; ++i) lp->buf[i] = SampleBuf{c.edges[i], c.nodes[i], c.neighbors[i], c.nbr_table[i]};
+  for (int i = 0; i < 2; ++i) lp->buf[i] = SampleBuf{c.edges[i], c.nodes[i], c.neighbors[i], c.nbr_table[i], nullptr, nullptr};
+  lp->buf[2].link_bits = lp->buf[2].link_valid = nullptr;
+  {
+    const char* f = getenv("AMMSB_LOOP_LINK_BITS");
+    if (f && strcmp(f, "0") == 0) {
+      fprintf(stderr, "ammsb_loop: AMMSB_LOOP_LINK_BITS=0 -- update_phi probes the training set for its link flags\n");
+    } else {
+      const size_t words = (size_t)c.max_nodes * ((lp->n_nbr + 31) / 32);
+      const size_t set_b = align256(sizeof(uint32_t) * words);
+      CREATE_HIP(hipMalloc(&lp->link_mem, NBUF * set_b + 256));
+      CREATE_HIP(hipMemset(lp->link_mem, 0, NBUF * set_b + 256));
+      for (int b = 0; b < NBUF; ++b) {
+        lp->buf[b].link_bits = lp->link_mem + b * (set_b / sizeof(uint32_t));
+        lp->buf[b].link_valid = lp->link_mem + NBUF * (set_b / sizeof(uint32_t)) + b;
+      }
+    }
+  }
   {
     const size_t e_b = align256(sizeof(uint64_t) * c.max_edges), n_b = align256(sizeof(uint32_t) * c.max_nodes);
     const size_t p_b = align256(sizeof(uint32_t) * (size_t)c.max_nodes * lp->n_nbr);
@@ -511,6 +537,7 @@
   auto choice = [&](uint32_t j) -> const ammsb_mb_choice& { return j == 0 ? *pending : next[j - 1]; };
   LOOP_HIP(lp, hipEventRecord(lp->ev_in, s));
   LOOP_HIP(lp, hipStreamWaitEvent(lp->main, lp->ev_in, 0));
+  if (done0 == 0 && lp->link_mem) LOOP_HIP(lp, hipMemsetAsync(lp->buf[p0 % NBUF].link_valid, 0, sizeof(uint32_t), lp->main));
   uint32_t done = done0;
   if (done0 == n_steps && avail0 <= n_steps) {
     Stage& st = lp->stage[lp->next_stage];
@@ -657,6 +684,7 @@
     copy(b.neighbors, a.neighbors, sizeof(uint32_t) * nv * lp->n_nbr);
     copy(b.nbr_table, a.nbr_table, sizeof(uint32_t) * nv * 2 * lp->n_nbr);
     LOOP_HIP(lp, hipGetLastError());
+    if (lp->link_mem) LOOP_HIP(lp, hipMemsetAsync(b.link_valid, 0, sizeof(uint32_t), lp->main));
   }
   LOOP_HIP(lp, hipEventRecord(lp->ev_out, lp->main));
   LOOP_HIP(lp, hipStreamWaitEvent(s, lp->ev_out, 0));
diff --git a/mcmc-ammsb-gpu_amd/csrc/ammsb_phi.hip b/mcmc-ammsb-gpu_amd/csrc/ammsb_phi.hip
--- a/mcmc-ammsb-gpu_amd/csrc/ammsb_phi.hip
+++ b/mcmc-ammsb-gpu_amd/csrc/ammsb_phi.hip
@@ -53,7 +53,21 @@
   uint32_t rows_nt;
   const ammsb_step_desc* desc;
   unsigned long long* stamps;
+  const uint32_t* link_bits;
+  const uint32_t* link_valid;
 };
+
+__device__ __forceinline__ const uint32_t* phi_link_bits(const PhiArgs& a) {
+  const uint32_t* lb = a.link_bits;
+  asm volatile("" : "+s"(lb));
+  if (lb && a.link_valid && *a.link_valid == 0u) lb = nullptr;
+  return lb;
+}
+__device__ __forceinline__ bool link_flag(const PhiArgs& a, const uint32_t* lb, uint64_t i, uint32_t q, uint32_t node,
+                                          uint32_t nb) {
+  if (lb) return ((lb[i * ((a.n + 31u) >> 5) + (q >> 5)] >> (q & 31u)) & 1u) != 0u;
+  return set_has(a.set, make_edge(node, nb));
+}
 
 
 struct PhiStep {
@@ -123,9 +137,10 @@
     const uint32_t node = a.nodes[i];
 
     __syncthreads();
+    const uint32_t* lb = phi_link_bits(a);
     for (uint32_t q = l; q < n; q += L) {
       const uint32_t nb = a.neighbors[i * n + q];
-      const bool y = set_has(a.set, make_edge(node, nb));
+      const bool y = link_flag(a, lb, i, q, node, nb);
       s_nb[q] = nb | (y ? 0x80000000u : 0u);
     }
     __syncthreads();
@@ -461,9 +476,10 @@
   for (uint64_t i = g; i < st.n_nodes; i += st.G) {
     const uint32_t node = a.nodes[i];
     group_sync();
+    const uint32_t* lb = phi_link_bits(a);
     for (uint32_t q = tid; q < n; q += L) {
       const uint32_t nbq = a.neighbors[i * n + q];
-      const bool y = set_has(a.set, make_edge(node, nbq));
+      const bool y = link_flag(a, lb, i, q, node, nbq);
       s_nb[q] = nbq | (y ? 0x80000000u : 0u);
     }
     group_sync();
@@ -646,9 +662,10 @@
     const uint32_t node = a.nodes[i];
     float* out = a.phi_vec + i * K;
     __syncthreads();
+    const uint32_t* lb = phi_link_bits(a);
     for (uint32_t q = tid; q < n; q += L) {
       const uint32_t nbq = a.neighbors[i * n + q];
-      const bool y = set_has(a.set, make_edge(node, nbq));
+      const bool y = link_flag(a, lb, i, q, node, nbq);
       s_nb[q] = nbq | (y ? 0x80000000u : 0u);
     }
     __syncthreads();
@@ -850,10 +867,11 @@
 #pragma unroll
     for (uint32_t r = 0; r < (uint32_t)(D - U); ++r)
       if (r < n) request(r, r);
+    const uint32_t* lb = phi_link_bits(a);
     const bool one_probe = n <= (uint32_t)L;
     const uint32_t my_nb = one_probe && (uint32_t)tid < n ? s_nb[tid] : 0u;
     SetProbe my_probe = {};
-    if (one_probe && (uint32_t)tid < n) my_probe = set_probe(a.set, make_edge(node, my_nb));
+    if (one_probe && (uint32_t)tid < n && !lb) my_probe = set_probe(a.set, make_edge(node, my_nb));
     float zraw[REGN ? KV : 1];
     if constexpr (REGN) {
       if (a.noise_on) {
@@ -862,11 +880,12 @@
       }
     }
     if (one_probe) {
-      if ((uint32_t)tid < n && set_hit(my_probe, make_edge(node, my_nb))) s_nb[tid] = my_nb | 0x80000000u;
+      if ((uint32_t)tid < n && (lb ? link_flag(a, lb, i, (uint32_t)tid, node, my_nb) : set_hit(my_probe, make_edge(node, my_nb))))
+        s_nb[tid] = my_nb | 0x80000000u;
     } else {
       for (uint32_t q = tid; q < n; q += L) {
         const uint32_t nb = s_nb[q];
-        if (set_has(a.set, make_edge(node, nb))) s_nb[q] = nb | 0x80000000u;
+        if (link_flag(a, lb, i, q, node, nb)) s_nb[q] = nb | 0x80000000u;
       }
     }
     __syncthreads();
@@ -1155,9 +1174,10 @@
 #pragma unroll
     for (uint32_t r = 0; r < (uint32_t)(D - U); ++r)
       if (r < n) request(r, r);
+    const uint32_t* lb = phi_link_bits(a);
     for (uint32_t q = l; q < n; q += 32) {
       const uint32_t nb = s_nb[q];
-      if (set_has(a.set, make_edge(node, nb))) s_nb[q] = nb | 0x80000000u;
+      if (link_flag(a, lb, i, q, node, nb)) s_nb[q] = nb | 0x80000000u;
     }
     asm volatile("s_waitcnt lgkmcnt(0)" ::: "memory");
     __builtin_amdgcn_wave_barrier();
@@ -1346,9 +1366,10 @@
   for (uint64_t i = g; i < st.n_nodes; i += st.G) {
     const uint32_t node = a.nodes[i];
     __syncthreads();
+    const uint32_t* lb = phi_link_bits(a);
     for (uint32_t q = tid; q < n; q += T) {
       const uint32_t nbq = a.neighbors[i * n + q];
-      const bool y = set_has(a.set, make_edge(node, nbq));
+      const bool y = link_flag(a, lb, i, q, node, nbq);
       s_nb[q] = nbq | (y ? 0x80000000u : 0u);
     }
     const float phi_sum = a.phi_sum[node];
@@ -2007,9 +2028,10 @@
   for (uint64_t i = g; i < st.n_nodes; i += st.G) {
     const uint32_t node = a.nodes[i];
     __syncthreads();
+    const uint32_t* lb = phi_link_bits(a);
     for (uint32_t q = t; q < n; q += T) {
       const uint32_t nbq = a.neighbors[i * n + q];
-      const bool y = set_has(a.set, make_edge(node, nbq));
+      const bool y = link_flag(a, lb, i, q, node, nbq);
       s_nb[q] = nbq | (y ? 0x80000000u : 0u);
     }
     __syncthreads();
@@ -2245,7 +2267,8 @@
                              const ammsb_set* training_set, const uint32_t* nodes, const uint32_t* neighbors,
                              uint32_t n_nodes, uint32_t step_count, ammsb_seed* seeds, uint32_t wg, uint32_t flags,
                              uint32_t group_begin, uint32_t group_end, float* phi_vec, const ammsb_step_desc* desc,
-                             unsigned long long* stamps, void* stream) {
+                             unsigned long long* stamps, const uint32_t* link_bits, const uint32_t* link_valid,
+                             void* stream) {
   AMMSB_CHECK_ARG(ctx, ctx && beta && pi && phi_sum && training_set && nodes && neighbors && seeds && phi_vec,
                   "null argument");
   AMMSB_CHECK_ARG(ctx, n_nodes > 0, "mini-batch nodes size = 0");
@@ -2286,6 +2309,8 @@
   a.eps_t = desc ? 0.0f : ammsb_eps_t(&p, step_count);
   a.desc = desc;
   a.stamps = stamps;
+  a.link_bits = link_bits;
+  a.link_valid = link_bits ? link_valid : nullptr;
   a.alpha = p.alpha;
   a.epsilon = p.epsilon;
   a.Nn = (1.0f * (float)p.N) / (float)p.num_node_sample;
@@ -2420,16 +2445,27 @@
                                 uint32_t n_nodes, uint32_t step_count, ammsb_seed* seeds, uint32_t wg, uint32_t flags,
                                 uint32_t group_begin, uint32_t group_end, float* phi_vec, void* stream) {
   return update_phi_common(ctx, beta, pi, phi_sum, training_set, nodes, neighbors, n_nodes, step_count, seeds, wg, flags,
-                           group_begin, group_end, phi_vec, nullptr, nullptr, stream);
+                           group_begin, group_end, phi_vec, nullptr, nullptr, nullptr, nullptr, stream);
+}
+
+extern "C" int ammsb_update_phi_links(ammsb_ctx* ctx, const float* beta, const ammsb_rpm* pi, const float* phi_sum,
+                                      const ammsb_set* training_set, const uint32_t* nodes, const uint32_t* neighbors,
+                                      const uint32_t* link_bits, uint32_t n_nodes, uint32_t step_count, ammsb_seed* seeds,
+                                      uint32_t wg, uint32_t flags, uint32_t group_begin, uint32_t group_end,
+                                      float* phi_vec, void* stream) {
+  AMMSB_CHECK_ARG(ctx, ctx && link_bits, "null argument");
+  return update_phi_common(ctx, beta, pi, phi_sum, training_set, nodes, neighbors, n_nodes, step_count, seeds, wg, flags,
+                           group_begin, group_end, phi_vec, nullptr, nullptr, link_bits, nullptr, stream);
 }
 
 int ammsb_update_phi_d(ammsb_ctx* ctx, const float* beta, const ammsb_rpm* pi, const float* phi_sum,
                        const ammsb_set* training_set, const uint32_t* nodes, const uint32_t* neighbors,
                        uint32_t n_nodes_cap, ammsb_seed* seeds, uint32_t wg, uint32_t flags, float* phi_vec,
-                       const ammsb_step_desc* desc, unsigned long long* stamps, void* stream) {
+                       const ammsb_step_desc* desc, unsigned long long* stamps, const uint32_t* link_bits,
+                       const uint32_t* link_valid, void* stream) {
   AMMSB_CHECK_ARG(ctx, ctx && desc, "null descriptor");
   return update_phi_common(ctx, beta, pi, phi_sum, training_set, nodes, neighbors, n_nodes_cap, 0, seeds, wg, flags, 0,
-                           0xFFFFFFFFu, phi_vec, desc, stamps, stream);
+                           0xFFFFFFFFu, phi_vec, desc, stamps, link_bits, link_valid, stream);
 }
 
 template <int KPT, int W, int D>
diff --git a/mcmc-ammsb-gpu_amd/csrc/ammsb_step.h b/mcmc-ammsb-gpu_amd/csrc/ammsb_step.h
--- a/mcmc-ammsb-gpu_amd/csrc/ammsb_step.h
+++ b/mcmc-ammsb-gpu_amd/csrc/ammsb_step.h
@@ -62,7 +62,8 @@
 int ammsb_update_phi_d(ammsb_ctx* ctx, const float* beta, const ammsb_rpm* pi, const float* phi_sum,
                        const ammsb_set* training_set, const uint32_t* nodes, const uint32_t* neighbors,
                        uint32_t n_nodes_cap, ammsb_seed* seeds, uint32_t wg, uint32_t flags, float* phi_vec,
-                       const ammsb_step_desc* desc, unsigned long long* stamps, void* stream);
+                       const ammsb_step_desc* desc, unsigned long long* stamps, const uint32_t* link_bits,
+                       const uint32_t* link_valid, void* stream);
 int ammsb_update_pi_d(ammsb_ctx* ctx, const ammsb_rpm* pi, float* phi_sum, const float* phi_vec, const uint32_t* nodes,
                       uint32_t n_nodes_cap, uint32_t wg, const ammsb_step_desc* desc, unsigned long long* stamps,
                       void* stream);
@@ -78,6 +79,10 @@
                       const ammsb_pi_fusion* fuse, unsigned long long* stamps, void* stream);
 int ammsb_sample_neighbors_d(ammsb_ctx* ctx, ammsb_seed* seeds, const uint32_t* nodes, uint32_t n_nodes_cap, uint32_t wg,
                              uint32_t* table, uint32_t* packed, const ammsb_step_desc* desc, void* stream);
+int ammsb_sample_neighbors_links_d(ammsb_ctx* ctx, ammsb_seed* seeds, const uint32_t* nodes, uint32_t n_nodes_cap,
+                                   uint32_t wg, uint32_t* table, uint32_t* packed, const uint64_t* csr_offsets,
+                                   const uint32_t* csr_targets, const ammsb_set* training_set, uint32_t* link_bits,
+                                   uint32_t* valid, const ammsb_step_desc* desc, void* stream);
 int ammsb_minibatch_link_d(ammsb_ctx* ctx, const uint64_t* csr_offsets, const uint32_t* csr_targets, uint32_t n_cap,
                            uint64_t* edges_out, uint32_t* nodes_out, const ammsb_step_desc* desc, void* stream);
 int ammsb_minibatch_nonlink_d(ammsb_ctx* ctx, ammsb_seed* seeds, uint32_t n_candidates_cap, uint32_t m,
diff --git a/mcmc-ammsb-gpu_amd/ops.py b/mcmc-ammsb-gpu_amd/ops.py
--- a/mcmc-ammsb-gpu_amd/ops.py
+++ b/mcmc-ammsb-gpu_amd/ops.py
@@ -276,6 +276,14 @@
             self.ctx.handle, _ptr(self.rand.seeds), _ptr(nodes), int(num_samples), self.local,
             _ptr(self.hash), _ptr(self.data), _stream()))
 
+    def sample_links(self, num_samples, nodes, csr_offsets, csr_targets, training_set, link_bits):
+        if num_samples > self.max_nodes:
+            raise AmmsbError("%d samples > buffer for %d" % (num_samples, self.max_nodes))
+        self.ctx.check(self.ctx.lib.ammsb_sample_neighbors_links(
+            self.ctx.handle, _ptr(self.rand.seeds), _ptr(nodes), int(num_samples), self.local,
+            _ptr(self.hash), _ptr(self.data), _ptr(csr_offsets), _ptr(csr_targets), C.byref(training_set.desc),
+            _ptr(link_bits), _stream()))
+
     def GetHash(self):
         return self.hash
 
@@ -311,6 +319,17 @@
                                        C.byref(self.set.desc), _ptr(nodes), _ptr(neighbors), int(n),
                                        self.count_calls, _ptr(self.rand.seeds), self.local, self.flags,
                                        int(group_begin), int(group_end), _ptr(self.phi_vec), _stream()))
+
+    def update_phi_links(self, nodes, neighbors, link_bits, n, group_begin=0, group_end=0xFFFFFFFF):
+        if n == 0:
+            raise AmmsbError("mini-batch nodes size = 0!")
+        if n > self.max_nodes:
+            raise AmmsbError("grads too small")
+        c = self.ctx
+        c.check(c.lib.ammsb_update_phi_links(c.handle, _ptr(self.beta), C.byref(self.pi.desc), _ptr(self.phi),
+                                             C.byref(self.set.desc), _ptr(nodes), _ptr(neighbors), _ptr(link_bits),
+                                             int(n), self.count_calls, _ptr(self.rand.seeds), self.local, self.flags,
+                                             int(group_begin), int(group_end), _ptr(self.phi_vec), _stream()))
 
     def update_pi(self, nodes, n, phi_vec=None):
         c = self.ctx
```

After: 35.27 million. 0.957x the previous value.
